# sourcedennis/wasm-pathtracer

Measured on AMD Instinct MI355X. Metric: Mray/s (primary+shadow+bounce) at 1920x1080, 1/2/4/8 GPU; L2 vs CPU ref, higher is better.
Workload: dtype f32; 1 GPU; C3 bunny scene (scene id 2), 1920x1080, 64 spp per GPU share (64 spp frame), depth 8, NormalNEE; rays=25682600955, parallelism=single GPU

## Files before the change

### include/wpt.h

```cpp
#ifndef WPT_H
#define WPT_H

#include <stddef.h>
#include <stdint.h>

#ifdef __cplusplus
extern "C" {
#endif

#define WPT_OK 0
#define WPT_ERR_NOT_INIT (-1)
#define WPT_ERR_ALREADY_INIT (-2)
#define WPT_ERR_INVALID_SCENE (-3)
#define WPT_ERR_INVALID_ARG (-4)
#define WPT_ERR_UNSUPPORTED (-5)
#define WPT_ERR_DEVICE (-6)
#define WPT_ERR_NO_MESH (-7)

#define WPT_NO_NEE 0
#define WPT_NORMAL_NEE 1
#define WPT_PNEE 2


int wpt_init(uint32_t width, uint32_t height, uint32_t scene_id, float cam_x, float cam_y, float cam_z,
// ... 17 lines not shown
int wpt_notify_mesh_loaded(uint32_t id);
int wpt_load_obj(uint32_t id, const char* text, size_t len, const float* scale, uint64_t* num_vertices);
int wpt_parse_obj(const char* text, size_t len, const float* scale, float* out, uint64_t capacity,
                  uint64_t* num_vertices);

uint8_t* wpt_allocate_texture(uint32_t id, uint32_t width, uint32_t height);

int wpt_notify_texture_loaded(uint32_t id);

int wpt_compute(size_t num_samples);


const char* wpt_last_error(void);

int wpt_set_device(int device);

int wpt_set_render_options(int32_t max_depth, uint32_t frame_seed, uint64_t batch_paths);

int wpt_set_partition(uint32_t rank, uint32_t nranks, uint32_t tile);

int64_t wpt_partition_pixels(uint32_t* out);

int64_t wpt_tile_partition(uint32_t width, uint32_t height, uint32_t rank, uint32_t nranks, uint32_t tile,
                           uint32_t* out);

int64_t wpt_photon_tree(uint32_t* child, float* cum, uint64_t* shot_stored);

int wpt_read_radiance(float* acc3, uint32_t* cnt);

int wpt_copy_partition(void* device_dst);

typedef int (*wpt_exchange_fn)(void* user);
int wpt_set_exchange(wpt_exchange_fn fn, void* user, void* local_dev, void* gathered_dev, uint64_t slot);
int64_t wpt_exchange_slot(void);

int wpt_comm_unique_id(void* out128);
int wpt_set_comm(uint32_t rank, uint32_t nranks, uint32_t tile, const void* unique_id128);
int wpt_gather_frame(uint32_t root);
int wpt_comm_destroy(void);
#define WPT_XFER_GATHER 0
#define WPT_XFER_ALLGATHER 1
typedef int (*wpt_transport_fn)(void* user, int32_t op, uint32_t root);
int wpt_set_transport(wpt_transport_fn fn, void* user, void* send_dev, void* recv_dev, uint64_t slot);
int64_t wpt_gather_plan(uint32_t rank, uint32_t nranks, uint32_t root, uint64_t slot, uint64_t* out);
float wpt_seq_sum(const float* v, uint64_t n);
float wpt_seq_sum_chunks(const float* v, uint64_t n);
int wpt_seq_sum_device(const float* v, uint64_t n, float* out);

int wpt_stats(uint64_t* out, size_t n);
int wpt_kernel_times(double* out, size_t n);
int wpt_set_counting(int on);
int wpt_set_profiling(int on);
int wpt_set_lanes(int32_t n);
#define WPT_OPT_DEFAULTS 0
#define WPT_OPT_TRAVERSAL 1
#define WPT_OPT_TRAVERSAL_SH 2
#define WPT_OPT_FUSED 3
#define WPT_OPT_FUSED_BELOW 4
#define WPT_OPT_SMALL_LANES 5
#define WPT_OPT_PIXEL_TILE 6
#define WPT_OPT_GRID_PCT 7
#define WPT_OPT_REFILL 8
#define WPT_OPT_REFILL_SH 9
#define WPT_OPT_TREELET 10
#define WPT_OPT_BVH_BUILD 11
#define WPT_OPT_LANES 12
#define WPT_OPT_FINISH_BELOW 13
#define WPT_OPT_TRACE_GRID_PCT 14
#define WPT_OPT_FINISH_EVERY 20
#define WPT_OPT_PROBE 22
#define WPT_OPT_STOCK 23
#define WPT_OPT_STOCK_LANES 24
#define WPT_OPT_FILL 25
#define WPT_OPT_ASYNC_PRIO 26
#define WPT_OPT_ASYNC_GRID_PCT 27
#define WPT_OPT_STOCK_AHEAD 30
#define WPT_OPT_STOCK_EVERY 32
#define WPT_OPT_STOCK_EXTRA 33
#define WPT_OPT_ASYNC_ONESHOT 31
#define WPT_OPT_STOCK_PREFILL 35
#define WPT_OPT_ASYNC_FUSED_BELOW 36
#define WPT_OPT_PRESOLVE 37
#define WPT_OPT_DROP_MISS 38
#define WPT_OPT_LOG 34
#define WPT_OPT_SCENE_TRAVERSAL 28
#define WPT_OPT_SCENE_TRI_ONLY 29
int wpt_set_option(int32_t option, int64_t value);
int64_t wpt_probe_read(uint32_t* meta, uint32_t* rec, uint64_t* rec_entries, double* ticks_per_us);
int wpt_get_option(int32_t option, int64_t* value);
int wpt_scene_build_info(double* out);
int wpt_clear_stats(void);
int wpt_sync(void);
int wpt_bvh_depth(void);

int wpt_trace_rays(size_t n, const float* rays, float* t_out, int32_t* id_out);
int wpt_shadow_rays(size_t n, const float* pq, const int32_t* light, uint8_t* occluded);
int wpt_presolve_rays(size_t n, const float* rays, uint8_t* resolved, float* t_out, int32_t* id_out);

int wpt_shutdown(void);

void* wpt_debug_scene_new(int32_t scene_id, const float* mesh_vertices, size_t num_vertices);
int wpt_debug_scene_info(void* h, uint64_t* out);
int wpt_debug_scene_nodes4(void* h, uint32_t* out);
int wpt_debug_scene_nodes(void* h, uint32_t* out);
int wpt_debug_scene_shapes(void* h, float* out);
int wpt_debug_scene_lights(void* h, uint32_t* out);
int wpt_debug_scene_presolve(void* h, size_t n, const float* rays, uint8_t* resolved, float* t_out, int32_t* id_out);
int wpt_debug_scene_guards(void* h, uint32_t* num_guards, float* boxes, uint32_t* leaf_guard);
void wpt_debug_scene_free(void* h);
void* wpt_debug_scene_new_gpu(int32_t scene_id, const float* mesh_vertices, size_t num_vertices);
int wpt_debug_scene_build_info(void* h, double* out);

#ifdef __cplusplus
}
#endif

#endif
```

### wasm-pathtracer_amd/_lib.py

```python
import ctypes
import os

HERE = os.path.dirname(os.path.abspath(__file__))
_VARIANT = os.environ.get("WPT_LIB_VARIANT", "")
LIB_PATH = os.path.join(HERE, f"libwpt_{_VARIANT}.so" if _VARIANT else "libwpt.so")

_lib = None

c_u32, c_i32, c_f32, c_sz = ctypes.c_uint32, ctypes.c_int32, ctypes.c_float, ctypes.c_size_t
c_p = ctypes.c_void_p

_SIGS = {
    "wpt_init": (ctypes.c_int, [c_u32, c_u32, c_u32, c_f32, c_f32, c_f32, c_f32, c_f32]),
    "wpt_results": (ctypes.POINTER(ctypes.c_uint8), [c_u32]),
    "wpt_update_scene": (ctypes.c_int, [c_u32]),
    "wpt_update_settings": (ctypes.c_int, [c_u32, c_u32, c_u32, c_u32, c_u32]),
    "wpt_update_viewport": (ctypes.c_int, [c_u32, c_u32]),
    "wpt_update_camera": (ctypes.c_int, [c_f32, c_f32, c_f32, c_f32, c_f32]),
    "wpt_allocate_mesh": (ctypes.c_int, [c_u32, c_u32]),
    "wpt_mesh_vertices": (ctypes.POINTER(ctypes.c_float), [c_u32]),
    "wpt_notify_mesh_loaded": (ctypes.c_int, [c_u32]),
    "wpt_load_obj": (ctypes.c_int, [c_u32, ctypes.c_char_p, c_sz, c_p, c_p]),
    "wpt_parse_obj": (ctypes.c_int, [ctypes.c_char_p, c_sz, c_p, c_p, ctypes.c_uint64, c_p]),
    "wpt_allocate_texture": (ctypes.POINTER(ctypes.c_uint8), [c_u32, c_u32, c_u32]),
    "wpt_notify_texture_loaded": (ctypes.c_int, [c_u32]),
    "wpt_compute": (ctypes.c_int, [c_sz]),
    "wpt_last_error": (ctypes.c_char_p, []),
    "wpt_set_device": (ctypes.c_int, [ctypes.c_int]),
    "wpt_set_render_options": (ctypes.c_int, [c_i32, c_u32, ctypes.c_uint64]),
    "wpt_set_partition": (ctypes.c_int, [c_u32, c_u32, c_u32]),
    "wpt_partition_pixels": (ctypes.c_int64, [c_p]),
    "wpt_tile_partition": (ctypes.c_int64, [c_u32, c_u32, c_u32, c_u32, c_u32, c_p]),
    "wpt_photon_tree": (ctypes.c_int64, [c_p, c_p, c_p]),
    "wpt_read_radiance": (ctypes.c_int, [c_p, c_p]),
    "wpt_copy_partition": (ctypes.c_int, [c_p]),
    "wpt_set_exchange": (ctypes.c_int, [c_p, c_p, c_p, c_p, ctypes.c_uint64]),
    "wpt_exchange_slot": (ctypes.c_int64, []),
    "wpt_stats": (ctypes.c_int, [c_p, c_sz]),
    "wpt_kernel_times": (ctypes.c_int, [c_p, c_sz]),
    "wpt_set_counting": (ctypes.c_int, [ctypes.c_int]),
    "wpt_set_profiling": (ctypes.c_int, [ctypes.c_int]),
    "wpt_set_lanes": (ctypes.c_int, [ctypes.c_int32]),
    "wpt_set_option": (ctypes.c_int, [ctypes.c_int32, ctypes.c_int64]),
    "wpt_get_option": (ctypes.c_int, [ctypes.c_int32, c_p]),
    "wpt_probe_read": (ctypes.c_int64, [c_p, c_p, c_p, c_p]),
    "wpt_scene_build_info": (ctypes.c_int, [c_p]),
    "wpt_clear_stats": (ctypes.c_int, []),
    "wpt_sync": (ctypes.c_int, []),
    "wpt_bvh_depth": (ctypes.c_int, []),
    "wpt_trace_rays": (ctypes.c_int, [c_sz, c_p, c_p, c_p]),
    "wpt_shadow_rays": (ctypes.c_int, [c_sz, c_p, c_p, c_p]),
    "wpt_presolve_rays": (ctypes.c_int, [c_sz, c_p, c_p, c_p, c_p]),
    "wpt_debug_scene_presolve": (ctypes.c_int, [c_p, c_sz, c_p, c_p, c_p, c_p]),
    "wpt_debug_scene_guards": (ctypes.c_int, [c_p, c_p, c_p, c_p]),
    "wpt_shutdown": (ctypes.c_int, []),
    "wpt_debug_scene_new": (c_p, [c_i32, c_p, c_sz]),
    "wpt_debug_scene_info": (ctypes.c_int, [c_p, c_p]),
    "wpt_debug_scene_nodes": (ctypes.c_int, [c_p, c_p]),
    "wpt_debug_scene_shapes": (ctypes.c_int, [c_p, c_p]),
    "wpt_debug_scene_nodes4": (ctypes.c_int, [c_p, c_p]),
    "wpt_comm_unique_id": (ctypes.c_int, [c_p]),
    "wpt_set_comm": (ctypes.c_int, [c_u32, c_u32, c_u32, c_p]),
    "wpt_gather_frame": (ctypes.c_int, [c_u32]),
    "wpt_comm_destroy": (ctypes.c_int, []),
    "wpt_set_transport": (ctypes.c_int, [c_p, c_p, c_p, c_p, ctypes.c_uint64]),
    "wpt_gather_plan": (ctypes.c_int64, [c_u32, c_u32, c_u32, ctypes.c_uint64, c_p]),
    "wpt_seq_sum": (ctypes.c_float, [c_p, ctypes.c_uint64]),
    "wpt_seq_sum_chunks": (ctypes.c_float, [c_p, ctypes.c_uint64]),
    "wpt_seq_sum_device": (ctypes.c_int, [c_p, ctypes.c_uint64, c_p]),
    "wpt_debug_scene_lights": (ctypes.c_int, [c_p, c_p]),
    "wpt_debug_scene_free": (None, [c_p]),
    "wpt_debug_scene_new_gpu": (c_p, [c_i32, c_p, c_sz]),
    "wpt_debug_scene_build_info": (ctypes.c_int, [c_p, c_p]),
}

EXPORTED = tuple(_SIGS)


def header_symbols():
    import re
    hdr = os.path.join(os.path.dirname(HERE), "include", "wpt.h")
    txt = open(hdr).read()
    return sorted(set(re.findall(r"\b(wpt_[a-z_0-9]+)\s*\(", txt)))


def lib():
    global _lib
    if _lib is not None:
        return _lib
    try:
        import torch
    except ImportError:
        pass
    if not os.path.exists(LIB_PATH):
        raise RuntimeError(f"{LIB_PATH} is missing: run __graft_entry__.build() (make -C wasm-pathtracer_amd/csrc)")
    L = ctypes.CDLL(LIB_PATH)
    for name, (res, args) in _SIGS.items():
        f = getattr(L, name)
        f.restype = res
        f.argtypes = args
    _lib = L
    return L
```

### wasm-pathtracer_amd/csrc/wpt_api.cpp

```cpp
#include <cstring>
#include <map>
#include <memory>
#include <string>
#include <vector>

#include "../../include/wpt.h"
#include "wpt_bvh_gpu.h"
#include "wpt_comm.h"
#include "wpt_obj.h"
#include "wpt_partition.h"
#include "wpt_render.h"
#include "wpt_seqsum.h"

using namespace wpt;

namespace {

struct Session {
  std::map<uint32_t, std::vector<float>> preload;
  std::map<uint32_t, std::vector<float>> meshes;
  std::map<uint32_t, std::vector<uint8_t>> textures;
  uint32_t scene_id = 0;
  HostScene scene;
  Renderer renderer;
// ... 411 lines not shown
  std::string err;
  if (!s.renderer.copy_partition((float*)s.comm_send, err)) return fail(WPT_ERR_DEVICE, err);
  if (!comm_gather(s.comm, s.comm_send, s.comm_recv, s.comm_slot, root, s.renderer.stream(), err))
    return fail(WPT_ERR_DEVICE, err);
  if (comm_rank(s.comm) == root && !s.renderer.unpack_ranks(s.comm_recv, s.comm_slot, err))
    return fail(WPT_ERR_DEVICE, err);
  return WPT_OK;
}

namespace {
int xfer_exchange(void* user) {
  Session& s = *(Session*)user;
  return s.xfer(s.xfer_user, WPT_XFER_ALLGATHER, 0);
}
}

int wpt_set_transport(wpt_transport_fn fn, void* user, void* send_dev, void* recv_dev, uint64_t slot) {
  if (!g_session) return fail(WPT_ERR_NOT_INIT, "init not called");
  Session& s = *g_session;
  if (!fn) {
    if (s.xfer) {
      s.renderer.set_exchange(nullptr, nullptr, nullptr, nullptr, 0);
      s.xfer = nullptr;
      s.xfer_user = nullptr;
      s.xfer_send = s.xfer_recv = nullptr;
      s.xfer_slot = 0;
    }
    return WPT_OK;
  }
  if (!send_dev || !recv_dev) return fail(WPT_ERR_INVALID_ARG, "null transport buffer");
  if (slot < s.renderer.exchange_slot() || slot < s.renderer.part_pixels())
    return fail(WPT_ERR_INVALID_ARG, "transport slot smaller than the largest partition");
  s.drop_comm();
  s.xfer = fn;
  s.xfer_user = user;
  s.xfer_send = (float4*)send_dev;
  s.xfer_recv = (float4*)recv_dev;
  s.xfer_slot = slot;
  s.renderer.set_exchange(xfer_exchange, &s, send_dev, recv_dev, slot);
  return WPT_OK;
}

int64_t wpt_gather_plan(uint32_t rank, uint32_t nranks, uint32_t root, uint64_t slot, uint64_t* out) {
  if (nranks == 0 || rank >= nranks || root >= nranks) return fail(WPT_ERR_INVALID_ARG, "bad rank");
  std::vector<XferOp> ops;
  gather_plan(rank, nranks, root, slot, ops);
  if (out)
    for (size_t i = 0; i < ops.size(); i++) {
      out[4 * i] = ops[i].peer;
      out[4 * i + 1] = ops[i].offset;
      out[4 * i + 2] = ops[i].count;
      out[4 * i + 3] = ops[i].recv ? 1u : 0u;
    }
  return (int64_t)ops.size();
}

float wpt_seq_sum(const float* v, uint64_t n) { return wpt::seq_sum_f32(v, (size_t)n); }

float wpt_seq_sum_chunks(const float* v, uint64_t n) {
  std::vector<wpt::ChunkEff> eff(2 * ((size_t)n / wpt::kSumChunk + 1));
  wpt::seq_sum_effects(v, (size_t)n, eff.data());
  return wpt::seq_sum_walk(v, (size_t)n, eff.data());
}

int wpt_seq_sum_device(const float* v, uint64_t n, float* out) {
  if (!g_session) return fail(WPT_ERR_NOT_INIT, "init not called");
  if (!out || (n && !v)) return fail(WPT_ERR_INVALID_ARG, "null pointer");
  std::string err;
  if (!g_session->renderer.seq_sum_device(v, n, *out, err)) return fail(WPT_ERR_DEVICE, err);
  return WPT_OK;
}

int wpt_comm_destroy(void) {
  if (!g_session) return fail(WPT_ERR_NOT_INIT, "init not called");
  g_session->drop_comm();
  return WPT_OK;
}

int wpt_stats(uint64_t* out, size_t n) {
  if (!g_session) return fail(WPT_ERR_NOT_INIT, "init not called");
  std::string err;
  if (!g_session->renderer.flush_counts(err)) return fail(WPT_ERR_DEVICE, err);
  const Stats& st = g_session->renderer.stats();
  uint64_t v[42] = {st.paths,          st.rays,           st.shadow_rays,    st.node_visits,  st.prim_tests,
                    st.bounces,        st.ext_visits,     st.ext_tests,      st.ext_node_bytes, st.sh_visits,
                    st.sh_tests,       st.sh_node_bytes,  st.fallback_ext,   st.fallback_sh,  st.ext_lane_iters,
                    st.ext_live_iters, st.sh_lane_iters,  st.sh_live_iters,  st.photon_rays,  st.photons,
                    st.sum_chunks,     st.sum_resummed,   st.sum_fetched,    st.stock_consumed, st.fill_paths,
                    st.trace_bytes,    st.finish_paths,   st.finish_max_bounces, st.max_ray_visits,
                    st.ex_body_lanes,  st.ex_bodies,      st.lf_body_lanes,  st.lf_bodies,    st.stock_traced,
                    st.stock_deficit,  st.stock_waits,    st.plan_us,        st.stock_us,
                    st.stock_rays,     st.stock_rays_used, st.presolved_rays,
                    st.dropped_rays};
  for (size_t i = 0; i < n && i < 42; i++) out[i] = v[i];
  return WPT_OK;
}

int wpt_kernel_times(double* out, size_t n) {
  if (!g_session) return fail(WPT_ERR_NOT_INIT, "init not called");
  const KernelTimes& t = g_session->renderer.times();
  double v[28] = {t.generate, (double)t.n_generate, t.extend, (double)t.n_extend, t.shade, (double)t.n_shade,
                  t.shadow, (double)t.n_shadow, t.accumulate, (double)t.n_accumulate, t.trace, (double)t.n_trace};
  for (int k = 0; k < 6; k++) {
    v[12 + 2 * k] = t.busy[k];
    v[13 + 2 * k] = (double)t.logical[k];
  }
  v[24] = t.retrace;
  v[25] = (double)t.n_retrace;
  v[26] = t.busy[6];
  v[27] = (double)t.logical[6];
  for (size_t i = 0; i < n && i < 28; i++) out[i] = v[i];
  return WPT_OK;
}

int wpt_set_counting(int on) {
  if (!g_session) return fail(WPT_ERR_NOT_INIT, "init not called");
  g_session->renderer.set_counting(on != 0);
  return WPT_OK;
}

int wpt_scene_build_info(double* out) {
  if (!g_session) return fail(WPT_ERR_NOT_INIT, "init not called");
  if (!out) return fail(WPT_ERR_INVALID_ARG, "null argument");
  out[0] = g_session->scene.bvh_ms;
  out[1] = g_session->scene.bvh_on_gpu ? 1.0 : 0.0;
  return WPT_OK;
}

int wpt_set_lanes(int32_t n) {
  if (!g_session) return fail(WPT_ERR_NOT_INIT, "init not called");
  if (!g_session->renderer.set_lanes(n)) return fail(WPT_ERR_INVALID_ARG, "lanes out of range");
  return WPT_OK;
}

int wpt_set_option(int32_t option, int64_t value) {
  if (option == WPT_OPT_BVH_BUILD) {
    if (value < 0 || value > 2) return fail(WPT_ERR_INVALID_ARG, "option value out of range");
    g_bvh_build = (int)value;
    return WPT_OK;
  }
  std::string err;
  if (!g_session) {
    if (option == WPT_OPT_DEFAULTS) {
      g_default_opts.clear();
      g_bvh_build = 0;
      return WPT_OK;
    }
    if (option == WPT_OPT_LANES && (value < 1 || value > kMaxLanes)) return fail(WPT_ERR_INVALID_ARG, "lanes out of range");
    if (option != WPT_OPT_LANES && option != WPT_OPT_GRID_PCT) {
      Renderer probe;
      if (!probe.set_option(option, value, err)) return fail(WPT_ERR_INVALID_ARG, err);
    } else if (option == WPT_OPT_GRID_PCT && (value < 1 || value > 100)) {
      return fail(WPT_ERR_INVALID_ARG, "option value out of range");
    }
    g_default_opts[option] = value;
    return WPT_OK;
  }
  Session& s = *g_session;
  int64_t prev = 0;
  const bool had = s.renderer.get_option(option, prev);
  if (!s.renderer.set_option(option, value, err)) return fail(WPT_ERR_INVALID_ARG, err);
  if (Renderer::scene_option(option)) {
    const int rc = rebuild_scene(s, s.scene_id);
    if (rc != WPT_OK) {
      const std::string keep = g_err;
      std::string e2;
      if (had) (void)s.renderer.set_option(option, prev, e2);
      g_err = keep;
      return rc;
    }
    return reset_session(s);
  }
  if (option == WPT_OPT_PIXEL_TILE && s.renderer.nranks() == 1) {
    if (!s.renderer.set_partition(s.renderer.rank(), s.renderer.nranks(), s.renderer.tile(), err))
      return fail(WPT_ERR_DEVICE, err);
  }
  return WPT_OK;
}

int64_t wpt_probe_read(uint32_t* meta, uint32_t* rec, uint64_t* rec_entries, double* ticks_per_us) {
  if (!g_session) return fail(WPT_ERR_NOT_INIT, "init not called");
  Session& s = *g_session;
  std::string err;
  if (!meta || !rec) {
    if (!s.renderer.probe_read(s.probe_meta, s.probe_rec, s.probe_tpu, err)) return fail(WPT_ERR_DEVICE, err);
    s.probe_taken = true;
    if (rec_entries) *rec_entries = s.probe_rec.size();
    if (ticks_per_us) *ticks_per_us = s.probe_tpu;
    return (int64_t)(s.probe_meta.size() / 5);
  }
  if (!s.probe_taken) return fail(WPT_ERR_INVALID_ARG, "probe: call with meta = rec = NULL first (size query)");
  if (!rec_entries || *rec_entries < s.probe_rec.size())
    return fail(WPT_ERR_INVALID_ARG, "probe: rec smaller than the size query's entries");
  std::memcpy(meta, s.probe_meta.data(), s.probe_meta.size() * sizeof(uint32_t));
  std::memcpy(rec, s.probe_rec.data(), s.probe_rec.size() * sizeof(uint4));
  *rec_entries = s.probe_rec.size();
  if (ticks_per_us) *ticks_per_us = s.probe_tpu;
  const int64_t n = (int64_t)(s.probe_meta.size() / 5);
  s.probe_meta.clear();
  s.probe_rec.clear();
  s.probe_taken = false;
  return n;
}

int wpt_get_option(int32_t option, int64_t* value) {
  if (!value) return fail(WPT_ERR_INVALID_ARG, "null argument");
  if (option == WPT_OPT_BVH_BUILD) { *value = g_bvh_build; return WPT_OK; }
  if (!g_session) {
    auto it = g_default_opts.find(option);
    if (it != g_default_opts.end()) { *value = it->second; return WPT_OK; }
    Renderer probe;
    if (!probe.get_option(option, *value)) return fail(WPT_ERR_INVALID_ARG, "unknown option");
    return WPT_OK;
  }
  if (!g_session->renderer.get_option(option, *value)) return fail(WPT_ERR_INVALID_ARG, "unknown option");
  return WPT_OK;
}

int wpt_set_profiling(int on) {
  if (!g_session) return fail(WPT_ERR_NOT_INIT, "init not called");
  g_session->renderer.set_profiling(on != 0);
  return WPT_OK;
}

int wpt_clear_stats(void) {
  if (!g_session) return fail(WPT_ERR_NOT_INIT, "init not called");
  g_session->renderer.clear_stats();
  return WPT_OK;
}

int wpt_sync(void) {
  if (!g_session) return fail(WPT_ERR_NOT_INIT, "init not called");
  std::string err;
  if (!g_session->renderer.sync(err)) return fail(WPT_ERR_DEVICE, err);
  return WPT_OK;
}

int wpt_bvh_depth(void) {
  if (!g_session) return fail(WPT_ERR_NOT_INIT, "init not called");
  return (int)g_session->renderer.bvh_depth();
}

int wpt_trace_rays(size_t n, const float* rays, float* t_out, int32_t* id_out) {
  if (!g_session) return fail(WPT_ERR_NOT_INIT, "init not called");
  std::string err;
  if (!g_session->renderer.trace_rays(n, rays, t_out, id_out, err)) return fail(WPT_ERR_DEVICE, err);
  return WPT_OK;
}

int wpt_presolve_rays(size_t n, const float* rays, uint8_t* resolved, float* t_out, int32_t* id_out) {
  if (!g_session) return fail(WPT_ERR_NOT_INIT, "init not called");
  if (n && (!rays || !resolved || !t_out || !id_out)) return fail(WPT_ERR_INVALID_ARG, "null argument");
  std::string err;
  if (!g_session->renderer.presolve_rays(n, rays, resolved, t_out, id_out, err)) return fail(WPT_ERR_DEVICE, err);
  return WPT_OK;
}

int wpt_shadow_rays(size_t n, const float* pq, const int32_t* light, uint8_t* occluded) {
  if (!g_session) return fail(WPT_ERR_NOT_INIT, "init not called");
  std::string err;
  if (!g_session->renderer.shadow_rays(n, pq, light, occluded, err)) return fail(WPT_ERR_INVALID_ARG, err);
  return WPT_OK;
}

int wpt_shutdown(void) {
  if (!g_session) return fail(WPT_ERR_NOT_INIT, "init not called");
  delete g_session;
  g_session = nullptr;
  return WPT_OK;
}

void* wpt_debug_scene_new(int32_t scene_id, const float* mesh_vertices, size_t num_vertices) {
  std::vector<float> mesh;
  if (mesh_vertices && num_vertices) mesh.assign(mesh_vertices, mesh_vertices + ((num_vertices / 3) * 9));
  HostScene* sc = new HostScene();
  std::string err;
  if (!build_scene(scene_id, mesh, *sc, err)) {
    delete sc;
    fail(WPT_ERR_INVALID_SCENE, err);
    return nullptr;
  }
  return sc;
}

void* wpt_debug_scene_new_gpu(int32_t scene_id, const float* mesh_vertices, size_t num_vertices) {
  static BvhGpu* gpu = nullptr;
  const hipError_t he = hipSetDevice(g_device);
  if (he != hipSuccess) {
    fail(WPT_ERR_DEVICE, std::string("hipSetDevice failed: ") + hipGetErrorString(he));
    return nullptr;
  }
  if (!gpu) gpu = new BvhGpu();
  gpu->min_shapes = 0;
  std::vector<float> mesh;
  if (mesh_vertices && num_vertices) mesh.assign(mesh_vertices, mesh_vertices + ((num_vertices / 3) * 9));
  HostScene* sc = new HostScene();
  std::string err;
  if (!build_scene(scene_id, mesh, *sc, err, gpu)) {
    delete sc;
    fail(err.rfind("HIP error", 0) == 0 || err.rfind("GPU BVH", 0) == 0 ? WPT_ERR_DEVICE : WPT_ERR_INVALID_SCENE,
         err);
    return nullptr;
  }
  return sc;
}

int wpt_debug_scene_build_info(void* h, double* out) {
  if (!h || !out) return fail(WPT_ERR_INVALID_ARG, "null argument");
  const HostScene* sc = (const HostScene*)h;
  out[0] = sc->bvh_ms;
  out[1] = sc->bvh_on_gpu ? 1.0 : 0.0;
  return WPT_OK;
}

int wpt_debug_scene_info(void* h, uint64_t* out) {
  const HostScene* sc = (const HostScene*)h;
  if (!sc) return fail(WPT_ERR_INVALID_ARG, "null scene");
  uint64_t v[8] = {sc->shapes.size(), sc->num_inf, sc->nodes.size(), sc->lights.size(), sc->depth,
                   sc->use_bvh ? 1u : 0u, sc->tri_only ? 1u : 0u, sc->nodes4.size()};
  memcpy(out, v, sizeof v);
  return WPT_OK;
}

int wpt_debug_scene_nodes(void* h, uint32_t* out) {
  const HostScene* sc = (const HostScene*)h;
  if (!sc) return fail(WPT_ERR_INVALID_ARG, "null scene");
  for (size_t i = 0; i < sc->nodes.size(); i++) {
    const Node2& n = sc->nodes[i];
    float b[6] = {n.bmin[0], n.bmin[1], n.bmin[2], n.bmax[0], n.bmax[1], n.bmax[2]};
    memcpy(out + 8 * i, b, sizeof b);
    out[8 * i + 6] = n.left_first;
    out[8 * i + 7] = n.count;
  }
  return WPT_OK;
}

int wpt_debug_scene_nodes4(void* h, uint32_t* out) {
  const HostScene* sc = (const HostScene*)h;
  if (!sc) return fail(WPT_ERR_INVALID_ARG, "null scene");
  for (size_t i = 0; i < sc->nodes4.size(); i++) {
    const Node4& n = sc->nodes4[i];
    uint32_t* o = out + 37 * i;
    memset(o, 0, 37 * sizeof(uint32_t));
    for (int k = 0; k < 4; k++) {
      const uint32_t c = n.child[k];
      if (c == kChildEmpty) continue;
      o[0]++;
      uint32_t* e = o + 1 + 9 * k;
      if (!(c & 0x80000000u)) {
        e[0] = 1;
        e[1] = c;
      } else {
        e[0] = 2;
        if ((c & 0xC0000000u) == 0xC0000000u) {
          e[1] = sc->leaf_table[2 * (c & 0x3FFFFFFFu)];
          e[2] = sc->leaf_table[2 * (c & 0x3FFFFFFFu) + 1];
        } else {
          e[1] = c & 0xFFFFFFu;
          e[2] = (c >> 24) & 0x3Fu;
        }
      }
      const float b[6] = {n.xmin[k], n.ymin[k], n.zmin[k], n.xmax[k], n.ymax[k], n.zmax[k]};
      memcpy(e + 3, b, sizeof b);
    }
  }
  return WPT_OK;
}

int wpt_debug_scene_shapes(void* h, float* out) {
  const HostScene* sc = (const HostScene*)h;
  if (!sc) return fail(WPT_ERR_INVALID_ARG, "null scene");
  for (size_t i = 0; i < sc->shapes.size(); i++) {
    const Shape& s = sc->shapes[i];
    float* o = out + 16 * i;
    memcpy(o, s.g, sizeof s.g);
    o[12] = (float)s.kind;
    o[13] = s.emissive ? 1.0f : 0.0f;
    o[14] = 0.0f;
    o[15] = 0.0f;
  }
  return WPT_OK;
}

int wpt_debug_scene_lights(void* h, uint32_t* out) {
  const HostScene* sc = (const HostScene*)h;
  if (!sc) return fail(WPT_ERR_INVALID_ARG, "null scene");
  for (size_t i = 0; i < sc->lights.size(); i++) out[i] = sc->lights[i];
  return WPT_OK;
}

int wpt_debug_scene_presolve(void* h, size_t n, const float* rays, uint8_t* resolved, float* t_out, int32_t* id_out) {
  const HostScene* sc = (const HostScene*)h;
  if (!sc || (n && (!rays || !resolved || !t_out || !id_out))) return fail(WPT_ERR_INVALID_ARG, "null argument");
  HostPlanes hp{};
  hp.num_inf = 0;
  PresolveBoxes pre{};
  if (sc->use_bvh && sc->shapes.size() > sc->num_inf && sc->num_inf <= 16) {
    pre = sc->pre;
    hp.num_inf = sc->num_inf;
    for (uint32_t i = 0; i < sc->num_inf; i++) {
      const float* g = sc->shapes[i].g;
      const V3 loc = mk(g[0], g[1], g[2]), nrm = mk(g[3], g[4], g[5]);
      hp.planes[i] = HostPlanes::P4{nrm.x, nrm.y, nrm.z, dot(nrm, loc)};
    }
  }
  for (size_t i = 0; i < n; i++) {
    const float* r = rays + 6 * i;
    resolved[i] = presolve_ray(hp, pre, mk(r[0], r[1], r[2]), mk(r[3], r[4], r[5]), t_out[i], id_out[i]) ? 1 : 0;
  }
  return WPT_OK;
}

int wpt_debug_scene_guards(void* h, uint32_t* num_guards, float* boxes, uint32_t* leaf_guard) {
  const HostScene* sc = (const HostScene*)h;
  if (!sc || !num_guards) return fail(WPT_ERR_INVALID_ARG, "null argument");
  *num_guards = sc->pre.num_guards;
  if (boxes) {
    memcpy(boxes, sc->pre.root, 6 * sizeof(float));
    memcpy(boxes + 6, sc->pre.guard, 6 * kMaxGuards * sizeof(float));
  }
  if (leaf_guard)
    for (size_t i = 0; i < sc->nodes.size(); i++) leaf_guard[i] = i < sc->leaf_guard.size() ? sc->leaf_guard[i] : ~0u;
  return WPT_OK;
}

void wpt_debug_scene_free(void* h) { delete (HostScene*)h; }

}
```

### wasm-pathtracer_amd/csrc/wpt_presolve.h

```cpp
#pragma once
#include "wpt_math.h"

namespace wpt {

constexpr int kMaxGuards = 4;

struct PresolveBoxes {
  uint32_t num_guards;
  float root[6];
  float guard[kMaxGuards][6];
};

WPT_HD void presolve_slab(const float* b, V3 o, V3 inv, float& hh, float& tmax) {
  const float tx1 = (b[0] - o.x) * inv.x;
  const float tx2 = (b[3] - o.x) * inv.x;
  const float ty1 = (b[1] - o.y) * inv.y;
  const float ty2 = (b[4] - o.y) * inv.y;
  const float tz1 = (b[2] - o.z) * inv.z;
  const float tz2 = (b[5] - o.z) * inv.z;
  const float tmin = fmaxf(fmaxf(fminf(tx1, tx2), fminf(ty1, ty2)), fminf(tz1, tz2));
  tmax = fminf(fminf(fmaxf(tx1, tx2), fmaxf(ty1, ty2)), fmaxf(tz1, tz2));
  hh = fmaxf(tmin, 0.0f);
}

WPT_HD float presolve_inf() {
#if defined(__HIP_DEVICE_COMPILE__)
  float v;
  asm volatile("v_mov_b32 %0, 0x7f800000" : "=v"(v));
  return v;
#else
  return u2f(0x7f800000u);
#endif
}

template <class SC>
WPT_HD bool presolve_ray(const SC& S, const PresolveBoxes& B, V3 o, V3 d, float& t, int32_t& id) {
  t = 0.0f;
  id = -1;
  if (B.num_guards == 0u) return false;
  if (d.x == 0.0f || d.y == 0.0f || d.z == 0.0f) return false;
  const V3 inv = mk(1.0f / d.x, 1.0f / d.y, 1.0f / d.z);
  const float inf = presolve_inf();
  if (!(fabsf(inv.x) < inf) || !(fabsf(inv.y) < inf) || !(fabsf(inv.z) < inf)) return false;
  float best = inf;
  int32_t best_id = -1;
  bool found = false;
  for (uint32_t i = 0; i < S.num_inf; i++) {
    const V3 n = mk(S.planes[i].x, S.planes[i].y, S.planes[i].z);
    const float n_dot_dir = dot(n, d);
    if (n_dot_dir == 0.0f) continue;
    const float tt = (S.planes[i].w - dot(n, o)) / n_dot_dir;
    if (tt <= 0.0f) continue;
    if (!found || (0.0f < tt && tt < best)) {
      found = true;
      best = tt;
      best_id = (int32_t)i;
    }
  }
  float hh, tmax;
  presolve_slab(B.root, o, inv, hh, tmax);
  if ((hh <= tmax) & (hh < best)) {
    bool clear = true;
#if defined(__HIP_DEVICE_COMPILE__)
#pragma unroll
#endif
    for (int g = 0; g < kMaxGuards; g++) {
      if ((uint32_t)g < B.num_guards) {
        presolve_slab(B.guard[g], o, inv, hh, tmax);
        clear = clear && (!(hh <= tmax) || best < hh);
      }
    }
    if (!clear) return false;
  }
  t = best_id >= 0 ? best : inf;
  id = best_id;
  return true;
}

struct HostPlanes {
  struct P4 { float x, y, z, w; };
  P4 planes[16];
  uint32_t num_inf;
};

}
```

### wasm-pathtracer_amd/csrc/wpt_render.h

```cpp
#pragma once
#include <hip/hip_runtime.h>
#include <stdint.h>
#include <string>
#include <algorithm>
#include <deque>
#include <vector>

#include "wpt_scene.h"
#include "wpt_seqsum.h"

namespace wpt {

constexpr int kMaxInf = 16;
constexpr int kMaxBvhDepth = 4096;
constexpr int kMaxBounces = 512;

struct DevScene {
  const float4* nodes;
  const float4* tree;
  uint32_t tree_pairs, tree_root_lf;
  const float4* prims;
  const uint32_t* kinds;
  const float4* all;
  const uint32_t* all_kinds;
  const float4* mats;
  const float4* lights;
  const float4* nodes4;
  const uint32_t* leaf_table;
  uint32_t num_inf, num_finite, num_shapes, num_lights;
  uint32_t use_bvh, tri_only;
  uint32_t refill_lanes;
  uint32_t refill_lanes_sh;
  int stack_cap;
  uint32_t* overflow;
  const uint32_t* oct_child;
  const float* oct_cum;
  const uint32_t* oct_corners;
  uint32_t oct_nodes;
  uint32_t oct_lds_words;
  float bg[3];
  float4 planes[kMaxInf];
  uint4* probe;
  const PresolveBoxes* pre;
};

struct Stats {
  uint64_t paths = 0;
  uint64_t rays = 0;
  uint64_t shadow_rays = 0;
  uint64_t node_visits = 0;
  uint64_t prim_tests = 0;
  uint64_t bounces = 0;
  uint64_t ext_visits = 0, ext_tests = 0, ext_node_bytes = 0;
  uint64_t sh_visits = 0, sh_tests = 0, sh_node_bytes = 0;
  uint64_t fallback_ext = 0, fallback_sh = 0;
  uint64_t ex_body_lanes = 0, ex_bodies = 0, lf_body_lanes = 0, lf_bodies = 0;
  uint64_t ext_lane_iters = 0, ext_live_iters = 0, sh_lane_iters = 0, sh_live_iters = 0;
  uint64_t photon_rays = 0, photons = 0;
  uint64_t trace_bytes = 0;
  uint64_t max_ray_visits = 0;
  uint64_t sum_chunks = 0, sum_resummed = 0, sum_fetched = 0;
  uint64_t finish_paths = 0, finish_max_bounces = 0;
  uint64_t stock_traced = 0, stock_consumed = 0, fill_paths = 0;
  uint64_t stock_deficit = 0, stock_waits = 0, plan_us = 0, stock_us = 0;
  uint64_t stock_rays = 0;
  uint64_t stock_rays_used = 0;
  uint64_t presolved_rays = 0;
  uint64_t dropped_rays = 0;
};

constexpr int kTimedKernels = 7;
struct KernelTimes {
  double generate = 0, extend = 0, shade = 0, shadow = 0, accumulate = 0, trace = 0, retrace = 0;
  uint64_t n_extend = 0, n_shadow = 0, n_shade = 0, n_generate = 0, n_accumulate = 0, n_trace = 0, n_retrace = 0;
  double busy[kTimedKernels] = {0, 0, 0, 0, 0, 0, 0};
  uint64_t logical[kTimedKernels] = {0, 0, 0, 0, 0, 0, 0};
};

constexpr int kMaxLanes = 8;
constexpr uint64_t kMinLanePaths = 1024;
constexpr size_t kFinishWord = 2 + 2 * (size_t)kMaxBounces;
constexpr size_t kResWord = kFinishWord + 4;
constexpr size_t kCountWords = kResWord + 2 * ((size_t)kMaxBounces + 1);
static_assert(kResWord % 2 == 0, "the presolved counts are 64-bit slots");
constexpr uint32_t kWorkWords = 16;
constexpr uint32_t kWorkCopies = 64;
struct PathSet {
  hipStream_t stream = nullptr;
  hipStream_t lo = nullptr;
  hipEvent_t done = nullptr;
  uint64_t cap = 0;
  uint32_t* pixel = nullptr;
  float4* col = nullptr;
  float4* ro[2] = {nullptr, nullptr};
  float4* rd[2] = {nullptr, nullptr};
  float4* thr[2] = {nullptr, nullptr};
  float* t = nullptr;
  int32_t* id = nullptr;
  float* t1 = nullptr;
  int32_t* id1 = nullptr;
  float4 *so = nullptr, *sd = nullptr, *sc = nullptr;
  uint32_t* counts = nullptr;
  uint32_t* h_counts = nullptr;
  uint2* spill = nullptr;
  size_t spill_cap = 0;
  float* hit_t(int k) const { return k ? t1 : t; }
  int32_t* hit_id(int k) const { return k ? id1 : id; }
  uint32_t* ext_count(int b) const { return b == 0 ? counts : counts + 2 + 2 * (b - 1); }
  uint32_t* sh_count(int b) const { return counts + 3 + 2 * b; }
  unsigned long long* append_ctr(int b) const { return reinterpret_cast<unsigned long long*>(counts + 2 + 2 * b); }
  unsigned long long* res_ctr(int b) const { return reinterpret_cast<unsigned long long*>(counts + kResWord + 2 * b); }
};

constexpr int kAsyncLane0 = 2;
struct Batch {
  enum State { kNew, kBouncing, kCountWait, kIssued };
  uint64_t k0 = 0, n = 0;
  int half = -1;
  const uint32_t* part = nullptr;
  uint32_t npix = 0;
  const uint32_t* moff = nullptr;
  const uint32_t* mbase = nullptr;
  const uint32_t* mlist = nullptr;
  uint32_t nent = 0;
  bool stock = false;
  bool async = false;
  int queue = 0;
  int lane0 = 0, nl = 1;
  uint64_t off[kMaxLanes + 1] = {};
  bool fused = false, pnee = false;
  bool presolve = false;
  int maxb = 0, b = 0;
  bool finished = false;
  State state = kNew;
  hipEvent_t done[kMaxLanes] = {};
  hipEvent_t live[kMaxLanes] = {};
  uint32_t* hc = nullptr;
  uint32_t* hl = nullptr;
};

struct LaunchCtx {
  int lane = 0;
  const PathSet* ps = nullptr;
  hipStream_t stream = nullptr;
  bool async = false;
  uint64_t paths = 0;
  int batch_lanes = 1;
  bool timed = false;
  bool count = false;
  int bounce = 0;
  int hit_sel = 0;
  const uint32_t* probe_res = nullptr;
};

class Renderer {
 public:
  Renderer();
  ~Renderer();
  bool set_device(int dev, std::string& err);
  bool upload_scene(const HostScene& sc, std::string& err);
  bool set_viewport(uint32_t w, uint32_t h, std::string& err);
  void set_camera(const float cam[5]);
  void set_types(int left, int right, int debug) { left_type_ = left; right_type_ = right; debug_ = debug; }
  void set_adaptive(bool left, bool right) { adaptive_[0] = left; adaptive_[1] = right; }
  bool adaptive() const { return adaptive_[0] || adaptive_[1]; }
  bool fill_sampling_blue(std::string& err);
  bool sampling_rgba(uint8_t* out, std::string& err);
  void set_options(int max_depth, uint32_t seed, uint64_t batch) {
    if (seed != seed_) photons_ok_ = false;
    max_depth_ = max_depth; seed_ = seed; if (batch) batch_ = batch;
  }
  bool build_photons(std::string& err);
  bool photon_tree(std::vector<uint32_t>& child, std::vector<float>& cum, uint64_t& shot, uint64_t& stored,
                   std::string& err);
  bool set_partition(uint32_t rank, uint32_t nranks, uint32_t tile, std::string& err);
  bool reset(std::string& err);
  bool compute(uint64_t num_paths, std::string& err);
  bool sync(std::string& err);
  bool results_rgba(uint8_t* host_out, std::string& err);
  bool read_radiance(float* acc3, uint32_t* cnt, std::string& err);
  bool copy_partition(float* dev_dst, std::string& err);
  using ExchangeFn = int (*)(void*);
  void set_exchange(ExchangeFn fn, void* user, void* local_dev, void* gathered_dev, uint64_t slot) {
    xfn_ = fn; xuser_ = user; xlocal_ = (float4*)local_dev; xall_ = (float4*)gathered_dev; xslot_ = slot;
  }
  uint64_t exchange_slot() const { return maxpart_; }
  uint32_t rank() const { return rank_; }
  uint32_t nranks() const { return nranks_; }
  uint32_t tile() const { return tile_; }
  bool unpack_ranks(const float4* gathered, uint64_t slot, std::string& err);
  bool trace_rays(size_t n, const float* rays, float* t_out, int32_t* id_out, std::string& err);
  bool presolve_rays(size_t n, const float* rays, uint8_t* resolved, float* t_out, int32_t* id_out, std::string& err);
  bool shadow_rays(size_t n, const float* pq, const int32_t* light, uint8_t* occ, std::string& err);
  bool probe_read(std::vector<uint32_t>& meta, std::vector<uint4>& rec, double& ticks_per_us, std::string& err);
  void set_counting(bool on) { counting_ = on; }
  void set_profiling(bool on) { profiling_ = on; }
  bool set_lanes(int n) {
    if (n < 1 || n > lanes_made_) return false;
    nlanes_ = n;
    return true;
  }
  int lanes() const { return nlanes_; }
  static bool scene_option(int opt) { return opt == 1 || opt == 2 || opt == 10; }
  bool set_option(int opt, int64_t v, std::string& err);
  bool get_option(int opt, int64_t& v) const;
  int wants_bvh4() const {
    return (traversal_ == 1 || traversal_sh_ == 1) ? 1 : (traversal_ == 3 || traversal_sh_ == 3) ? 2 : 0;
  }
  bool seq_sum_device(const float* v, uint64_t n, float& out, std::string& err);
  const Stats& stats() const { return stats_; }
  const KernelTimes& times() const { return times_; }
  void clear_stats() {
    std::string e;
    (void)flush_counts(e);
    stats_ = Stats();
    times_ = KernelTimes();
  }
  bool flush_counts(std::string& err);
  uint32_t width() const { return w_; }
  uint32_t height() const { return h_; }
  uint32_t part_pixels() const { return (uint32_t)part_pix_.size(); }
  const std::vector<uint32_t>& part_list() const { return part_pix_; }
  hipStream_t stream() const { return stream_; }
  uint32_t bvh_depth() const { return depth_; }

 private:
  bool ensure_paths(uint64_t n, std::string& err);
  bool ensure_lane(int i, uint64_t n, std::string& err);
  void free_lane_paths(PathSet& L);
  LaunchCtx batch_ctx(const Batch& B, int i, int b) const;
  LaunchCtx lane0_ctx(bool count) const;
  bool run_batch(uint64_t k0, uint64_t n, int half, std::string& err, const uint32_t* part_pix = nullptr,
                 uint32_t part_n = 0, const Batch* map = nullptr);
  bool batch_begin(Batch& B, std::string& err);
  bool batch_advance(Batch& B, bool block, std::string& err);
  bool batch_tail(Batch& B, std::string& err);
  void batch_counts(const Batch& B, const uint32_t* hc);
  bool pump(bool block, std::string& err);
  bool wait_issued(Batch* B, std::string& err);
  bool drain_async(std::string& err);
  bool host_wait(hipEvent_t e, std::string& err);
  bool host_wait_stream(hipStream_t s, std::string& err);
  hipEvent_t ev_sync_ = nullptr;
  uint64_t batch_cap() const;
  int main_lanes() const;
  bool compute_half(int h, uint64_t n, std::string& err);
  bool merge_random_halves(uint64_t nl, uint64_t nr, bool& merged, std::string& err);
  bool plan_round(int h, std::string& err);
  bool exchange_frame(std::string& err);
  bool plan_slice(int h, uint64_t a, uint64_t b, uint64_t& local, std::string& err);
  void free_rounds();
  bool launch_extend(const LaunchCtx& C, const float4* ro, const float4* rd, const uint32_t* cnt, std::string& err);
  bool launch_shadow(const LaunchCtx& C, const uint32_t* cnt, uint8_t* occ_out, std::string& err);
  bool launch_trace(const LaunchCtx& C, std::string& err);
  bool size_grids(std::string& err);
  uint32_t max_grid() const;
  size_t spill_slots() const;
  uint32_t spill_grid(const PathSet& L) const;
  bool ensure_spill(int l, uint32_t grid, std::string& err);
  uint32_t oneshot_grid(uint64_t paths) const {
    const uint64_t g = (2 * paths + 255) / 256;
    const uint64_t gmax = (1ull << 30) / (sizeof(uint2) * 256 * spill_slots());
    return (uint32_t)std::max<uint64_t>(1, std::min(g, gmax));
  }
  void free_scene();
  void free_paths();
  void free_photons();
  bool adaptive_[2] = {false, false};
  struct HalfRounds {
    uint64_t total = 0, pos = 0;
    uint32_t idx = 0;
    uint32_t* rc = nullptr;
    uint32_t* rbase = nullptr;
    uint32_t* gc = nullptr;
    uint32_t* gbase = nullptr;
// ... 44 lines not shown
  uint32_t refill_id_ = 0;
  int refill_lane_ = 0;
  uint32_t round_need_[2] = {0, 0};
  bool stock_redo_[2] = {false, false};
  int log_ = 0;
  bool stock_active(int h) const { return stock_slots_ != 0 && nranks_ == 1 && adaptive_[h]; }
  bool stock_alloc(std::string& err);
  void stock_drop();
  bool stock_round(int h, uint64_t left, std::string& err);
  bool stock_consume(int h, uint64_t a, uint64_t b, std::string& err);
  bool stock_flush(std::string& err);
  bool refill_count(Refill& f, bool block, std::string& err);
  uint32_t refill_scale(int h, uint32_t ahead, uint64_t after) const;
  Refill* refill_slot(std::string& err);
  void refill_plan(Refill& F, int h, uint32_t ahead, uint32_t q);
  bool refill_issue(Refill& F, int h, uint64_t wt, std::string& err);
  bool stock_prefill(int h, uint64_t budget, std::string& err);
  bool stock_prefill_ = true;
  std::deque<Batch*> aq_[2];
  bool fill_on_ = false;
  int async_prio_ = 0;
  int async_grid_pct_ = 100;
  uint64_t async_fused_below_ = 1ull << 26;
  uint32_t* d_seam_pix_[2] = {nullptr, nullptr};
  uint32_t* d_rest_pix_[2] = {nullptr, nullptr};
  uint32_t seam_npix_[2] = {0, 0}, rest_npix_[2] = {0, 0};
  static constexpr int kMaxFill = 8;
  Batch fill_[kMaxFill];
  int nfill_ = 0;
  hipEvent_t fill_ev_[kMaxFill][2] = {};
  uint32_t* h_fill_cnt_ = nullptr;
  bool async_pending() const { return !aq_[0].empty() || !aq_[1].empty(); }
  int fill_lane() const { return kAsyncLane0 + stock_lanes_; }
  bool issue_fill(int h, uint64_t k0, uint64_t n, std::string& err);
  bool drain_fill(std::string& err);
  bool compute_halves(uint64_t nl, uint64_t nr, std::string& err);
  uint32_t async_grid(const LaunchCtx& C, uint32_t g, int base_pct, uint32_t rays_per_path = 1) const {
    if (!C.async) return g;
    if (async_oneshot_) return std::max<uint32_t>(1u, (uint32_t)((C.paths * rays_per_path + 255) / 256));
    return async_grid_pct_ > 0 ? std::max<uint32_t>(1u, (uint32_t)((uint64_t)g * async_grid_pct_ / base_pct)) : g;
  }
  bool async_oneshot_ = false;
  uint8_t* d_samp_ = nullptr;
  ExchangeFn xfn_ = nullptr;
  void* xuser_ = nullptr;
  float4* xlocal_ = nullptr;
  float4* xall_ = nullptr;
  uint64_t xslot_ = 0;
  uint64_t maxpart_ = 0;
  uint32_t* d_xidx_ = nullptr;
  bool photons_ok_ = false;
  uint64_t photons_shot_ = 0, photons_stored_ = 0;
  std::vector<uint32_t> oct_child_;
  std::vector<float> oct_cum_;
  uint32_t* d_oct_child_ = nullptr;
  float* d_oct_cum_ = nullptr;
  uint32_t* d_oct_corners_ = nullptr;

  int device_ = -1;
  int ncu_ = 256;
  static constexpr int kTravVariants = 8;
  uint32_t grid_ext_[2 * kTravVariants] = {};
  uint32_t grid_sh_[2 * kTravVariants] = {};
  uint32_t grid_tr_[4] = {};
  uint32_t grid_shade_ = 512;
  uint32_t shade_occ_[32] = {};
  size_t shade_occ_smem_[32] = {};
  bool fused_ = false;
  uint64_t fused_below_ = 1ull << 24;
  int small_lanes_ = 2;
  int traversal_ = 3, traversal_sh_ = 3;
  int trav_ext_ = 0, trav_sh_ = 0;
  bool treelet_ = true;
  uint32_t pixel_tile_ = 8;
  int grid_pct_ = 50;
#ifndef WPT_TRACE_GRID_PCT
#define WPT_TRACE_GRID_PCT 75
#endif
  int trace_grid_pct_ = WPT_TRACE_GRID_PCT;
  uint32_t refill_ = 12, refill_sh_ = 16;
  uint64_t finish_below_ = 1u << 18;
  int finish_every_ = 4;
  uint32_t num_guards_ = 0;
  bool presolve_ = true;
  bool drop_miss_ = true;
  uint32_t probe_cap_ = 0, probe_waves_ = 0, probe_used_ = 0;
  uint4* d_probe_ = nullptr;
  std::vector<uint32_t> probe_meta_;
  uint4* probe_slot(const LaunchCtx& C, int kernel, uint32_t grid);
  uint32_t* d_fallback_ = nullptr;
  hipStream_t stream_ = nullptr;
  PathSet lanes_[kMaxLanes];
  int lanes_made_ = 0;
  bool stats_pending_ = false;
  int pend_nl_ = 0, pend_b_ = 0;
  bool pend_stock_ = false, pend_presolve_ = false;
  int nlanes_ = 4;
  hipEvent_t ev_main_ = nullptr;
  hipEvent_t ev_ref_ = nullptr;
  std::vector<void*> scene_bufs_;
  DevScene ds_{};
  uint32_t depth_ = 0;
  bool scene_ok_ = false;

  uint32_t w_ = 0, h_ = 0;
  float cam_[5] = {0, 0, 0, 0, 0};
  int left_type_ = 1, right_type_ = 1, debug_ = 0;
  int max_depth_ = 0;
  uint32_t seed_ = 0xBABABEBEu;
  uint64_t batch_ = 1ull << 27;

  uint32_t rank_ = 0, nranks_ = 1, tile_ = 16;
  std::vector<uint32_t> part_pix_;
  uint32_t* d_part_pix_ = nullptr;
  uint32_t* d_half_pix_[2] = {nullptr, nullptr};
  uint32_t* d_frame_pix_ = nullptr;
  uint32_t half_npix_[2] = {0, 0};
  uint64_t next_path_ = 0;

  float4* d_acc_ = nullptr;
  uint32_t* d_cnt_ = nullptr;
  uint8_t* d_rgba_ = nullptr;

  unsigned long long* d_work_ = nullptr;
  uint32_t* h_word_ = nullptr;

  bool counting_ = false;
  bool profiling_ = false;
  Stats stats_;
  KernelTimes times_;
  struct PendingTiming {
    hipEvent_t a, b;
    int slot;
  };
  bool next_event(hipEvent_t* e, std::string& err);
  bool resolve_timings(std::string& err);
  std::vector<hipEvent_t> ev_pool_;
  size_t ev_used_ = 0;
  std::vector<PendingTiming> pending_;
};

}
```

### wasm-pathtracer_amd/csrc/wpt_render.hip

```cpp
#include "wpt_render.h"
#include "wpt_partition.h"
#include "wpt_photon.h"
#include "wpt_quartic.h"
#include "wpt_seqsum.h"

#include <algorithm>
#include <chrono>
#include <cstdlib>
#include <cmath>
#include <cstdio>
#include <cstring>
#include <deque>
#include <mutex>
#include <unordered_map>
#include <thread>
#include <type_traits>

#define HIP_OK(expr)                                                     \
  do {                                                                   \
    hipError_t e_ = (expr);                                              \
    if (e_ != hipSuccess) {                                              \
      err = std::string(#expr " failed: ") + hipGetErrorString(e_);      \
      return false;                                                      \
    }                                                                    \
// ... 925 lines not shown
  const bool self_z = xs_next(s) <= wz;
  const float ajx = xs * xo, ajy = ys * yo, ajz = zs * zo;
  uint32_t corner[8];
  if (depth <= kOctLattice) {
    const int32_t kx = (int32_t)((b[0] + sz) / xs), ky = (int32_t)((b[1] + sz) / ys), kz = (int32_t)((b[2] + sz) / zs);
    const uint32_t ax = oct_cell(v.x + ajx, kx + (int32_t)xo, xs, depth);
    const uint32_t ay = oct_cell(v.y + ajy, ky + (int32_t)yo, ys, depth);
    const uint32_t az = oct_cell(v.z + ajz, kz + (int32_t)zo, zs, depth);
    corner[0] = leaf;
    const int32_t last = (1 << depth) - 1;
    const auto adj = [&](int32_t k, float off) {
      const int32_t a = k + (int32_t)off;
      return (uint32_t)(a < 0 ? 0 : (a > last ? last : a));
    };
    if (WPT_OCT_TABLE && S.oct_corners && ax == adj(kx, xo) && ay == adj(ky, yo) && az == adj(kz, zo)) {
      const uint32_t ocase = (xo > 0.0f ? 4u : 0u) | (yo > 0.0f ? 2u : 0u) | (zo > 0.0f ? 1u : 0u);
      const uint4* row = reinterpret_cast<const uint4*>(S.oct_corners + 64 * (size_t)leaf + 8 * ocase);
      const uint4 q0 = row[0], q1 = row[1];
      corner[1] = q0.y;
      corner[2] = q0.z;
      corner[3] = q0.w;
      corner[4] = q1.x;
      corner[5] = q1.y;
      corner[6] = q1.z;
      corner[7] = q1.w;
    } else {
#pragma unroll
      for (int c = 1; c < 8; c++)
        corner[c] =
            oct_walk(O, (c & 4) ? ax : (uint32_t)kx, (c & 2) ? ay : (uint32_t)ky, (c & 1) ? az : (uint32_t)kz, depth);
    }
  } else {
    float nb[6];
    int d;
    corner[0] = leaf;
#pragma unroll
    for (int c = 1; c < 8; c++)
      corner[c] = oct_find(S, O, add(v, mk((c & 4) ? ajx : 0.0f, (c & 2) ? ajy : 0.0f, (c & 1) ? ajz : 0.0f)), depth, nb, d);
  }
  const int pick = (self_x ? 0 : 4) + (self_y ? 0 : 2) + (self_z ? 0 : 1);
  uint32_t node = corner[0];
#pragma unroll
  for (int c = 1; c < 8; c++) node = pick == c ? corner[c] : node;
  const auto cum = O.cum + (size_t)node * S.num_lights;
  const float r = xs_next(s);
  uint32_t lo = 0, hi = S.num_lights;
  while (lo + 1u < hi) {
    const uint32_t mid = (lo + hi) / 2u;
    if (cum[mid] <= r) lo = mid;
    else hi = mid;
  }
  light = lo;
  float p = 0.0f;
  p += oct_bin_prob(S, O, corner[0], lo) * wx * wy * wz;
  p += oct_bin_prob(S, O, corner[4], lo) * wax * wy * wz;
  p += oct_bin_prob(S, O, corner[2], lo) * wx * way * wz;
  p += oct_bin_prob(S, O, corner[1], lo) * wx * wy * waz;
  p += oct_bin_prob(S, O, corner[6], lo) * wax * way * wz;
  p += oct_bin_prob(S, O, corner[3], lo) * wx * way * waz;
  p += oct_bin_prob(S, O, corner[5], lo) * wax * wy * waz;
  p += oct_bin_prob(S, O, corner[7], lo) * wax * way * waz;
  pdf = p;
}

template <bool TRI_ONLY>
__device__ __forceinline__ V3 hit_normal(const DevScene& S, int32_t id, V3 o, V3 d, float t) {
  uint32_t kind;
  const float4* rec = shape_rec<TRI_ONLY>(S, id, kind);
  if (rec) return TRI_ONLY ? tri_normal(rec, d) : prim_normal(kind, rec, o, d, t);
  V3 pn = ld3(S.planes[id]);
  if (dot(pn, d) > 0.0f) pn = neg(pn);
  return normalize(pn);
}

__device__ __forceinline__ void st_hit(float* t, int32_t* id, float tv, int32_t iv) {
  *t = tv;
  *id = iv;
}

struct ShadeParams {
  int max_depth;
  int debug;
  int drop_miss;
};

struct RayStream {
  float4* o;
  float4* d;
  float4* thr;
};
struct ShadowStream {
  float4* o;
  float4* d;
  float4* c;
};

struct ShadeOut {
  bool alive, shadow;
  float4 ro, rd, th;
  float4 so, sd, sc;
};

template <bool TRI_ONLY, bool PNEE, class OV, bool CR = false>
__device__ __forceinline__ void shade_path(const DevScene& S, const OV& O, const ShadeParams& P,
                                           float4* __restrict__ col, float t,
                                           int32_t id, float4 o4, float4 d4, float4 th4, ShadeOut& R,
                                           const lds_f4v* lq = nullptr) {
  const V3 o = ld3(o4), d = ld3(d4);
  const uint32_t path = __float_as_uint(d4.w);
  V3 thr = ld3(th4);
  uint32_t flags = __float_as_uint(th4.w);
  const uint32_t type = (flags >> kTypeShift) & 3u;
  const bool has_nee = type == 1u || type == 2u;
  bool bounced = (flags & kFlagBounced) != 0;
  const uint32_t depth = ((flags >> kDepthShift) & kDepthMask) + 1u;
  auto end_counts = [&](uint32_t nsh) {
    if constexpr (CR) reinterpret_cast<uint32_t*>(col + path)[3] = depth | (nsh << 16);
  };
  if (id < 0) {
    const V3 add_c = mulv(thr, mk(S.bg[0], S.bg[1], S.bg[2]));
    if ((__float_as_uint(add_c.x) | __float_as_uint(add_c.y) | __float_as_uint(add_c.z)) != 0u) {
      const float4 c4 = col[path];
      const V3 c = add(ld3(c4), add_c);
      col[path] = make_float4(c.x, c.y, c.z, c4.w);
    }
    end_counts(flags >> kShadowShift);
    return;
  }
  const float4 m = S.mats[id];
  V3 nrm = mk(0.0f, 0.0f, 0.0f);
  if (TRI_ONLY) nrm = hit_normal<TRI_ONLY>(S, id, o, d, t);
  const V3 hp = add(o, scale(d, t));
  if (m.w != 0.0f) {
    if (P.debug ? !bounced : (!has_nee || !bounced)) {
      const float4 c4 = col[path];
      const V3 c = add(ld3(c4), mulv(thr, ld3(m)));
      col[path] = make_float4(c.x, c.y, c.z, c4.w);
    }
    end_counts(flags >> kShadowShift);
    return;
  }
  if (!TRI_ONLY) nrm = hit_normal<TRI_ONLY>(S, id, o, d, t);
  uint32_t s = __float_as_uint(o4.w);
  const float r1 = xs_next(s);
  const float r2 = xs_next(s);
  const float ang = (2.0f * kPi) * r1;
  const float x = mcos(ang) * sqrtf(1.0f - r2);
  const float y = sqrtf(r2);
  const float z = msin(ang) * sqrtf(1.0f - r2);
  const V3 xn = orthogonal(nrm);
  const V3 zn = cross(nrm, xn);
  const V3 wi = normalize(add(add(scale(xn, x), scale(nrm, y)), scale(zn, z)));
  const float pdf = dot(wi, nrm) / kPi;
  const float ipi = 1.0f / kPi;
  const V3 brdf = mk(clamp01(ipi * m.x), clamp01(ipi * m.y), clamp01(ipi * m.z));
  const float cos_i = dot(wi, nrm);
  thr = divs(scale(mulv(thr, brdf), cos_i), pdf);
  const V3 no = add(hp, scale(wi, kEpsilon));
  bounced = true;
  if (has_nee && S.num_lights > 0) {
    uint32_t li;
    float light_chance;
    if (PNEE && type == 2u) {
      photon_sample(S, O, s, hp, li, light_chance);
    } else {
      li = xs_next_in_range(s, S.num_lights);
      light_chance = 1.0f / (float)S.num_lights;
    }
    float4 L0, L1, L2, L3, L4;
    if (lq) {
      const lds_f4v* q = lq + 5 * li;
      L0 = to_f4(q[0]);
      L1 = to_f4(q[1]);
      L2 = to_f4(q[2]);
      L3 = to_f4(q[3]);
      L4 = to_f4(q[4]);
    } else {
      const float4* L = S.lights + 5 * (size_t)li;
      L0 = L[0];
      L1 = L[1];
      L2 = L[2];
      L3 = L[3];
      L4 = L[4];
    }
    const float q1 = xs_next(s);
    const float q2 = xs_next(s);
    const float q1s = sqrtf(q1);
    const V3 pt = add(add(scale(ld3(L0), 1.0f - q1s), scale(ld3(L1), q1s * (1.0f - q2))), scale(ld3(L2), q2 * q1s));
    V3 ln = ld3(L3);
    if (xs_next(s) > 0.5f) ln = neg(ln);
    const V3 inten = ld3(L4);
    V3 tl = sub(pt, hp);
    const float d2 = dot(tl, tl);
    const float dl = sqrtf(d2);
    tl = divs(tl, dl);
    const float ci = dot(tl, nrm);
    const float co = dot(neg(tl), ln);
    if (ci > 0.0f && co > 0.0f) {
      if (P.debug) {
        const float4 c4 = col[path];
        const V3 c = add(ld3(c4), mulv(thr, inten));
        col[path] = make_float4(c.x, c.y, c.z, c4.w);
      } else {
        const float solid = (L0.w * co) / d2;
        const V3 contrib = scale(scale(scale(mulv(thr, inten), solid), ci), 1.0f / light_chance);
        const V3 sorig = add(hp, scale(tl, kEpsilon));
        R.so = make_float4(sorig.x, sorig.y, sorig.z, dl);
        R.sd = make_float4(tl.x, tl.y, tl.z, L1.w);
        R.sc = make_float4(contrib.x, contrib.y, contrib.z, d4.w);
        R.shadow = true;
      }
    }
  }
  const bool capped = P.max_depth > 0 && (int)depth >= P.max_depth;
  if (!capped && depth < (uint32_t)kMaxBounces) {
    const float keep = fmaxf(fminf(fmaxf(fmaxf(thr.x, thr.y), thr.z), 0.9f), 0.1f);
    if (xs_next(s) < keep) {
      thr = scale(thr, 1.0f / keep);
      const uint32_t nsh = (flags >> kShadowShift) + (R.shadow ? 1u : 0u);
      flags = (flags & ~((~0u) << kDepthShift)) | (depth << kDepthShift) | (nsh << kShadowShift) | kFlagBounced;
      R.ro = make_float4(no.x, no.y, no.z, __uint_as_float(s));
      R.rd = make_float4(wi.x, wi.y, wi.z, d4.w);
      R.th = make_float4(thr.x, thr.y, thr.z, __uint_as_float(flags));
      R.alive = true;
    }
  }
  if (!R.alive) end_counts((flags >> kShadowShift) + (R.shadow ? 1u : 0u));
}

template <bool TRI_ONLY, bool PNEE, int OCT, bool CR = false, bool PS = false>
__global__ void WPT_SHADE_BOUNDS k_shade(DevScene S, ShadeParams P, RayStream in, RayStream out,
                                                       ShadowStream sh, float4* __restrict__ col,
                                                       const uint32_t* __restrict__ count, const float* __restrict__ t_in,
                                                       const int32_t* __restrict__ id_in,
                                                       unsigned long long* __restrict__ append,
                                                       float* __restrict__ t_nx, int32_t* __restrict__ id_nx,
                                                       uint32_t end) {
  constexpr uint32_t kWaves = kShadeBlock / 64;
  static_assert(kWaves < 64, "the scan's totals and the second atomic lane sit in one wave");
  __shared__ uint32_t s_off[PS ? 3 : 2][kWaves];
  __shared__ f4v s_light[5 * kShadeLights];
  const uint32_t nh = *count;
  const uint32_t n = PS ? nh + reinterpret_cast<const uint32_t*>(append)[kResWord - 2] : nh;
  const bool lds_lights = S.num_lights <= kShadeLights;
  if (lds_lights) {
    for (uint32_t k = threadIdx.x; k < 5 * S.num_lights; k += kShadeBlock) {
      const float4 v = S.lights[k];
      s_light[k] = f4v{v.x, v.y, v.z, v.w};
    }
  }
  extern __shared__ uint32_t s_oct[];
  if (PNEE && OCT != 0) {
    const uint32_t nc = S.oct_nodes, nw = S.oct_lds_words;
    for (uint32_t k = threadIdx.x; k < nw; k += kShadeBlock)
      s_oct[k] = k < nc ? S.oct_child[k] : __float_as_uint(S.oct_cum[k - nc]);
  }
  __syncthreads();
  using OV = std::conditional_t<OCT == 2, OctL2, std::conditional_t<OCT == 1, OctL1, OctG>>;
  OV O;
  if constexpr (OCT == 2) {
    O.child = (const lds_u32*)s_oct;
    O.cum = (const lds_f32*)(s_oct + S.oct_nodes);
  } else if constexpr (OCT == 1) {
    O.child = (const lds_u32*)s_oct;
    O.cum = S.oct_cum;
  } else {
    O.child = S.oct_child;
    O.cum = S.oct_cum;
  }
  const uint32_t lane = threadIdx.x & 63u, wid = threadIdx.x >> 6;
  const uint64_t below = (1ull << lane) - 1ull;
  for (uint32_t i0 = blockIdx.x * kShadeBlock; i0 < n; i0 += gridDim.x * kShadeBlock) {
    const uint32_t i = i0 + threadIdx.x;
    ShadeOut R;
    R.alive = R.shadow = false;
    if (i < n) {
      const uint32_t q = !PS || i < nh ? i : end - 1u - (i - nh);
      shade_path<TRI_ONLY, PNEE, OV, CR>(S, O, P, col, t_in[q], id_in[q], in.o[q], in.d[q], in.thr[q], R,
                                     lds_lights ? (const lds_f4v*)s_light : nullptr);
    }
    bool res = false;
    float pt = 0.0f;
    int32_t pid = -1;
    if constexpr (PS) {
      if (R.alive) res = presolve_ray(S, *S.pre, ld3(R.ro), ld3(R.rd), pt, pid);
    }
    bool drop = false;
    if constexpr (PS) {
      if (res && pid < 0 && P.drop_miss) {
        const V3 add_c = mulv(ld3(R.th), mk(S.bg[0], S.bg[1], S.bg[2]));
        drop = (__float_as_uint(add_c.x) | __float_as_uint(add_c.y) | __float_as_uint(add_c.z)) == 0u;
      }
      if (drop) {
        R.alive = res = false;
        if constexpr (CR) {
          const uint32_t f = __float_as_uint(R.th.w);
          reinterpret_cast<uint32_t*>(col + __float_as_uint(R.rd.w))[3] =
              (((f >> kDepthShift) & kDepthMask) + 1u) | ((f >> kShadowShift) << 16);
        }
      }
    }
    const uint64_t am = __ballot(R.alive && !res), sm = __ballot(R.shadow), rm = PS ? __ballot(res) : 0ull;
    const uint64_t dm = PS ? __ballot(drop) : 0ull;
    if (lane == 0) {
      s_off[0][wid] = (uint32_t)__popcll(am);
      s_off[1][wid] = (uint32_t)__popcll(sm);
      if constexpr (PS) s_off[2][wid] = (uint32_t)__popcll(rm) | ((uint32_t)__popcll(dm) << 16);
    }
    __syncthreads();
    if constexpr (!PS) {
      if (wid == 0) {
        const uint32_t a = lane < kWaves ? s_off[0][lane] : 0u, b = lane < kWaves ? s_off[1][lane] : 0u;
        uint32_t ia = a, ib = b;
#pragma unroll
        for (uint32_t k = 1; k < kWaves; k <<= 1) {
          const uint32_t ya = __shfl_up(ia, k, 64), yb = __shfl_up(ib, k, 64);
          if (lane >= k) { ia += ya; ib += yb; }
        }
        unsigned long long base = 0ull;
        if (lane == kWaves - 1) base = atomicAdd(append, (unsigned long long)ia | ((unsigned long long)ib << 32));
        const uint32_t ba = (uint32_t)__shfl((int)(uint32_t)base, (int)(kWaves - 1), 64);
        const uint32_t bb = (uint32_t)__shfl((int)(uint32_t)(base >> 32), (int)(kWaves - 1), 64);
        if (lane < kWaves) {
          s_off[0][lane] = ba + ia - a;
          s_off[1][lane] = bb + ib - b;
        }
      }
    } else if (wid == 0) {
      const uint32_t a = lane < kWaves ? s_off[0][lane] : 0u, b = lane < kWaves ? s_off[1][lane] : 0u;
      const uint32_t c = lane < kWaves ? s_off[2][lane] : 0u;
      uint32_t ia = a, ib = b, ic = c;
#pragma unroll
      for (uint32_t k = 1; k < kWaves; k <<= 1) {
        const uint32_t ya = __shfl_up(ia, k, 64), yb = __shfl_up(ib, k, 64), yc = __shfl_up(ic, k, 64);
        if (lane >= k) { ia += ya; ib += yb; ic += yc; }
      }
      const uint32_t tc = (uint32_t)__shfl((int)ic, (int)(kWaves - 1), 64);
      unsigned long long base = 0ull;
      uint32_t off;
      asm volatile("v_mov_b32 %0, %1" : "=v"(off) : "i"((uint32_t)(kResWord / 2)));
      if (lane == kWaves - 1 || lane == kWaves)
        base = atomicAdd(append + (lane == kWaves - 1 ? 0u : off),
                         lane == kWaves - 1 ? ((unsigned long long)ia | ((unsigned long long)ib << 32))
                                            : ((unsigned long long)(tc & 0xffffu) | ((unsigned long long)(tc >> 16) << 32)));
      const uint32_t ba = (uint32_t)__shfl((int)(uint32_t)base, (int)(kWaves - 1), 64);
      const uint32_t bb = (uint32_t)__shfl((int)(uint32_t)(base >> 32), (int)(kWaves - 1), 64);
      const uint32_t bc = (uint32_t)__shfl((int)(uint32_t)base, (int)kWaves, 64);
      if (lane < kWaves) {
        s_off[0][lane] = ba + ia - a;
        s_off[1][lane] = bb + ib - b;
        s_off[2][lane] = bc + ((ic - c) & 0xffffu);
      }
    }
    __syncthreads();
    if (R.alive) {
      uint32_t p = s_off[0][wid] + (uint32_t)__popcll(am & below);
      if constexpr (PS) {
        if (res) p = end - 1u - (s_off[2][wid] + (uint32_t)__popcll(rm & below));
      }
      st_stream(out.o + p, R.ro);
      st_stream(out.d + p, R.rd);
      st_stream(out.thr + p, R.th);
      if constexpr (PS) {
        if (res) {
          t_nx[p] = pt;
          id_nx[p] = pid;
        }
      }
    }
    if (R.shadow) {
      const uint32_t p = s_off[1][wid] + (uint32_t)__popcll(sm & below);
      st_stream(sh.o + p, R.so);
      st_stream(sh.d + p, R.sd);
      st_stream(sh.c + p, R.sc);
    }
    __syncthreads();
  }
}

struct WaveFeed {
  uint32_t n, v, wave, nwaves;
  __device__ WaveFeed(uint32_t n_) : n(n_), v(0) {
    wave = (blockIdx.x * kTBlock + threadIdx.x) >> 6;
    nwaves = (gridDim.x * kTBlock) >> 6;
  }
  static constexpr uint32_t K = kFeedChunk;
  __device__ uint32_t pos(uint32_t k) const { return ((k / K) * nwaves + wave) * K + (k % K); }
  __device__ bool more() const { return pos(v) < n; }
  __device__ uint32_t taken() const { return taken_below(n); }
  __device__ uint32_t taken_below(uint32_t m) const {
    const uint32_t C = m / K, rem = m % K;
    const uint32_t full = C > wave ? (C - wave - 1u) / nwaves + 1u : 0u;
    const uint32_t part = (rem != 0u && C % nwaves == wave) ? rem : 0u;
    return min(v, full * K + part);
  }
  __device__ uint32_t take(uint64_t take_m) {
    const uint32_t rank = (uint32_t)__popcll(take_m & ((1ull << (threadIdx.x & 63)) - 1ull));
    const uint32_t p = pos(v + rank);
    v += (uint32_t)__popcll(take_m);
    return p;
  }
};

__global__ void __launch_bounds__(kBlock) k_photon_gen(DevScene S, uint32_t seed, uint32_t k0, uint32_t n,
                                                       float4* __restrict__ ro, float4* __restrict__ rd,
                                                       float4* __restrict__ rec) {
  const uint32_t i = blockIdx.x * kBlock + threadIdx.x;
  if (i >= n) return;
  uint32_t s = photon_seed(seed, k0 + i);
  const uint32_t li = xs_next_in_range(s, S.num_lights);
  const float4* L = S.lights + 5 * (size_t)li;
  const float4 L0 = L[0], L1 = L[1], L2 = L[2], L3 = L[3], L4 = L[4];
  const float q1 = xs_next(s);
  const float q2 = xs_next(s);
  const float q1s = sqrtf(q1);
  const V3 pt = add(add(scale(ld3(L0), 1.0f - q1s), scale(ld3(L1), q1s * (1.0f - q2))), scale(ld3(L2), q2 * q1s));
  V3 ln = ld3(L3);
  if (xs_next(s) > 0.5f) ln = neg(ln);
  float x, y, z;
  do {
    x = xs_next(s) * 2.0f - 1.0f;
    y = xs_next(s) * 2.0f - 1.0f;
    z = xs_next(s) * 2.0f - 1.0f;
  } while (x * x + y * y + z * z > 1.0f);
  V3 v = normalize(mk(x, y, z));
  if (dot(v, ln) < 0.0f) v = neg(v);
  const V3 o = add(pt, scale(v, kEpsilon));
  ro[i] = make_float4(o.x, o.y, o.z, 0.0f);
  rd[i] = make_float4(v.x, v.y, v.z, 0.0f);
  const float imax = fmaxf(fmaxf(L4.x, L4.y), L4.z);
  rec[i] = make_float4(__uint_as_float(li), dot(ln, v) * imax, 0.0f, 0.0f);
}

template <bool TRI_ONLY>
__global__ void __launch_bounds__(kBlock) k_photon_hit(DevScene S, uint32_t n, const float4* __restrict__ ro,
                                                       const float4* __restrict__ rd, const float* __restrict__ t_in,
                                                       const int32_t* __restrict__ id_in,
                                                       const float4* __restrict__ rec, float4* __restrict__ hit_out,
                                                       uint32_t* __restrict__ light_out) {
  const uint32_t i = blockIdx.x * kBlock + threadIdx.x;
  if (i >= n) return;
  const int32_t id = id_in[i];
  const float4 r = rec[i];
  if (id < 0 || S.mats[id].w != 0.0f) {
    light_out[i] = 0xFFFFFFFFu;
    return;
  }
  const V3 o = ld3(ro[i]), d = ld3(rd[i]);
  const float t = t_in[i];
  const V3 nrm = hit_normal<TRI_ONLY>(S, id, o, d, t);
  const V3 hp = add(add(o, scale(d, t)), scale(nrm, kEpsilon));
  hit_out[i] = make_float4(hp.x, hp.y, hp.z, r.y);
  light_out[i] = __float_as_uint(r.x);
// ... 296 lines not shown
        cv = ct = cb = 0;
      }
    }
  }
  if (COUNT) {
    const unsigned long long wet = wave_sum(et), wst = wave_sum(st), web = wave_sum(eb), wsb = wave_sum(sb);
    work_add(work, 0, ev);
    work_add_wave(work, 1, wet);
    work_add_wave(work, 2, web);
    work_add(work, 3, sv);
    work_add_wave(work, 4, wst);
    work_add_wave(work, 5, wsb);
    const unsigned long long ne_w = feed.taken_below(ne), ns_w = feed.taken() - ne_w;
    work_add_wave(work, 15, 40ull * ne_w + 64ull * ns_w + web + wsb + 64ull * (wet + wst));
    bodies.flush(work, 6, 8);
    for (int o = 32; o > 0; o >>= 1) vmax = max(vmax, (uint32_t)__shfl_xor((int)vmax, o));
    if ((threadIdx.x & 63u) == 0u && vmax) atomicMax(work + (blockIdx.x & (kWorkCopies - 1u)) * kWorkWords + 14, (unsigned long long)vmax);
  }
}

template <bool TRI_ONLY, bool PNEE, bool CR = false>
#ifndef WPT_FINISH_WAVES
#define WPT_FINISH_WAVES 1
#endif
__global__ void __launch_bounds__(kTBlock, TRI_ONLY ? WPT_FINISH_WAVES : 1) k_finish(DevScene S, ShadeParams P, RayStream in,
                                                   const uint32_t* __restrict__ count, float4* __restrict__ col,
                                                   uint2* __restrict__ spill, uint32_t* __restrict__ counters) {
  __shared__ uint32_t s_code[kLdsSlots * kTBlock];
  __shared__ float s_h[kLdsSlots * kTBlock];
  __shared__ float s_lrec[16 * kLdsLights];
  __shared__ int32_t s_lid[kLdsLights];
  __shared__ f4v s_tree[4 * kTreePairs + 1];
  const Hot H = load_hot(S, (lds_f32h*)s_lrec, (lds_i32*)s_lid, (lds_f4v*)s_tree, (const float4*)s_tree);
  const uint32_t n = *count;
  const uint32_t G = gridDim.x * kTBlock;
  const Stack stk{(lds_u32*)(s_code + threadIdx.x), (lds_f32*)(s_h + threadIdx.x),
                  spill + blockIdx.x * kTBlock + threadIdx.x, G, S.stack_cap, S.overflow};
  const OctG O{S.oct_child, S.oct_cum};
  const float inf = __int_as_float(0x7f800000);
  uint32_t nrays = 0, nshadow = 0, npaths = 0, longest = 0, dummy = 0;
  for (uint32_t i = blockIdx.x * kTBlock + threadIdx.x; i < n; i += G) {
    float4 o4 = in.o[i], d4 = in.d[i], th4 = in.thr[i];
    const uint32_t r0 = nrays;
    npaths++;
    for (;;) {
      Lane L;
      bool occ = false;
      nrays++;
      if (begin_extend<TRI_ONLY, false, false>(S, H, L, ld3(o4), ld3(d4), dummy, dummy, dummy))
        while (step<false, TRI_ONLY, false, false>(S, H, L, stk, -1, 0.0f, occ, dummy, dummy, dummy)) {
        }
      ShadeOut R;
      R.alive = R.shadow = false;
      shade_path<TRI_ONLY, PNEE, OctG, CR>(S, O, P, col, L.best_id >= 0 ? L.best : inf, L.best_id, o4, d4, th4, R);
      if (R.shadow) {
        nshadow++;
        const float dir_len = R.so.w, early0 = 0.0f;
        const int32_t light = (int32_t)__float_as_uint(R.sd.w);
        float early = early0;
        bool occluded = false;
        Lane Ls;
        if (begin_shadow<TRI_ONLY, false, false>(S, H, Ls, ld3(R.so), ld3(R.sd), dir_len, light, early, occluded,
                                                 dummy, dummy, dummy))
          while (step<true, TRI_ONLY, false, false>(S, H, Ls, stk, light, early, occluded, dummy, dummy, dummy)) {
          }
        if (!shadow_verdict(Ls, dir_len, light, occluded)) add_contribution(col, R.sc);
      }
      if (!R.alive) break;
      o4 = R.ro;
      d4 = R.rd;
      th4 = R.th;
    }
    longest = max(longest, nrays - r0);
  }
  if (nrays) atomicAdd(counters, nrays);
  if (nshadow) atomicAdd(counters + 1, nshadow);
  if (npaths) {
    atomicAdd(counters + 2, npaths);
    atomicMax(counters + 3, longest);
  }
}

__global__ void k_probe_add(uint4* rec, const uint32_t* __restrict__ res) { rec[0].w += res[0] + res[1]; }

__global__ void __launch_bounds__(kBlock) k_presolve(DevScene S, uint32_t n, const float* __restrict__ rays,
                                                     uint8_t* __restrict__ resolved, float* __restrict__ t_out,
                                                     int32_t* __restrict__ id_out) {
  const uint32_t i = blockIdx.x * kBlock + threadIdx.x;
  if (i >= n) return;
  const float* r = rays + 6 * (size_t)i;
  float t;
  int32_t id;
  const bool res = presolve_ray(S, *S.pre, mk(r[0], r[1], r[2]), mk(r[3], r[4], r[5]), t, id);
  resolved[i] = res ? 1 : 0;
  t_out[i] = t;
  id_out[i] = id;
}

__global__ void __launch_bounds__(kBlock) k_accumulate(const uint32_t* __restrict__ part_pix, uint64_t k0, uint32_t n,
                                                       uint32_t npix, const float4* __restrict__ col,
                                                       float4* __restrict__ acc, uint32_t* __restrict__ cnt) {
  const uint32_t i = blockIdx.x * kBlock + threadIdx.x;
  const uint32_t lim = n < npix ? n : npix;
  if (i >= lim) return;
  const uint32_t pl = (uint32_t)((k0 + i) % npix);
  const uint32_t pixel = part_pix ? part_pix[pl] : pl;
  float4 a = acc[pixel];
  uint32_t c = cnt[pixel];
  for (uint32_t j = i; j < n; j += npix) {
    const float4 v = col[j];
    a.x += v.x;
    a.y += v.y;
    a.z += v.z;
    c += 1;
  }
  acc[pixel] = a;
  cnt[pixel] = c;
}

__global__ void k_rgba(const float4* __restrict__ acc, const uint32_t* __restrict__ cnt, uint32_t npix,
                       uint8_t* __restrict__ out) {
  const uint32_t i = blockIdx.x * kBlock + threadIdx.x;
  if (i >= npix) return;
  const float4 a = acc[i];
  const uint32_t c = cnt[i];
  uchar4 r = make_uchar4(0, 0, 0, 255);
  if (c > 0) {
    const float fc = (float)c;
    r.x = (uint8_t)(fmaxf(fminf(a.x / fc, 1.0f), 0.0f) * 255.0f);
    r.y = (uint8_t)(fmaxf(fminf(a.y / fc, 1.0f), 0.0f) * 255.0f);
    r.z = (uint8_t)(fmaxf(fminf(a.z / fc, 1.0f), 0.0f) * 255.0f);
  }
  reinterpret_cast<uchar4*>(out)[i] = r;
}

__global__ void k_pack_partition(const uint32_t* __restrict__ part_pix, uint32_t n, const float4* __restrict__ acc,
                                 const uint32_t* __restrict__ cnt, float4* __restrict__ out) {
  const uint32_t i = blockIdx.x * kBlock + threadIdx.x;
  if (i >= n) return;
  const uint32_t p = part_pix ? part_pix[i] : i;
  float4 a = acc[p];
  a.w = __uint_as_float(cnt[p]);
  out[i] = a;
}

inline uint32_t blocks_for(uint64_t n) { return (uint32_t)((n + kBlock - 1) / kBlock); }

}

namespace {
struct RingBlock {
  int dev;
  void* p;
  size_t bytes;
};
constexpr size_t kRingCacheBlocks = 4;
std::mutex& ring_mu() {
  static std::mutex* m = new std::mutex;
  return *m;
}
std::vector<RingBlock>& ring_cache() {
  static std::vector<RingBlock>* v = new std::vector<RingBlock>;
  return *v;
}
}

static hipError_t ring_take(int dev, size_t bytes, void** p, size_t* got) {
  {
    std::lock_guard<std::mutex> g(ring_mu());
    auto& c = ring_cache();
    size_t best = c.size();
    for (size_t i = 0; i < c.size(); i++)
      if (c[i].dev == dev && c[i].bytes >= bytes && c[i].bytes / 2 <= bytes && (best == c.size() || c[i].bytes < c[best].bytes))
        best = i;
    if (best < c.size()) {
      *p = c[best].p;
      *got = c[best].bytes;
      c.erase(c.begin() + best);
      return hipSuccess;
// ... 86 lines not shown
  }
  if (h_fill_cnt_) (void)hipHostFree(h_fill_cnt_);
  for (auto& fe : fill_ev_)
    for (hipEvent_t e : fe)
      if (e) (void)hipEventDestroy(e);
  if (ev_main_) (void)hipEventDestroy(ev_main_);
  if (ev_sync_) (void)hipEventDestroy(ev_sync_);
  if (ev_ref_) (void)hipEventDestroy(ev_ref_);
  if (h_word_) (void)hipHostFree(h_word_);
  for (auto& e : ev_pool_)
    if (e) (void)hipEventDestroy(e);
  if (stream_) (void)hipStreamDestroy(stream_);
}

bool Renderer::set_device(int dev, std::string& err) {
  if (device_ == dev && stream_) return true;
  if (stream_) {
    err = "device already selected";
    return false;
  }
  HIP_OK(hipSetDevice(dev));
  device_ = dev;
  HIP_OK(hipStreamCreateWithFlags(&stream_, hipStreamNonBlocking));
  HIP_OK(hipDeviceGetAttribute(&ncu_, hipDeviceAttributeMultiprocessorCount, dev));
  HIP_OK(hipEventCreateWithFlags(&ev_main_, hipEventDisableTiming));
  HIP_OK(hipEventCreateWithFlags(&ev_sync_, hipEventDisableTiming));
  HIP_OK(hipEventCreate(&ev_ref_));
  HIP_OK(hipHostMalloc(&h_word_, sizeof(uint32_t) * 4));
  lanes_made_ = kMaxLanes;
  for (int i = 0; i < kMaxLanes; i++) {
    PathSet& L = lanes_[i];
    if (i == 0) L.stream = stream_;
    else HIP_OK(hipStreamCreateWithFlags(&L.stream, hipStreamNonBlocking));
    HIP_OK(hipEventCreateWithFlags(&L.done, hipEventDisableTiming));
    HIP_OK(hipMalloc(&L.counts, sizeof(uint32_t) * kCountWords));
    HIP_OK(hipHostMalloc(&L.h_counts, sizeof(uint32_t) * kCountWords));
  }
  HIP_OK(hipMalloc(&d_work_, sizeof(unsigned long long) * kWorkWords * kWorkCopies));
  HIP_OK(hipMalloc(&d_fallback_, sizeof(uint32_t) * 4));
  HIP_OK(hipMemset(d_fallback_, 0, sizeof(uint32_t) * 4));
  HIP_OK(hipMemset(d_work_, 0, sizeof(unsigned long long) * kWorkWords * kWorkCopies));
  return true;
}

void Renderer::free_scene() {
  for (void* p : scene_bufs_) (void)hipFree(p);
  scene_bufs_.clear();
  scene_ok_ = false;
}

void Renderer::free_lane_paths(PathSet& L) {
  void* bufs[] = {L.pixel, L.col, L.ro[0], L.rd[0], L.thr[0], L.ro[1], L.rd[1], L.thr[1], L.t, L.id, L.t1, L.id1,
                  L.so, L.sd, L.sc};
  for (void* p : bufs)
    if (p) (void)hipFree(p);
  L.pixel = nullptr;
  L.col = nullptr;
  for (int k = 0; k < 2; k++) L.ro[k] = L.rd[k] = L.thr[k] = nullptr;
  L.t = L.t1 = nullptr;
  L.id = L.id1 = nullptr;
  L.so = L.sd = L.sc = nullptr;
  L.cap = 0;
}

void Renderer::free_paths() {
  for (PathSet& L : lanes_) free_lane_paths(L);
}

bool Renderer::upload_scene(const HostScene& sc, std::string& err) {
  if (!stream_) { err = "no device"; return false; }
  if (!drain_async(err)) return false;
  stock_drop();
  HIP_OK(hipStreamSynchronize(stream_));
  free_photons();
  free_scene();
  if (sc.num_inf > (uint32_t)kMaxInf && sc.use_bvh) { err = "too many infinite shapes"; return false; }
  if (sc.use_bvh && sc.depth >= (uint32_t)kMaxBvhDepth) { err = "BVH deeper than supported"; return false; }
  const size_t ns = sc.shapes.size();
  const size_t nf = ns - sc.num_inf;
  auto rec = [](const Shape& s, float4* out) {
    memset(out, 0, 4 * sizeof(float4));
    const float* g = s.g;
    if (s.kind == kTri) {
      V3 v0 = mk(g[0], g[1], g[2]), v1 = mk(g[3], g[4], g[5]), v2 = mk(g[6], g[7], g[8]);
      V3 n = cross(sub(v1, v0), sub(v2, v0));
      V3 nn = normalize(n);
      float od = dot(n, v0);
      out[0] = make_float4(v0.x, v0.y, v0.z, n.x);
      out[1] = make_float4(v1.x, v1.y, v1.z, n.y);
      out[2] = make_float4(v2.x, v2.y, v2.z, n.z);
      out[3] = make_float4(nn.x, nn.y, nn.z, od);
    } else if (s.kind == kPlane) {
      V3 loc = mk(g[0], g[1], g[2]), n = mk(g[3], g[4], g[5]);
      out[0] = make_float4(n.x, n.y, n.z, dot(n, loc));
      out[1] = make_float4(loc.x, loc.y, loc.z, 0.0f);
    } else if (s.kind == kSphere) {
      out[0] = make_float4(g[0], g[1], g[2], g[3]);
    } else if (s.kind == kTorus) {
      out[0] = make_float4(g[0], g[1], g[2], g[3]);
      out[1] = make_float4(g[4], 0.0f, 0.0f, 0.0f);
    } else {
      out[0] = make_float4(g[0], g[1], g[2], g[3]);
      out[1] = make_float4(g[4], g[5], 0.0f, 0.0f);
    }
  };
  std::vector<float4> prims(4 * std::max<size_t>(nf, 1)), all(4 * std::max<size_t>(ns, 1));
  std::vector<uint32_t> kinds(std::max<size_t>(nf, 1)), all_kinds(std::max<size_t>(ns, 1));
  std::vector<float4> mats(std::max<size_t>(ns, 1));
  for (size_t i = 0; i < ns; i++) {
    const Shape& s = sc.shapes[i];
    rec(s, &all[4 * i]);
    all_kinds[i] = s.kind;
    if (i >= sc.num_inf) {
      rec(s, &prims[4 * (i - sc.num_inf)]);
      kinds[i - sc.num_inf] = s.kind;
    }
    mats[i] = make_float4(s.m[0], s.m[1], s.m[2], s.emissive ? 1.0f : 0.0f);
  }
  std::vector<float4> lights(5 * std::max<size_t>(sc.lights.size(), 1));
  for (size_t l = 0; l < sc.lights.size(); l++) {
    const Shape& s = sc.shapes[sc.lights[l]];
    if (s.kind != kTri) { err = "only triangles can be area lights (Tracable::pick_random)"; return false; }
    const float* g = s.g;
    V3 v0 = mk(g[0], g[1], g[2]), v1 = mk(g[3], g[4], g[5]), v2 = mk(g[6], g[7], g[8]);
    float a = len(sub(v0, v1)), b = len(sub(v1, v2)), c = len(sub(v2, v0));
    float sp = (a + b + c) * 0.5f;
    float area = sqrtf(sp * (sp - a) * (sp - b) * (sp - c));
    V3 nn = normalize(cross(sub(v1, v0), sub(v2, v0)));
    lights[5 * l + 0] = make_float4(v0.x, v0.y, v0.z, area);
    lights[5 * l + 1] = make_float4(v1.x, v1.y, v1.z, u2f(sc.lights[l]));
    lights[5 * l + 2] = make_float4(v2.x, v2.y, v2.z, 0.0f);
    lights[5 * l + 3] = make_float4(nn.x, nn.y, nn.z, 0.0f);
    lights[5 * l + 4] = make_float4(s.m[0], s.m[1], s.m[2], 0.0f);
  }
  const std::vector<Node2>& tree_nodes = sc.nodes;
  std::vector<float4> nodes(2 * tree_nodes.size());
  for (size_t i = 0; i < tree_nodes.size(); i++) {
    const Node2& n = tree_nodes[i];
    nodes[2 * i] = make_float4(n.bmin[0], n.bmin[1], n.bmin[2], n.bmax[0]);
    nodes[2 * i + 1] = make_float4(n.bmax[1], n.bmax[2], u2f(n.left_first), u2f(n.count));
  }
  auto up = [&](const void* src, size_t bytes, void** dst) -> bool {
    void* p = nullptr;
    if (hipMalloc(&p, bytes) != hipSuccess) { err = "hipMalloc failed (scene)"; return false; }
    scene_bufs_.push_back(p);
    if (hipMemcpy(p, src, bytes, hipMemcpyHostToDevice) != hipSuccess) { err = "hipMemcpy failed (scene)"; return false; }
    *dst = p;
    return true;
  };
  DevScene ds{};
  void* p;
  if (!up(nodes.data(), nodes.size() * sizeof(float4), &p)) return false;
  ds.nodes = (const float4*)p;
  {
    std::vector<float4> tree;
    uint32_t root_lf = 0;
    const uint32_t root = 0u;
    const bool on = kTreePairs > 0 && sc.use_bvh && !sc.nodes.empty() && tree_nodes[root].count == 0 &&
                    tree_nodes.size() < (size_t)kTreeFlag && treelet_;
    if (on) {
      auto encodable = [&](uint32_t n) {
        return tree_nodes[n].count == 0 || (tree_nodes[n].count < 128u && tree_nodes[n].left_first < (1u << 24));
      };
      std::vector<uint32_t> order;
      std::unordered_map<uint32_t, uint32_t> tix;
      std::deque<uint32_t> q{tree_nodes[root].left_first};
      while (!q.empty() && order.size() < kTreePairs) {
        const uint32_t lf = q.front();
        q.pop_front();
        if (!encodable(lf) || !encodable(lf + 1)) continue;
        tix[lf] = (uint32_t)order.size();
        order.push_back(lf);
        for (uint32_t c = lf; c < lf + 2; c++)
          if (tree_nodes[c].count == 0) q.push_back(tree_nodes[c].left_first);
      }
      for (uint32_t t = 0; t < order.size(); t++) {
        for (uint32_t k = 0; k < 4; k++) tree.push_back(nodes[2 * (size_t)order[t] + k]);
        for (uint32_t c = 0; c < 2; c++) {
          const Node2& n = tree_nodes[order[t] + c];
          auto it = tix.find(n.left_first);
          if (n.count == 0 && it != tix.end()) tree[4 * t + 2 * c + 1].z = u2f(kTreeFlag | it->second);
        }
      }
      if (!order.empty() && order[0] == tree_nodes[root].left_first) root_lf = kTreeFlag;
      else tree.clear();
    }
    ds.tree_pairs = (uint32_t)(tree.size() / 4);
    ds.tree_root_lf = root_lf;
    if (tree.empty()) tree.push_back(make_float4(0.f, 0.f, 0.f, 0.f));
    if (!up(tree.data(), tree.size() * sizeof(float4), &p)) return false;
    ds.tree = (const float4*)p;
  }
  if (!up(prims.data(), prims.size() * sizeof(float4), &p)) return false;
  ds.prims = (const float4*)p;
  if (!up(kinds.data(), kinds.size() * sizeof(uint32_t), &p)) return false;
  ds.kinds = (const uint32_t*)p;
  if (!up(all.data(), all.size() * sizeof(float4), &p)) return false;
  ds.all = (const float4*)p;
  if (!up(all_kinds.data(), all_kinds.size() * sizeof(uint32_t), &p)) return false;
  ds.all_kinds = (const uint32_t*)p;
  if (!up(mats.data(), mats.size() * sizeof(float4), &p)) return false;
  ds.mats = (const float4*)p;
  if (!up(lights.data(), lights.size() * sizeof(float4), &p)) return false;
  ds.lights = (const float4*)p;
  {
    const size_t n4 = std::max<size_t>(sc.nodes4.size(), 1);
    std::vector<Node4> n4v(n4);
    if (!sc.nodes4.empty()) memcpy(n4v.data(), sc.nodes4.data(), sizeof(Node4) * sc.nodes4.size());
    if (!up(n4v.data(), sizeof(Node4) * n4, &p)) return false;
    ds.nodes4 = (const float4*)p;
    std::vector<uint32_t> lt(std::max<size_t>(sc.leaf_table.size(), 2), 0u);
    std::copy(sc.leaf_table.begin(), sc.leaf_table.end(), lt.begin());
    if (!up(lt.data(), sizeof(uint32_t) * lt.size(), &p)) return false;
    ds.leaf_table = (const uint32_t*)p;
    auto mode = [&](int want) {
      const bool b4 = want == 1 || (want == 3 && !sc.tri_only && sc.use_bvh);
      return (b4 && !sc.nodes4.empty()) ? 1 : 0;
    };
    trav_ext_ = mode(traversal_);
    trav_sh_ = mode(traversal_sh_);
  }
  ds.num_inf = sc.num_inf;
  ds.num_finite = (uint32_t)nf;
  ds.num_shapes = (uint32_t)ns;
  ds.num_lights = (uint32_t)sc.lights.size();
  ds.use_bvh = sc.use_bvh ? 1u : 0u;
  ds.tri_only = sc.tri_only ? 1u : 0u;
  ds.refill_lanes = refill_;
  ds.refill_lanes_sh = refill_sh_;
  for (int k = 0; k < 3; k++) ds.bg[k] = sc.background[k];
  for (uint32_t i = 0; i < sc.num_inf && i < (uint32_t)kMaxInf; i++) ds.planes[i] = all[4 * i];
  {
    PresolveBoxes pre{};
    if (sc.use_bvh && nf != 0) pre = sc.pre;
    if (!up(&pre, sizeof pre, &p)) return false;
    ds.pre = (const PresolveBoxes*)p;
    num_guards_ = pre.num_guards;
  }
  ds_ = ds;
  depth_ = sc.depth;
  ds_.stack_cap = (int)std::max<uint32_t>(sc.depth + 2, 3 * sc.depth4 + 4);
  ds_.overflow = d_fallback_ + 2;
  if (!size_grids(err)) return false;
  scene_ok_ = true;
  return true;
}

bool Renderer::set_option(int opt, int64_t v, std::string& err) {
  auto range = [&](int64_t lo, int64_t hi) {
    if (v < lo || v > hi) {
      err = "option value out of range";
      return false;
    }
    return true;
  };
  switch (opt) {
    case 1:
    case 2:
      if (!range(0, 3) || v == 2) { err = "traversal: 0 (bvh2), 1 (bvh4) or 3 (auto)"; return false; }
      (opt == 1 ? traversal_ : traversal_sh_) = (int)v;
      return true;
    case 3: if (!range(0, 1)) return false; fused_ = v != 0; return true;
    case 4: if (!range(0, (int64_t)1 << 40)) return false; fused_below_ = (uint64_t)v; return true;
    case 5: if (!range(1, kMaxLanes)) return false; small_lanes_ = (int)v; return true;
    case 6: if (!range(0, 4096)) return false; pixel_tile_ = (uint32_t)v; return true;
    case 7:
      if (!range(1, 100)) return false;
      grid_pct_ = (int)v;
      return !stream_ || size_grids(err);
    case 8: if (!range(1, 64)) return false; refill_ = (uint32_t)v; ds_.refill_lanes = refill_; return true;
    case 9: if (!range(1, 64)) return false; refill_sh_ = (uint32_t)v; ds_.refill_lanes_sh = refill_sh_; return true;
    case 10: if (!range(0, 1)) return false; treelet_ = v != 0; return true;
    case 12:
      if (!set_lanes((int)v)) { err = "lanes out of range"; return false; }
      return true;
    case 13: if (!range(0, (int64_t)1 << 32)) return false; finish_below_ = (uint64_t)v; return true;
    case 14:
      if (!range(1, 100)) return false;
      trace_grid_pct_ = (int)v;
      return !stream_ || size_grids(err);
    case 20: if (!range(1, 64)) return false; finish_every_ = (int)v; return true;
    case 23:
      if (v != 0 && (v < 64 || v > 4096 || (v & (v - 1)) != 0)) { err = "stock: 0 or a power of two 64..4096"; return false; }
      if (!drain_async(err)) return false;
      stock_drop();
      stock_slots_ = (uint32_t)v;
      return true;
    case 25: if (!range(0, 1)) return false; fill_on_ = v != 0; return true;
    case 30: if (!range(0, 64)) return false; stock_ahead_ = (uint32_t)v; return true;
    case 32: if (!range(1, 1024)) return false; stock_every_ = (uint32_t)v; return true;
    case 33: if (!range(0, 64)) return false; stock_extra_ = (uint32_t)v; return true;
    case 31: if (!range(0, 1)) return false; async_oneshot_ = v != 0; return true;
    case 34: if (!range(0, 1)) return false; log_ = (int)v; return true;
    case 35: if (!range(0, 1)) return false; stock_prefill_ = v != 0; return true;
    case 36: if (!range(0, (int64_t)1 << 40)) return false; async_fused_below_ = (uint64_t)v; return true;
    case 37: if (!range(0, 1)) return false; presolve_ = v != 0; return true;
    case 38: if (!range(0, 1)) return false; drop_miss_ = v != 0; return true;
    case 26:
      if (!range(0, 1)) return false;
      if (!drain_async(err)) return false;
      async_prio_ = (int)v;
      return true;
    case 27: if (!range(0, 100)) return false; async_grid_pct_ = (int)v; return true;
    case 28:
    case 29: err = "read-only option"; return false;
    case 24:
      if (!range(1, kMaxLanes - kAsyncLane0 - 1)) return false;
      if (!drain_async(err)) return false;
      stock_lanes_ = (int)v;
      refill_lane_ = 0;
      return true;
    case 22:
      if (!range(0, 1 << 20)) return false;
      probe_cap_ = (uint32_t)v;
      probe_used_ = 0;
      probe_meta_.clear();
      if (d_probe_) { (void)hipFree(d_probe_); d_probe_ = nullptr; }
      return true;
    default: err = "unknown option"; return false;
  }
}

bool Renderer::get_option(int opt, int64_t& v) const {
  switch (opt) {
    case 1: v = traversal_; return true;
    case 2: v = traversal_sh_; return true;
    case 3: v = fused_ ? 1 : 0; return true;
    case 4: v = (int64_t)fused_below_; return true;
    case 5: v = small_lanes_; return true;
    case 6: v = pixel_tile_; return true;
    case 7: v = grid_pct_; return true;
    case 8: v = refill_; return true;
    case 9: v = refill_sh_; return true;
    case 10: v = treelet_ ? 1 : 0; return true;
    case 12: v = nlanes_; return true;
    case 13: v = (int64_t)finish_below_; return true;
    case 14: v = trace_grid_pct_; return true;
    case 20: v = finish_every_; return true;
    case 22: v = probe_cap_; return true;
    case 23: v = stock_slots_; return true;
    case 25: v = fill_on_ ? 1 : 0; return true;
    case 30: v = stock_ahead_; return true;
    case 32: v = stock_every_; return true;
    case 33: v = stock_extra_; return true;
    case 31: v = async_oneshot_ ? 1 : 0; return true;
    case 34: v = log_; return true;
    case 35: v = stock_prefill_ ? 1 : 0; return true;
    case 36: v = (int64_t)async_fused_below_; return true;
    case 37: v = presolve_ ? 1 : 0; return true;
    case 38: v = drop_miss_ ? 1 : 0; return true;
    case 26: v = async_prio_; return true;
    case 27: v = async_grid_pct_; return true;
    case 28: v = !scene_ok_ ? -1 : !ds_.use_bvh ? 2 : trav_ext_; return true;
    case 29: v = !scene_ok_ ? -1 : ds_.tri_only ? 1 : 0; return true;
    case 24: v = stock_lanes_; return true;
    default: return false;
  }
}

bool Renderer::set_viewport(uint32_t w, uint32_t h, std::string& err) {
  if (!stream_) { err = "no device"; return false; }
  if (w == 0 || h == 0) { err = "empty viewport"; return false; }
  if (!drain_async(err)) return false;
  stock_drop();
  HIP_OK(hipStreamSynchronize(stream_));
  w_ = w;
  h_ = h;
  free_rounds();
  if (d_acc_) (void)hipFree(d_acc_);
  if (d_cnt_) (void)hipFree(d_cnt_);
  if (d_rgba_) (void)hipFree(d_rgba_);
  if (d_samp_) (void)hipFree(d_samp_);
  d_acc_ = nullptr; d_cnt_ = nullptr; d_rgba_ = nullptr; d_samp_ = nullptr;
  HIP_OK(hipMalloc(&d_acc_, sizeof(float4) * (size_t)w * h));
  HIP_OK(hipMalloc(&d_cnt_, sizeof(uint32_t) * (size_t)w * h));
  HIP_OK(hipMalloc(&d_rgba_, 4 * (size_t)w * h));
  HIP_OK(hipMalloc(&d_samp_, 4 * (size_t)w * h));
  return set_partition(rank_, nranks_, tile_, err);
}

void Renderer::set_camera(const float cam[5]) { memcpy(cam_, cam, sizeof cam_); }

bool Renderer::set_partition(uint32_t rank, uint32_t nranks, uint32_t tile, std::string& err) {
  if (nranks == 0 || rank >= nranks || tile == 0) { err = "bad partition"; return false; }
  if (!drain_async(err)) return false;
  stock_drop();
  HIP_OK(hipStreamSynchronize(stream_));
  rank_ = rank; nranks_ = nranks; tile_ = tile;
  part_pix_.clear();
  if (d_part_pix_) { (void)hipFree(d_part_pix_); d_part_pix_ = nullptr; }
  for (uint32_t*& p : d_half_pix_)
    if (p) { (void)hipFree(p); p = nullptr; }
  for (int k = 0; k < 2; k++) {
    if (d_seam_pix_[k]) { (void)hipFree(d_seam_pix_[k]); d_seam_pix_[k] = nullptr; }
    if (d_rest_pix_[k]) { (void)hipFree(d_rest_pix_[k]); d_rest_pix_[k] = nullptr; }
    seam_npix_[k] = rest_npix_[k] = 0;
  }
  if (d_frame_pix_) { (void)hipFree(d_frame_pix_); d_frame_pix_ = nullptr; }
  half_npix_[0] = half_npix_[1] = 0;
  if (d_xidx_) { (void)hipFree(d_xidx_); d_xidx_ = nullptr; }
  maxpart_ = 0;
  if (w_ && h_ && nranks > 1) {
    tile_partition(w_, h_, rank, nranks, tile, part_pix_);
    if (!part_pix_.empty()) {
      HIP_OK(hipMalloc(&d_part_pix_, sizeof(uint32_t) * part_pix_.size()));
      HIP_OK(hipMemcpy(d_part_pix_, part_pix_.data(), sizeof(uint32_t) * part_pix_.size(), hipMemcpyHostToDevice));
    }
    std::vector<std::vector<uint32_t>> parts(nranks);
    for (uint32_t r = 0; r < nranks; r++) {
      tile_partition(w_, h_, r, nranks, tile, parts[r]);
      maxpart_ = std::max<uint64_t>(maxpart_, parts[r].size());
    }
    std::vector<uint32_t> xidx((size_t)nranks * maxpart_, 0xFFFFFFFFu);
    for (uint32_t r = 0; r < nranks; r++)
      std::copy(parts[r].begin(), parts[r].end(), xidx.begin() + (size_t)r * maxpart_);
    if (!xidx.empty()) {
      HIP_OK(hipMalloc(&d_xidx_, sizeof(uint32_t) * xidx.size()));
      HIP_OK(hipMemcpy(d_xidx_, xidx.data(), sizeof(uint32_t) * xidx.size(), hipMemcpyHostToDevice));
    }
  } else if (w_ && h_) {
    part_pix_.resize((size_t)w_ * h_);
    for (size_t i = 0; i < part_pix_.size(); i++) part_pix_[i] = (uint32_t)i;
    const uint32_t tile_px = pixel_tile_;
    std::vector<uint32_t> px;
    tile_order(w_, h_, 0, w_, tile_px, px);
    HIP_OK(hipMalloc(&d_frame_pix_, sizeof(uint32_t) * px.size()));
    HIP_OK(hipMemcpy(d_frame_pix_, px.data(), sizeof(uint32_t) * px.size(), hipMemcpyHostToDevice));
    const uint32_t half = w_ / 2;
    for (int hh = 0; hh < 2; hh++) {
      tile_order(w_, h_, hh ? half : 0u, hh ? w_ : half, tile_px, px);
      half_npix_[hh] = (uint32_t)px.size();
      if (!px.empty()) {
        HIP_OK(hipMalloc(&d_half_pix_[hh], sizeof(uint32_t) * px.size()));
// ... 67 lines not shown
}

bool Renderer::ensure_paths(uint64_t n, std::string& err) { return ensure_lane(0, n, err); }

#define LAUNCH_TIMED(C, slot, accum, counter, ...)                       \
  do {                                                                   \
    hipEvent_t a_ = nullptr, b_ = nullptr;                               \
    if ((C).timed) {                                                     \
      if (!next_event(&a_, err) || !next_event(&b_, err)) return false;  \
      HIP_OK(hipEventRecord(a_, (C).stream));                            \
    }                                                                    \
    __VA_ARGS__;                                                         \
    HIP_OK(hipGetLastError());                                           \
    if ((C).timed) {                                                     \
      HIP_OK(hipEventRecord(b_, (C).stream));                            \
      pending_.push_back(PendingTiming{a_, b_, slot});                   \
    }                                                                    \
  } while (0)

bool Renderer::next_event(hipEvent_t* e, std::string& err) {
  if (ev_used_ == ev_pool_.size()) {
    hipEvent_t x;
    HIP_OK(hipEventCreate(&x));
    ev_pool_.push_back(x);
  }
  *e = ev_pool_[ev_used_++];
  return true;
}

bool Renderer::resolve_timings(std::string& err) {
  std::vector<std::pair<float, float>> iv[kTimedKernels];
  for (const PendingTiming& p : pending_) {
    float ms = 0, t0 = 0, t1 = 0;
    HIP_OK(hipEventElapsedTime(&ms, p.a, p.b));
    HIP_OK(hipEventElapsedTime(&t0, ev_ref_, p.a));
    HIP_OK(hipEventElapsedTime(&t1, ev_ref_, p.b));
    double* acc[kTimedKernels] = {&times_.generate, &times_.extend,     &times_.shade,  &times_.shadow,
                                  &times_.accumulate, &times_.trace, &times_.retrace};
    uint64_t* n[kTimedKernels] = {&times_.n_generate,   &times_.n_extend, &times_.n_shade,  &times_.n_shadow,
                                  &times_.n_accumulate, &times_.n_trace,  &times_.n_retrace};
    *acc[p.slot] += ms;
    *n[p.slot] += 1;
    iv[p.slot].push_back({t0, t1});
  }
  for (int k = 0; k < kTimedKernels; k++) {
    std::sort(iv[k].begin(), iv[k].end());
    double busy = 0, lo = 0, hi = -1e30;
    for (const auto& x : iv[k]) {
      if (x.first > hi) {
        if (hi > lo) busy += hi - lo;
        lo = x.first;
        hi = x.second;
      } else {
        hi = std::max<double>(hi, x.second);
      }
    }
    if (hi > lo) busy += hi - lo;
    times_.busy[k] += busy;
  }
  pending_.clear();
  ev_used_ = 0;
  return true;
}

uint64_t Renderer::batch_cap() const {
  const int nl = main_lanes();
  uint64_t c = lanes_[0].cap;
  for (int i = 1; i < nl; i++) c = std::min(c, lanes_[i].cap);
  return c * (uint64_t)nl;
}

int Renderer::main_lanes() const {
  const bool async = (stock_slots_ || fill_on_) && nranks_ == 1 && (adaptive_[0] || adaptive_[1]);
  return async ? std::min(nlanes_, kAsyncLane0) : nlanes_;
}

static void add_counts(Stats& st, const uint32_t* hc, int b, bool stock, bool presolve) {
  uint64_t& r = stock ? st.stock_rays : st.rays;
  uint64_t& sr = stock ? st.stock_rays : st.shadow_rays;
  for (int i = 0; i < b; i++) {
    const uint32_t drop = presolve ? hc[kResWord + 2 * i + 1] : 0u;
    const uint64_t res = (uint64_t)(presolve ? hc[kResWord + 2 * i] : 0u) + drop;
    r += (i == 0 ? hc[0] : hc[2 + 2 * (i - 1)]) + res;
    sr += hc[3 + 2 * i];
    st.presolved_rays += res;
    st.dropped_rays += drop;
  }
  r += hc[kFinishWord];
  sr += hc[kFinishWord + 1];
  st.finish_paths += hc[kFinishWord + 2];
  st.finish_max_bounces = std::max<uint64_t>(st.finish_max_bounces, hc[kFinishWord + 3]);
}

bool Renderer::flush_counts(std::string& err) {
  if (!stats_pending_) return true;
  for (int l = 0; l < pend_nl_; l++)
    if (!host_wait(lanes_[l].done, err)) return false;
  for (int l = 0; l < pend_nl_; l++) add_counts(stats_, lanes_[l].h_counts, pend_b_, pend_stock_, pend_presolve_);
  stats_pending_ = false;
  return true;
}

void Renderer::batch_counts(const Batch& B, const uint32_t* hc) {
  for (int i = 0; i < B.nl; i++) add_counts(stats_, hc + (size_t)i * kCountWords, B.b, B.stock, B.presolve);
  stats_.bounces += (uint64_t)B.b;
}

bool Renderer::batch_begin(Batch& B, std::string& err) {
  const bool round = B.half >= 0 && !B.moff;
  const uint32_t* rnd_off = B.moff ? B.moff : round ? rounds_[B.half].rc : nullptr;
  const uint32_t* rnd_base = B.moff ? B.mbase : round ? rounds_[B.half].rbase : nullptr;
  const uint32_t npix = B.moff ? B.nent : B.part ? B.npix : (uint32_t)part_pix_.size();
  const uint32_t* part = B.part ? B.part : (nranks_ > 1 ? d_part_pix_ : nullptr);
  GenParams G;
  G.W = w_; G.H = h_; G.npix = npix;
  const float fw = (float)w_, fh = (float)h_;
  G.w_inv = 1.0f / fw; G.h_inv = 1.0f / fh; G.ar = fw / fh;
  G.cam[0] = cam_[0]; G.cam[1] = cam_[1]; G.cam[2] = cam_[2];
  G.cx = mcos(cam_[3]); G.sx = msin(cam_[3]);
  G.cy = mcos(cam_[4]); G.sy = msin(cam_[4]);
  G.seed = seed_;
  G.half = w_ / 2;
  G.left_type = (uint32_t)left_type_; G.right_type = (uint32_t)right_type_;
  const uint32_t slots = B.stock ? stock_used_slots_ : 0u;
  for (int i = 0; i <= B.nl; i++) B.off[i] = B.n * (uint64_t)i / (uint64_t)B.nl;
  B.presolve = presolve_ && max_depth_ > 0 && num_guards_ != 0;
  if (profiling_ && !B.async) HIP_OK(hipEventRecord(ev_ref_, stream_));
  HIP_OK(hipEventRecord(ev_main_, stream_));
  for (int i = 0; i < B.nl; i++) {
    const int l = B.lane0 + i;
    PathSet& L = lanes_[l];
    if (B.presolve && !L.t1 && L.cap) {
      HIP_OK(hipMalloc(&L.t1, 4 * L.cap));
      HIP_OK(hipMalloc(&L.id1, 4 * L.cap));
    }
    const LaunchCtx C = batch_ctx(B, i, 0);
    const hipStream_t s = C.stream;
    if (C.paths > L.cap) { err = "batch exceeds lane capacity"; return false; }
    if (l != 0) HIP_OK(hipStreamWaitEvent(s, ev_main_, 0));
    if (s != L.stream) HIP_OK(hipStreamWaitEvent(s, L.done, 0));
    const uint32_t nn = (uint32_t)C.paths;
    HIP_OK(hipMemsetAsync(L.counts, 0, sizeof(uint32_t) * (B.presolve ? kCountWords : kResWord), s));
    if (B.presolve)
      LAUNCH_TIMED(C, 0, generate, n_generate,
                   k_generate_ps<<<(nn + kBlock * kGenTile - 1u) / (kBlock * kGenTile), kBlock, 0, s>>>(
                       G, part, B.k0 + B.off[i], nn, L.pixel, L.thr[0], L.col, L.ro[0], L.rd[0], L.counts, rnd_off,
                       rnd_base, B.mlist, slots, ds_, L.t, L.id, reinterpret_cast<uint32_t*>(L.res_ctr(0)),
                       drop_miss_ ? 1u : 0u));
    else
      LAUNCH_TIMED(C, 0, generate, n_generate,
                   k_generate<<<blocks_for(nn), kBlock, 0, s>>>(G, part, B.k0 + B.off[i], nn, L.pixel, L.thr[0], L.col,
                                                              L.ro[0], L.rd[0], L.counts, rnd_off, rnd_base, B.mlist,
                                                              slots));
  }
  B.maxb = max_depth_ > 0 ? std::min(max_depth_, kMaxBounces) : kMaxBounces;
  B.fused = (fused_ || B.n < (B.async && async_fused_below_ ? async_fused_below_ : fused_below_)) && trav_ext_ != 1 &&
            trav_sh_ != 1;
  B.pnee = left_type_ == 2 || right_type_ == 2;
  B.b = 0;
  B.finished = false;
  B.state = Batch::kBouncing;
  return true;
}

bool Renderer::batch_advance(Batch& B, bool block, std::string& err) {
  const ShadeParams SP{max_depth_, debug_, drop_miss_ ? 1 : 0};
  auto launch_finish = [&](const LaunchCtx& C, const RayStream& rin, uint32_t g, bool pn) -> bool {
    const PathSet& L = *C.ps;
#define WPT_FIN(T, PN, CR)                                                                                 \
  k_finish<T, PN, CR><<<g, kTBlock, 0, C.stream>>>(ds_, SP, rin, L.ext_count(C.bounce + 1), L.col, L.spill, \
                                                  L.counts + kFinishWord)
#define WPT_FIN2(T, PN) \
  if (B.stock) WPT_FIN(T, PN, true); \
  else WPT_FIN(T, PN, false)
    if (ds_.tri_only) {
      if (pn) WPT_FIN2(true, true);
      else WPT_FIN2(true, false);
    } else {
      if (pn) WPT_FIN2(false, true);
      else WPT_FIN2(false, false);
    }
#undef WPT_FIN2
#undef WPT_FIN
    HIP_OK(hipGetLastError());
    return true;
  };
  while (B.state == Batch::kBouncing || B.state == Batch::kCountWait) {
    if (B.state == Batch::kCountWait) {
      const int b = B.b - 1;
      uint32_t live[kMaxLanes];
      uint64_t left = 0;
      if (B.async) {
        for (int i = 0; i < B.nl; i++) {
          if (!block) {
            const hipError_t q = hipEventQuery(B.live[i]);
            if (q == hipErrorNotReady) return true;
            HIP_OK(q);
          }
          HIP_OK(hipEventSynchronize(B.live[i]));
        }
        for (int i = 0; i < B.nl; i++) live[i] = B.hl[i];
      } else {
        if (async_pending() && !pump(false, err)) return false;
        for (int i = 0; i < B.nl; i++)
          if (!host_wait_stream(lanes_[B.lane0 + i].stream, err)) return false;
        for (int i = 0; i < B.nl; i++) live[i] = lanes_[B.lane0 + i].h_counts[0];
      }
      for (int i = 0; i < B.nl; i++) left += live[i];
      B.state = Batch::kBouncing;
      if (left == 0) break;
      if (left <= finish_below_ && b + 1 < B.maxb) {
        for (int i = 0; i < B.nl; i++) {
          const LaunchCtx C = batch_ctx(B, i, b);
          const PathSet& L = *C.ps;
          if (B.fused && !launch_shadow(C, L.sh_count(b), nullptr, err)) return false;
          if (live[i] == 0) continue;
          const RayStream rin{L.ro[(b + 1) & 1], L.rd[(b + 1) & 1], L.thr[(b + 1) & 1]};
          const uint32_t g =
              (uint32_t)std::min<uint64_t>((live[i] + kTBlock - 1) / kTBlock,
                                           std::min(async_grid(C, grid_tr_[ds_.tri_only ? 1 : 0], trace_grid_pct_),
                                                    spill_grid(L)));
          if (!launch_finish(C, rin, g, B.pnee)) return false;
        }
        B.finished = true;
        break;
      }
      continue;
    }
    if (B.b >= B.maxb) break;
    const int b = B.b;
    for (int i = 0; i < B.nl; i++) {
      const LaunchCtx C = batch_ctx(B, i, b);
      const PathSet& L = *C.ps;
      const uint32_t nn = (uint32_t)C.paths;
      const int hs = C.hit_sel;
      const bool traced = (B.fused && b > 0) ? launch_trace(C, err)
                                             : launch_extend(C, L.ro[b & 1], L.rd[b & 1], L.ext_count(b), err);
      if (!traced) return false;
      {
        const RayStream in{L.ro[b & 1], L.rd[b & 1], L.thr[b & 1]};
        const RayStream out{L.ro[(b + 1) & 1], L.rd[(b + 1) & 1], L.thr[(b + 1) & 1]};
        const ShadowStream sh{L.so, L.sd, L.sc};
        [[maybe_unused]] const uint32_t sgrid =
            std::max<uint32_t>(1, std::min<uint32_t>((nn + kShadeBlock - 1) / kShadeBlock, grid_shade_));
#if WPT_SHADE_GRID_VAR
#define WPT_SHADE_GRID(T, PN, OC, CR, PS)                                                                       \
  const int vi = (PS ? 16 : 0) + (CR ? 8 : 0) + (T ? 4 : 0) + (PN ? 1 + OC : 0);                                \
  const size_t smem = OC ? 4 * (size_t)ds_.oct_lds_words : 0;                                                   \
  if (shade_occ_[vi] == 0 || shade_occ_smem_[vi] != smem) {                                                     \
// ... 751 lines not shown

bool Renderer::results_rgba(uint8_t* out, std::string& err) {
  const uint32_t np = w_ * h_;
  k_rgba<<<blocks_for(np), kBlock, 0, stream_>>>(d_acc_, d_cnt_, np, d_rgba_);
  HIP_OK(hipGetLastError());
  HIP_OK(hipMemcpyAsync(out, d_rgba_, 4 * (size_t)np, hipMemcpyDeviceToHost, stream_));
  HIP_OK(hipStreamSynchronize(stream_));
  return true;
}

bool Renderer::read_radiance(float* acc3, uint32_t* cnt, std::string& err) {
  const size_t np = (size_t)w_ * h_;
  std::vector<float4> a(np);
  HIP_OK(hipMemcpyAsync(a.data(), d_acc_, sizeof(float4) * np, hipMemcpyDeviceToHost, stream_));
  if (cnt) HIP_OK(hipMemcpyAsync(cnt, d_cnt_, sizeof(uint32_t) * np, hipMemcpyDeviceToHost, stream_));
  HIP_OK(hipStreamSynchronize(stream_));
  for (size_t i = 0; i < np; i++) {
    acc3[3 * i] = a[i].x;
    acc3[3 * i + 1] = a[i].y;
    acc3[3 * i + 2] = a[i].z;
  }
  return true;
}

bool Renderer::copy_partition(float* dev_dst, std::string& err) {
  const uint32_t n = (uint32_t)part_pix_.size();
  k_pack_partition<<<blocks_for(n), kBlock, 0, stream_>>>(nranks_ > 1 ? d_part_pix_ : nullptr, n, d_acc_, d_cnt_,
                                                          (float4*)dev_dst);
  HIP_OK(hipGetLastError());
  HIP_OK(hipStreamSynchronize(stream_));
  return true;
}

bool Renderer::launch_extend(const LaunchCtx& C, const float4* ro, const float4* rd, const uint32_t* cnt,
                             std::string& err) {
  const PathSet& L = *C.ps;
  const int v = (ds_.tri_only ? 1 : 0) | (C.count ? 2 : 0) | (trav_ext_ << 2);
  const int full = C.batch_lanes == 1 ? kTravVariants : 0;
  const uint32_t g = std::min(async_grid(C, grid_ext_[v + full], 100), spill_grid(L));
  DevScene ds = ds_;
  ds.probe = probe_slot(C, 1, g);
#define WPT_EXT(T, CN, F)                                                                                     \
  k_extend<T, CN, F><<<g, kTBlock, 0, C.stream>>>(ds, ro, rd, cnt, L.hit_t(C.hit_sel), L.hit_id(C.hit_sel), \
                                                 L.spill, d_work_, d_fallback_)
  switch (v) {
    case 0: LAUNCH_TIMED(C, 1, extend, n_extend, WPT_EXT(false, false, 0)); break;
    case 1: LAUNCH_TIMED(C, 1, extend, n_extend, WPT_EXT(true, false, 0)); break;
    case 2: LAUNCH_TIMED(C, 1, extend, n_extend, WPT_EXT(false, true, 0)); break;
    case 3: LAUNCH_TIMED(C, 1, extend, n_extend, WPT_EXT(true, true, 0)); break;
    case 4: LAUNCH_TIMED(C, 1, extend, n_extend, WPT_EXT(false, false, 1)); break;
    case 5: LAUNCH_TIMED(C, 1, extend, n_extend, WPT_EXT(true, false, 1)); break;
    case 6: LAUNCH_TIMED(C, 1, extend, n_extend, WPT_EXT(false, true, 1)); break;
    default: LAUNCH_TIMED(C, 1, extend, n_extend, WPT_EXT(true, true, 1)); break;
  }
#undef WPT_EXT
  if (ds.probe && C.probe_res) {
    k_probe_add<<<1, 1, 0, C.stream>>>(ds.probe, C.probe_res);
    HIP_OK(hipGetLastError());
  }
  return true;
}

bool Renderer::launch_shadow(const LaunchCtx& C, const uint32_t* cnt, uint8_t* occ_out, std::string& err) {
  const PathSet& L = *C.ps;
  const int v = (ds_.tri_only ? 1 : 0) | (C.count ? 2 : 0) | (trav_sh_ << 2);
  const int full = C.batch_lanes == 1 ? kTravVariants : 0;
  const uint32_t g = std::min(async_grid(C, grid_sh_[v + full], 100), spill_grid(L));
  DevScene ds = ds_;
  ds.probe = probe_slot(C, 3, g);
#define WPT_SH(T, CN, F)                                                                                        \
  k_shadow<T, CN, F><<<g, kTBlock, 0, C.stream>>>(ds, cnt, L.so, L.sd, L.sc, L.col, occ_out, L.spill, d_work_, \
                                                 d_fallback_)
  switch (v) {
    case 0: LAUNCH_TIMED(C, 3, shadow, n_shadow, WPT_SH(false, false, 0)); break;
    case 1: LAUNCH_TIMED(C, 3, shadow, n_shadow, WPT_SH(true, false, 0)); break;
    case 2: LAUNCH_TIMED(C, 3, shadow, n_shadow, WPT_SH(false, true, 0)); break;
    case 3: LAUNCH_TIMED(C, 3, shadow, n_shadow, WPT_SH(true, true, 0)); break;
    case 4: LAUNCH_TIMED(C, 3, shadow, n_shadow, WPT_SH(false, false, 1)); break;
    case 5: LAUNCH_TIMED(C, 3, shadow, n_shadow, WPT_SH(true, false, 1)); break;
    case 6: LAUNCH_TIMED(C, 3, shadow, n_shadow, WPT_SH(false, true, 1)); break;
    default: LAUNCH_TIMED(C, 3, shadow, n_shadow, WPT_SH(true, true, 1)); break;
  }
#undef WPT_SH
  return true;
}

bool Renderer::launch_trace(const LaunchCtx& C, std::string& err) {
  const PathSet& L = *C.ps;
  const int b = C.bounce;
  const int v = (ds_.tri_only ? 1 : 0) | (C.count ? 2 : 0);
  const uint32_t g = std::min(async_grid(C, grid_tr_[v], trace_grid_pct_, 2), spill_grid(L));
  DevScene ds = ds_;
  ds.probe = probe_slot(C, 5, g);
#define WPT_TR(T, CN)                                                                                          \
  k_trace<T, CN><<<g, kTBlock, 0, C.stream>>>(ds, L.ro[b & 1], L.rd[b & 1], L.ext_count(b), L.hit_t(C.hit_sel), \
                                             L.hit_id(C.hit_sel), L.sh_count(b - 1), L.so, L.sd, L.sc, L.col,  \
                                             L.spill, d_work_)
  switch (v) {
    case 0: LAUNCH_TIMED(C, 5, trace, n_trace, WPT_TR(false, false)); break;
    case 1: LAUNCH_TIMED(C, 5, trace, n_trace, WPT_TR(true, false)); break;
    case 2: LAUNCH_TIMED(C, 5, trace, n_trace, WPT_TR(false, true)); break;
    default: LAUNCH_TIMED(C, 5, trace, n_trace, WPT_TR(true, true)); break;
  }
#undef WPT_TR
  if (ds.probe && C.probe_res) {
    k_probe_add<<<1, 1, 0, C.stream>>>(ds.probe, C.probe_res);
    HIP_OK(hipGetLastError());
  }
  return true;
}

uint4* Renderer::probe_slot(const LaunchCtx& C, int kernel, uint32_t grid) {
  if (probe_used_ >= probe_cap_) return nullptr;
  const uint32_t waves = grid * (kTBlock / 64);
  if (!d_probe_) {
    probe_waves_ = max_grid() * (kTBlock / 64);
    const uint64_t cap_max = (1ull << 28) / std::max<uint32_t>(probe_waves_, 1);
    probe_cap_ = (uint32_t)std::min<uint64_t>(probe_cap_, cap_max);
    if (hipMalloc(&d_probe_, sizeof(uint4) * (size_t)probe_waves_ * probe_cap_) != hipSuccess) {
      d_probe_ = nullptr;
      probe_cap_ = 0;
      return nullptr;
    }
  }
  if (waves > probe_waves_) return nullptr;
  const uint32_t first = probe_used_ * probe_waves_;
  probe_meta_.insert(probe_meta_.end(), {(uint32_t)kernel, (uint32_t)C.lane, (uint32_t)C.bounce, waves, first});
  probe_used_++;
  return d_probe_ + first;
}

bool Renderer::probe_read(std::vector<uint32_t>& meta, std::vector<uint4>& rec, double& ticks_per_us,
                          std::string& err) {
  HIP_OK(hipDeviceSynchronize());
  int khz = 0;
  HIP_OK(hipDeviceGetAttribute(&khz, hipDeviceAttributeWallClockRate, device_ < 0 ? 0 : device_));
  ticks_per_us = khz / 1000.0;
  meta = probe_meta_;
  rec.assign((size_t)probe_used_ * probe_waves_, make_uint4(0, 0, 0, 0));
  if (probe_used_) HIP_OK(hipMemcpy(rec.data(), d_probe_, sizeof(uint4) * rec.size(), hipMemcpyDeviceToHost));
  probe_used_ = 0;
  probe_meta_.clear();
  return true;
}

size_t Renderer::spill_slots() const {
  return (size_t)ds_.stack_cap > (size_t)kLdsSlots ? (size_t)ds_.stack_cap - kLdsSlots : 1;
}

uint32_t Renderer::spill_grid(const PathSet& L) const {
  return (uint32_t)std::min<size_t>(L.spill_cap / (spill_slots() * kTBlock), 0xFFFFFFFFu);
}

bool Renderer::ensure_spill(int l, uint32_t grid, std::string& err) {
  PathSet& L = lanes_[l];
  const size_t need = spill_slots() * (size_t)grid * kTBlock;
  if (need <= L.spill_cap) return true;
  HIP_OK(hipStreamSynchronize(L.stream));
  if (L.lo) HIP_OK(hipStreamSynchronize(L.lo));
  if (L.spill) (void)hipFree(L.spill);
  L.spill = nullptr;
  L.spill_cap = 0;
  HIP_OK(hipMalloc(&L.spill, need * sizeof(uint2)));
  L.spill_cap = need;
  return true;
}

uint32_t Renderer::max_grid() const {
  uint32_t g = 0;
  for (uint32_t x : grid_ext_) g = std::max(g, x);
  for (uint32_t x : grid_sh_) g = std::max(g, x);
  for (uint32_t x : grid_tr_) g = std::max(g, x);
  return g;
}

bool Renderer::size_grids(std::string& err) {
  int bpc = 0;
#define WPT_OCC(arr, idx, K)                                                      \
  HIP_OK(hipOccupancyMaxActiveBlocksPerMultiprocessor(&bpc, K, (int)kTBlock, 0)); \
  arr[idx] = (uint32_t)std::max(1, ncu_ * (bpc > 0 ? bpc : 1) * pct / 100);
  for (int full = 0; full < 2; full++) {
    const int pct = full ? 100 : grid_pct_;
    const int o = full ? kTravVariants : 0;
    WPT_OCC(grid_ext_, o + 0, (k_extend<false, false, 0>));
    WPT_OCC(grid_ext_, o + 1, (k_extend<true, false, 0>));
    WPT_OCC(grid_ext_, o + 2, (k_extend<false, true, 0>));
    WPT_OCC(grid_ext_, o + 3, (k_extend<true, true, 0>));
    WPT_OCC(grid_ext_, o + 4, (k_extend<false, false, 1>));
    WPT_OCC(grid_ext_, o + 5, (k_extend<true, false, 1>));
// ... 423 lines not shown
      for (uint32_t oc = 0; oc < 8; oc++) {
        const uint32_t ax = adj(it.kx, (oc & 4u) ? 1 : -1), ay = adj(it.ky, (oc & 2u) ? 1 : -1),
                       az = adj(it.kz, (oc & 1u) ? 1 : -1);
        uint32_t* row = corners.data() + 64 * (size_t)it.node + 8 * oc;
        row[0] = it.node;
        for (uint32_t c = 1; c < 8; c++)
          row[c] = walk((c & 4u) ? ax : it.kx, (c & 2u) ? ay : it.ky, (c & 1u) ? az : it.kz, it.d);
      }
    }
    HIP_OK(hipMalloc(&d_oct_corners_, sizeof(uint32_t) * corners.size()));
    HIP_OK(hipMemcpy(d_oct_corners_, corners.data(), sizeof(uint32_t) * corners.size(), hipMemcpyHostToDevice));
    ds_.oct_corners = d_oct_corners_;
  }
  {
    const size_t nodes = oct_child_.size(), all = nodes + oct_cum_.size();
    ds_.oct_lds_words = all <= kOctLdsWords ? (uint32_t)all : nodes <= kOctLdsWords ? (uint32_t)nodes : 0u;
  }
  photons_ok_ = true;
  return true;
}

bool Renderer::photon_tree(std::vector<uint32_t>& child, std::vector<float>& cum, uint64_t& shot, uint64_t& stored,
                           std::string& err) {
  if (!scene_ok_) { err = "no scene"; return false; }
  if (!build_photons(err)) return false;
  child = oct_child_;
  cum = oct_cum_;
  shot = photons_shot_;
  stored = photons_stored_;
  return true;
}

bool Renderer::trace_rays(size_t n, const float* rays, float* t_out, int32_t* id_out, std::string& err) {
  if (!scene_ok_) { err = "no scene"; return false; }
  if (n == 0) return true;
  if (n > 0xFFFFFFFFull) { err = "too many rays"; return false; }
  if (!ensure_paths(n, err)) return false;
  const PathSet& L = lanes_[0];
  std::vector<float4> o(n), d(n);
  for (size_t i = 0; i < n; i++) {
    const float* r = rays + 6 * i;
    o[i] = make_float4(r[0], r[1], r[2], 0.0f);
    d[i] = make_float4(r[3], r[4], r[5], 0.0f);
  }
  const uint32_t nn = (uint32_t)n;
  HIP_OK(hipMemcpyAsync(L.ro[0], o.data(), 16 * n, hipMemcpyHostToDevice, stream_));
  HIP_OK(hipMemcpyAsync(L.rd[0], d.data(), 16 * n, hipMemcpyHostToDevice, stream_));
  HIP_OK(hipMemcpyAsync(L.counts, &nn, 4, hipMemcpyHostToDevice, stream_));
  if (!launch_extend(lane0_ctx(counting_), L.ro[0], L.rd[0], L.counts, err)) return false;
  HIP_OK(hipMemcpyAsync(t_out, L.t, 4 * n, hipMemcpyDeviceToHost, stream_));
  HIP_OK(hipMemcpyAsync(id_out, L.id, 4 * n, hipMemcpyDeviceToHost, stream_));
  HIP_OK(hipStreamSynchronize(stream_));
  return true;
}

bool Renderer::presolve_rays(size_t n, const float* rays, uint8_t* resolved, float* t_out, int32_t* id_out,
                             std::string& err) {
  if (!scene_ok_) { err = "no scene"; return false; }
  if (n == 0) return true;
  if (n > 0xFFFFFFFFull / 8) { err = "too many rays"; return false; }
  float* dr = nullptr;
  float* dt = nullptr;
  int32_t* di = nullptr;
  uint8_t* df = nullptr;
  bool ok = hipMalloc(&dr, 24 * n) == hipSuccess && hipMalloc(&dt, 4 * n) == hipSuccess &&
            hipMalloc(&di, 4 * n) == hipSuccess && hipMalloc(&df, n) == hipSuccess;
  if (ok) ok = hipMemcpyAsync(dr, rays, 24 * n, hipMemcpyHostToDevice, stream_) == hipSuccess;
  if (ok) {
    k_presolve<<<blocks_for((uint32_t)n), kBlock, 0, stream_>>>(ds_, (uint32_t)n, dr, df, dt, di);
    ok = hipGetLastError() == hipSuccess &&
         hipMemcpyAsync(resolved, df, n, hipMemcpyDeviceToHost, stream_) == hipSuccess &&
         hipMemcpyAsync(t_out, dt, 4 * n, hipMemcpyDeviceToHost, stream_) == hipSuccess &&
         hipMemcpyAsync(id_out, di, 4 * n, hipMemcpyDeviceToHost, stream_) == hipSuccess &&
         hipStreamSynchronize(stream_) == hipSuccess;
  }
  (void)hipFree(dr);
  (void)hipFree(dt);
  (void)hipFree(di);
  (void)hipFree(df);
  if (!ok) err = "HIP error in presolve_rays";
  return ok;
}

bool Renderer::shadow_rays(size_t n, const float* pq, const int32_t* light, uint8_t* occ, std::string& err) {
  if (!scene_ok_) { err = "no scene"; return false; }
  if (n == 0) return true;
  if (n > 0xFFFFFFFFull) { err = "too many rays"; return false; }
  for (size_t i = 0; i < n; i++)
    if (light[i] < (int32_t)ds_.num_inf || light[i] >= (int32_t)ds_.num_shapes) { err = "light id out of range"; return false; }
  if (!ensure_paths(n, err)) return false;
  std::vector<float4> o(n), d(n);
  for (size_t i = 0; i < n; i++) {
    const float* r = pq + 6 * i;
    const V3 p = mk(r[0], r[1], r[2]), q = mk(r[3], r[4], r[5]);
    V3 dir = sub(q, p);
    const float dl = len(dir);
    dir = divs(dir, dl);
    const V3 org = add(p, scale(dir, kEpsilon));
    o[i] = make_float4(org.x, org.y, org.z, dl);
    d[i] = make_float4(dir.x, dir.y, dir.z, u2f((uint32_t)light[i]));
  }
  uint8_t* dq = nullptr;
  HIP_OK(hipMalloc(&dq, n));
  const uint32_t nn = (uint32_t)n;
  const PathSet& L = lanes_[0];
  HIP_OK(hipMemcpyAsync(L.so, o.data(), 16 * n, hipMemcpyHostToDevice, stream_));
  HIP_OK(hipMemcpyAsync(L.sd, d.data(), 16 * n, hipMemcpyHostToDevice, stream_));
  HIP_OK(hipMemcpyAsync(L.counts, &nn, 4, hipMemcpyHostToDevice, stream_));
  const bool ok = launch_shadow(lane0_ctx(counting_), L.counts, dq, err);
  if (ok) {
    HIP_OK(hipMemcpyAsync(occ, dq, n, hipMemcpyDeviceToHost, stream_));
    HIP_OK(hipStreamSynchronize(stream_));
  }
  (void)hipFree(dq);
  return ok;
}

}
```

### wasm-pathtracer_amd/csrc/wpt_scene.cpp

```cpp
#include "wpt_scene.h"

#include <algorithm>
#include <chrono>
#include <cmath>
#include <cstring>

namespace wpt {

namespace {

struct Box {
  float x0, y0, z0, x1, y1, z1;
};
inline Box join(const Box& a, const Box& o) {
  return Box{fminf(a.x0, o.x0), fminf(a.y0, o.y0), fminf(a.z0, o.z0),
             fmaxf(a.x1, o.x1), fmaxf(a.y1, o.y1), fmaxf(a.z1, o.z1)};
}
inline float surface(const Box& b) {
  float xs = b.x1 - b.x0, ys = b.y1 - b.y0, zs = b.z1 - b.z0;
  return 2.0f * (xs * ys + xs * zs + ys * zs);
}

bool shape_bounds(const Shape& s, Box* b, V3* loc) {
  switch (s.kind) {
// ... 292 lines not shown
  sc.leaf_table.clear();
  sc.depth4 = 0;
  if (sc.shapes.size() <= sc.num_inf) return;
  Collapse4 c(sc);
  c.costs();
  if (!c.leaf(0) && c.pick_t(0, 4) == 1) {
    c.make_node(0, 0);
    return;
  }
  sc.nodes4.push_back(Node4{});
  std::vector<Collapse4::Entry> kids;
  c.cut(0, 4, kids, 1);
  c.fill(0, kids);
}

void build_guards(HostScene& sc) {
  sc.pre = PresolveBoxes{};
  sc.leaf_guard.assign(sc.nodes.size(), ~0u);
  if (sc.shapes.size() <= sc.num_inf || sc.nodes.empty()) return;
  std::vector<uint32_t> leaves;
  {
    std::vector<uint32_t> todo{0u};
    while (!todo.empty()) {
      const uint32_t n = todo.back();
      todo.pop_back();
      if (sc.nodes[n].count != 0) { leaves.push_back(n); continue; }
      todo.push_back(sc.nodes[n].left_first);
      todo.push_back(sc.nodes[n].left_first + 1);
    }
  }
  struct Group {
    std::vector<uint32_t> leaves;
    float b[6];
    bool whole = false;
  };
  auto bounds = [&](Group& g) {
    for (int k = 0; k < 3; k++) { g.b[k] = INFINITY; g.b[3 + k] = -INFINITY; }
    for (uint32_t n : g.leaves)
      for (int k = 0; k < 3; k++) {
        g.b[k] = fminf(g.b[k], sc.nodes[n].bmin[k]);
        g.b[3 + k] = fmaxf(g.b[3 + k], sc.nodes[n].bmax[k]);
      }
  };
  auto area = [](const Group& g) {
    const double x = (double)g.b[3] - g.b[0], y = (double)g.b[4] - g.b[1], z = (double)g.b[5] - g.b[2];
    return x * y + y * z + z * x;
  };
  std::vector<Group> groups(1);
  groups[0].leaves = leaves;
  bounds(groups[0]);
  while (groups.size() < (size_t)kMaxGuards) {
    int pick = -1;
    for (size_t i = 0; i < groups.size(); i++)
      if (!groups[i].whole && groups[i].leaves.size() > 1 && (pick < 0 || area(groups[i]) > area(groups[pick])))
        pick = (int)i;
    if (pick < 0) break;
    Group& g = groups[pick];
    float best_gap = 0.0f, cut = 0.0f;
    int axis = -1;
    for (int k = 0; k < 3; k++) {
      std::vector<uint32_t> ord = g.leaves;
      std::sort(ord.begin(), ord.end(), [&](uint32_t a, uint32_t b) { return sc.nodes[a].bmin[k] < sc.nodes[b].bmin[k]; });
      float hi = sc.nodes[ord[0]].bmax[k];
      for (size_t i = 1; i < ord.size(); i++) {
        const float lo = sc.nodes[ord[i]].bmin[k];
        if (lo > hi && lo - hi > best_gap) { best_gap = lo - hi; cut = lo; axis = k; }
        hi = fmaxf(hi, sc.nodes[ord[i]].bmax[k]);
      }
    }
    if (axis < 0) { g.whole = true; continue; }
    Group a, b;
    for (uint32_t n : g.leaves) (sc.nodes[n].bmin[axis] < cut ? a : b).leaves.push_back(n);
    bounds(a);
    bounds(b);
    groups[pick] = std::move(a);
    groups.push_back(std::move(b));
  }
  sc.pre.num_guards = (uint32_t)groups.size();
  for (int k = 0; k < 3; k++) { sc.pre.root[k] = sc.nodes[0].bmin[k]; sc.pre.root[3 + k] = sc.nodes[0].bmax[k]; }
  for (size_t i = 0; i < groups.size(); i++) {
    for (int k = 0; k < 6; k++) sc.pre.guard[i][k] = groups[i].b[k];
    for (uint32_t n : groups[i].leaves) sc.leaf_guard[n] = (uint32_t)i;
  }
}

bool scene_init(HostScene& sc, std::vector<Shape> shapes, const float bg[3], Bvh2Builder* gpu, std::string* err) {
  sc.background[0] = bg[0]; sc.background[1] = bg[1]; sc.background[2] = bg[2];
  sc.use_bvh = true;
  sc.nodes.clear();
  Builder b(sc.nodes);
  std::vector<Shape> finite;
  finite.reserve(shapes.size());
  b.loc.reserve(shapes.size());
  b.box.reserve(shapes.size());
  uint32_t num_inf = 0;
  for (size_t i = 0; i < shapes.size(); i++) {
    Box bx;
    V3 lc;
    if (shape_bounds(shapes[i], &bx, &lc)) {
      b.loc.push_back(lc);
      b.box.push_back(bx);
      finite.push_back(shapes[i]);
    } else {
      std::swap(shapes[num_inf], shapes[i]);
      num_inf++;
    }
  }
  sc.num_inf = num_inf;
  sc.nodes.push_back(Node2{});
  sc.nodes.push_back(Node2{});
  sc.depth = 0;
  sc.shapes.reserve(shapes.size());
  sc.shapes.assign(shapes.begin(), shapes.begin() + num_inf);
  sc.bvh_on_gpu = false;
  sc.bvh_ms = 0.0;
  if (!finite.empty() && gpu && finite.size() >= gpu->min_shapes) {
    static_assert(sizeof(Box) == 6 * sizeof(float) && sizeof(V3) == 3 * sizeof(float), "packed boxes");
    std::string e;
    if (!gpu->build(&b.box[0].x0, &b.loc[0].x, finite.size(), sc.nodes, b.ord, sc.depth, sc.bvh_ms, e)) {
      if (err) *err = e;
      return false;
    }
    sc.bvh_on_gpu = true;
    for (uint32_t i : b.ord) sc.shapes.push_back(finite[i]);
  } else if (!finite.empty()) {
    const auto t0 = std::chrono::steady_clock::now();
    b.ord.resize(finite.size());
    for (size_t i = 0; i < finite.size(); i++) b.ord[i] = (uint32_t)i;
    for (auto& bn : b.bins) bn.reserve(finite.size());
    Box all;
    b.hull(b.ord.data(), b.ord.size(), &all);
    uint32_t maxd = 0;
    Node2 root = b.subdivide(0, finite.size(), all, 0, &maxd);
    sc.nodes[0] = root;
    sc.depth = maxd;
    sc.bvh_ms = std::chrono::duration<double, std::milli>(std::chrono::steady_clock::now() - t0).count();
    for (uint32_t i : b.ord) sc.shapes.push_back(finite[i]);
  }
  sc.tri_only = true;
  for (size_t i = num_inf; i < sc.shapes.size(); i++)
    if (sc.shapes[i].kind != kTri) sc.tri_only = false;
  sc.lights.clear();
  for (size_t i = 0; i < sc.shapes.size(); i++)
    if (sc.shapes[i].emissive) sc.lights.push_back((uint32_t)i);
  sc.nodes4.clear();
  sc.leaf_table.clear();
  sc.depth4 = 0;
  if (sc.want_bvh4 == 1 || (sc.want_bvh4 == 2 && !sc.tri_only && sc.use_bvh)) build_bvh4(sc);
  build_guards(sc);
  return true;
}

namespace {
V3 clamp_color(float r, float g, float b) { return mk(clamp01(r), clamp01(g), clamp01(b)); }

void museum_lights(std::vector<Shape>& s, float x, float y, V3 color) {
  V3 lc1 = mk(x - 1.0f, 0.0f, y + 2.8f), lc2 = mk(x + 1.0f, 0.0f, y + 2.8f);
  V3 lc3 = mk(x + 1.0f, 1.0f, y + 2.5f), lc4 = mk(x - 1.0f, 1.0f, y + 2.5f);
  s.push_back(make_triangle(lc3, lc2, lc1, true, color));
  s.push_back(make_triangle(lc4, lc3, lc1, true, color));
  lc1 = mk(x - 1.0f, 0.0f, y - 2.8f); lc2 = mk(x + 1.0f, 0.0f, y - 2.8f);
  lc3 = mk(x + 1.0f, 1.0f, y - 2.5f); lc4 = mk(x - 1.0f, 1.0f, y - 2.5f);
  s.push_back(make_triangle(lc3, lc2, lc1, true, color));
  s.push_back(make_triangle(lc4, lc3, lc1, true, color));
}

// ... 94 lines not shown
```

### wasm-pathtracer_amd/interface.py

```python
import ctypes

import numpy as np

from ._lib import lib

OK = 0
ERR_NOT_INIT, ERR_ALREADY_INIT, ERR_INVALID_SCENE, ERR_INVALID_ARG = -1, -2, -3, -4
ERR_UNSUPPORTED, ERR_DEVICE, ERR_NO_MESH = -5, -6, -7
NO_NEE, NORMAL_NEE, PNEE = 0, 1, 2


class WptError(RuntimeError):
    def __init__(self, code, msg):
        super().__init__(f"[{code}] {msg}")
        self.code = code


def _check(rc):
    if rc < 0:
        raise WptError(rc, lib().wpt_last_error().decode())
    return rc


def init(width, height, scene_id, cam_x, cam_y, cam_z, cam_rot_x, cam_rot_y):
# ... 82 lines not shown
    mesh_vertices(mesh_id, v.shape[0])[:] = v
    return notify_mesh_loaded(mesh_id)


def set_device(dev):
    _check(lib().wpt_set_device(dev))


def set_render_options(max_depth=0, frame_seed=0xBABABEBE, batch_paths=0):
    _check(lib().wpt_set_render_options(max_depth, frame_seed, batch_paths))


def set_partition(rank, nranks, tile=16):
    _check(lib().wpt_set_partition(rank, nranks, tile))


def partition_pixels():
    n = _check(lib().wpt_partition_pixels(None))
    out = np.empty(n, dtype=np.uint32)
    _check(lib().wpt_partition_pixels(out.ctypes.data))
    return out


def tile_partition(width, height, rank, nranks, tile=16):
    n = _check(lib().wpt_tile_partition(width, height, rank, nranks, tile, None))
    out = np.empty(n, dtype=np.uint32)
    _check(lib().wpt_tile_partition(width, height, rank, nranks, tile, out.ctypes.data))
    return out


def photon_tree(num_lights):
    n = _check(lib().wpt_photon_tree(None, None, None))
    child = np.empty(n, dtype=np.uint32)
    cum = np.empty(n * max(num_lights, 1), dtype=np.float32)
    ss = np.empty(2, dtype=np.uint64)
    _check(lib().wpt_photon_tree(child.ctypes.data, cum.ctypes.data, ss.ctypes.data))
    return child, cum[: n * num_lights].reshape(n, num_lights), int(ss[0]), int(ss[1])


def read_radiance(width, height):
    acc = np.empty(width * height * 3, dtype=np.float32)
    cnt = np.empty(width * height, dtype=np.uint32)
    _check(lib().wpt_read_radiance(acc.ctypes.data, cnt.ctypes.data))
    return acc.reshape(height, width, 3), cnt.reshape(height, width)


def comm_unique_id():
    buf = ctypes.create_string_buffer(128)
    _check(lib().wpt_comm_unique_id(buf))
    return buf.raw


def set_comm(rank, nranks, tile, unique_id):
    uid = ctypes.create_string_buffer(bytes(unique_id), 128)
    _check(lib().wpt_set_comm(rank, nranks, tile, uid))


def gather_frame(root=0):
    _check(lib().wpt_gather_frame(root))


def gather_plan(rank, nranks, root, slot):
    n = _check(lib().wpt_gather_plan(rank, nranks, root, slot, None))
    out = np.zeros(4 * max(n, 1), dtype=np.uint64)
    _check(lib().wpt_gather_plan(rank, nranks, root, slot, out.ctypes.data))
    return [(int(a), int(b), int(c), bool(d)) for a, b, c, d in out[: 4 * n].reshape(-1, 4)]


def comm_destroy():
    _check(lib().wpt_comm_destroy())


def copy_partition(device_ptr):
    _check(lib().wpt_copy_partition(ctypes.c_void_p(device_ptr)))


def stats():
    keys = ("paths", "rays", "shadow_rays", "node_visits", "prim_tests", "bounces", "ext_visits", "ext_tests",
            "ext_node_bytes", "sh_visits", "sh_tests", "sh_node_bytes", "fallback_ext", "fallback_sh",
            "ext_lane_iters", "ext_live_iters", "sh_lane_iters", "sh_live_iters", "photon_rays", "photons",
            "sum_chunks", "sum_resummed", "sum_fetched", "stock_consumed", "fill_paths", "trace_bytes",
            "finish_paths", "finish_max_bounces", "max_ray_visits", "ex_body_lanes", "ex_bodies", "lf_body_lanes",
            "lf_bodies", "stock_traced", "stock_deficit", "stock_waits", "plan_us", "stock_us",
            "stock_rays", "stock_rays_used", "presolved_rays", "dropped_rays")
    out = (ctypes.c_uint64 * len(keys))()
    _check(lib().wpt_stats(ctypes.addressof(out), len(keys)))
    return dict(zip(keys, list(out)))


def kernel_times():
    out = (ctypes.c_double * 28)()
    _check(lib().wpt_kernel_times(ctypes.addressof(out), 28))
    names = ("generate", "extend", "shade", "shadow", "accumulate", "trace")
    kt = {n: {"ms": out[2 * i], "launches": int(out[2 * i + 1]), "busy_ms": out[12 + 2 * i],
              "logical_launches": int(out[13 + 2 * i])} for i, n in enumerate(names)}
    return kt


def set_counting(on):
    _check(lib().wpt_set_counting(1 if on else 0))


def set_profiling(on):
    _check(lib().wpt_set_profiling(1 if on else 0))


def scene_build_info():
    out = (ctypes.c_double * 2)()
    _check(lib().wpt_scene_build_info(ctypes.addressof(out)))
    return float(out[0]), bool(out[1])


def set_lanes(n):
    _check(lib().wpt_set_lanes(int(n)))


OPTIONS = {"defaults": 0, "traversal": 1, "traversal_sh": 2, "fused": 3, "fused_below": 4, "small_lanes": 5, "pixel_tile": 6,
           "grid_pct": 7, "refill": 8, "refill_sh": 9, "treelet": 10, "bvh_build": 11, "lanes": 12,
           "finish_below": 13, "trace_grid_pct": 14, "finish_every": 20, "probe": 22, "stock": 23, "stock_lanes": 24,
           "fill": 25, "async_prio": 26, "async_grid_pct": 27, "scene_traversal": 28, "scene_tri_only": 29,
           "stock_ahead": 30, "async_oneshot": 31, "stock_every": 32, "stock_extra": 33,
           "log": 34, "stock_prefill": 35, "async_fused_below": 36, "presolve": 37, "drop_miss": 38}
TRAVERSALS = {"bvh2": 0, "bvh4": 1, "auto": 3}
OPTION_VALUES = {"traversal": TRAVERSALS, "traversal_sh": TRAVERSALS,
                 "bvh_build": {"auto": 0, "host": 1, "gpu": 2}}


def set_option(name, value):
    if isinstance(value, str) and not value.lstrip("-").isdigit():
        value = OPTION_VALUES[name][value]
    _check(lib().wpt_set_option(OPTIONS[name], int(value)))


def get_option(name):
    v = ctypes.c_int64(0)
    _check(lib().wpt_get_option(OPTIONS[name], ctypes.addressof(v)))
    return v.value


def probe_read():
    L = lib()
    ent = ctypes.c_uint64(0)
    tpu = ctypes.c_double(0.0)
    n = L.wpt_probe_read(None, None, ctypes.addressof(ent), ctypes.addressof(tpu))
    if n < 0:
        raise WptError(int(n), L.wpt_last_error().decode())
    meta = np.zeros((n, 5), np.uint32)
    rec = np.zeros((ent.value, 4), np.uint32)
    if n:
        ent.value = rec.shape[0]
        _check(L.wpt_probe_read(meta.ctypes.data, rec.ctypes.data, ctypes.addressof(ent), ctypes.addressof(tpu)))
    return meta, rec, tpu.value


def clear_stats():
    _check(lib().wpt_clear_stats())


def sync():
    _check(lib().wpt_sync())


def bvh_depth():
    return _check(lib().wpt_bvh_depth())


def trace_rays(rays):
    r = np.ascontiguousarray(rays, dtype=np.float32).reshape(-1, 6)
    n = r.shape[0]
    t = np.empty(n, dtype=np.float32)
    ids = np.empty(n, dtype=np.int32)
    _check(lib().wpt_trace_rays(n, r.ctypes.data, t.ctypes.data, ids.ctypes.data))
    return t, ids


def shadow_rays(pq, light_ids):
    p = np.ascontiguousarray(pq, dtype=np.float32).reshape(-1, 6)
    li = np.ascontiguousarray(light_ids, dtype=np.int32)
    occ = np.empty(p.shape[0], dtype=np.uint8)
    _check(lib().wpt_shadow_rays(p.shape[0], p.ctypes.data, li.ctypes.data, occ.ctypes.data))
    return occ.astype(bool)


def presolve_rays(rays):
    r = np.ascontiguousarray(rays, dtype=np.float32).reshape(-1, 6)
    n = r.shape[0]
    res = np.zeros(n, dtype=np.uint8)
    t = np.empty(n, dtype=np.float32)
    ids = np.empty(n, dtype=np.int32)
    _check(lib().wpt_presolve_rays(n, r.ctypes.data, res.ctypes.data, t.ctypes.data, ids.ctypes.data))
    return res.astype(bool), t, ids


def shutdown():
    _check(lib().wpt_shutdown())


class DebugScene:

    def __init__(self, scene_id, mesh=None, gpu=False):
        L = lib()
        m = None if mesh is None else np.ascontiguousarray(mesh, dtype=np.float32)
        new = L.wpt_debug_scene_new_gpu if gpu else L.wpt_debug_scene_new
        self.h = new(scene_id, None if m is None else m.ctypes.data, 0 if m is None else m.size // 3)
        if not self.h:
            raise WptError(ERR_INVALID_SCENE, L.wpt_last_error().decode())
        bi = np.zeros(2, dtype=np.float64)
        _check(L.wpt_debug_scene_build_info(self.h, bi.ctypes.data))
        self.bvh_ms, self.bvh_on_gpu = float(bi[0]), bool(bi[1])
        info = np.zeros(8, dtype=np.uint64)
        L.wpt_debug_scene_info(self.h, info.ctypes.data)
        (self.num_shapes, self.num_inf, self.num_nodes, self.num_lights, self.depth, self.use_bvh,
         self.tri_only, self.num_nodes4) = (int(x) for x in info)

    def nodes(self):
        out = np.empty((self.num_nodes, 8), dtype=np.uint32)
        lib().wpt_debug_scene_nodes(self.h, out.ctypes.data)
        return out

    def nodes4(self):
        out = np.empty((self.num_nodes4, 37), dtype=np.uint32)
        if self.num_nodes4:
            lib().wpt_debug_scene_nodes4(self.h, out.ctypes.data)
        return out

    def shapes(self):
        out = np.empty((self.num_shapes, 16), dtype=np.float32)
        lib().wpt_debug_scene_shapes(self.h, out.ctypes.data)
        return out

    def lights(self):
        out = np.empty(self.num_lights, dtype=np.uint32)
        lib().wpt_debug_scene_lights(self.h, out.ctypes.data)
        return out

    def presolve(self, rays):
        r = np.ascontiguousarray(rays, dtype=np.float32).reshape(-1, 6)
        n = r.shape[0]
        res = np.zeros(n, dtype=np.uint8)
        t = np.empty(n, dtype=np.float32)
        ids = np.empty(n, dtype=np.int32)
        _check(lib().wpt_debug_scene_presolve(self.h, n, r.ctypes.data, res.ctypes.data, t.ctypes.data,
                                              ids.ctypes.data))
        return res.astype(bool), t, ids

    def guards(self):
        ng = ctypes.c_uint32(0)
        boxes = np.zeros(30, dtype=np.float32)
        lg = np.zeros(max(self.num_nodes, 1), dtype=np.uint32)
        _check(lib().wpt_debug_scene_guards(self.h, ctypes.addressof(ng), boxes.ctypes.data, lg.ctypes.data))
        return boxes[:6].copy(), boxes[6:].reshape(4, 6)[: ng.value].copy(), lg[: self.num_nodes]

    def __del__(self):
        try:
            if getattr(self, "h", None):
                lib().wpt_debug_scene_free(self.h)
                self.h = None
        except Exception:
            pass
```

Before: 9635 Mray/s.

## Presolve unoccluded shadow rays in shade kernel and add contributions directly

Adds a conservative shadow-ray presolve in the shade kernel. It tests infinite planes, guard boxes that hold no lights, and a few emissive guard triangles, so that shadow rays which provably reach the light skip the shadow traversal stream and add their contribution straight to the color buffer. The goal is to cut the number of shadow rays enqueued and traversed in the BVH. In exchange it adds per-lane slab and triangle tests, a third packed counter field (the packing narrows from 16-bit to 10-bit fields), an extra atomic lane, and non-atomic color updates from the shade kernel.

```diff
diff --git a/include/wpt.h b/include/wpt.h
--- a/include/wpt.h
+++ b/include/wpt.h
@@ -123,6 +123,7 @@
 #define WPT_OPT_ASYNC_FUSED_BELOW 36
 #define WPT_OPT_PRESOLVE 37
 #define WPT_OPT_DROP_MISS 38
+#define WPT_OPT_PRESOLVE_SHADOW 39
 #define WPT_OPT_LOG 34
 #define WPT_OPT_SCENE_TRAVERSAL 28
 #define WPT_OPT_SCENE_TRI_ONLY 29
@@ -137,6 +138,7 @@
 int wpt_trace_rays(size_t n, const float* rays, float* t_out, int32_t* id_out);
 int wpt_shadow_rays(size_t n, const float* pq, const int32_t* light, uint8_t* occluded);
 int wpt_presolve_rays(size_t n, const float* rays, uint8_t* resolved, float* t_out, int32_t* id_out);
+int wpt_presolve_shadow_rays(size_t n, const float* pq, const int32_t* light, uint8_t* resolved);
 
 int wpt_shutdown(void);
 
@@ -148,6 +150,8 @@
 int wpt_debug_scene_lights(void* h, uint32_t* out);
 int wpt_debug_scene_presolve(void* h, size_t n, const float* rays, uint8_t* resolved, float* t_out, int32_t* id_out);
 int wpt_debug_scene_guards(void* h, uint32_t* num_guards, float* boxes, uint32_t* leaf_guard);
+int wpt_debug_scene_presolve_shadow(void* h, size_t n, const float* pq, const int32_t* light, uint8_t* resolved);
+int wpt_debug_scene_guard_lights(void* h, uint32_t* light_guards, uint32_t* num, int32_t* ids);
 void wpt_debug_scene_free(void* h);
 void* wpt_debug_scene_new_gpu(int32_t scene_id, const float* mesh_vertices, size_t num_vertices);
 int wpt_debug_scene_build_info(void* h, double* out);
diff --git a/wasm-pathtracer_amd/_lib.py b/wasm-pathtracer_amd/_lib.py
--- a/wasm-pathtracer_amd/_lib.py
+++ b/wasm-pathtracer_amd/_lib.py
@@ -53,6 +53,9 @@
     "wpt_presolve_rays": (ctypes.c_int, [c_sz, c_p, c_p, c_p, c_p]),
     "wpt_debug_scene_presolve": (ctypes.c_int, [c_p, c_sz, c_p, c_p, c_p, c_p]),
     "wpt_debug_scene_guards": (ctypes.c_int, [c_p, c_p, c_p, c_p]),
+    "wpt_presolve_shadow_rays": (ctypes.c_int, [c_sz, c_p, c_p, c_p]),
+    "wpt_debug_scene_presolve_shadow": (ctypes.c_int, [c_p, c_sz, c_p, c_p, c_p]),
+    "wpt_debug_scene_guard_lights": (ctypes.c_int, [c_p, c_p, c_p, c_p]),
     "wpt_shutdown": (ctypes.c_int, []),
     "wpt_debug_scene_new": (c_p, [c_i32, c_p, c_sz]),
     "wpt_debug_scene_info": (ctypes.c_int, [c_p, c_p]),
diff --git a/wasm-pathtracer_amd/csrc/wpt_api.cpp b/wasm-pathtracer_amd/csrc/wpt_api.cpp
--- a/wasm-pathtracer_amd/csrc/wpt_api.cpp
+++ b/wasm-pathtracer_amd/csrc/wpt_api.cpp
@@ -517,7 +517,7 @@
   std::string err;
   if (!g_session->renderer.flush_counts(err)) return fail(WPT_ERR_DEVICE, err);
   const Stats& st = g_session->renderer.stats();
-  uint64_t v[42] = {st.paths,          st.rays,           st.shadow_rays,    st.node_visits,  st.prim_tests,
+  uint64_t v[43] = {st.paths,          st.rays,           st.shadow_rays,    st.node_visits,  st.prim_tests,
                     st.bounces,        st.ext_visits,     st.ext_tests,      st.ext_node_bytes, st.sh_visits,
                     st.sh_tests,       st.sh_node_bytes,  st.fallback_ext,   st.fallback_sh,  st.ext_lane_iters,
                     st.ext_live_iters, st.sh_lane_iters,  st.sh_live_iters,  st.photon_rays,  st.photons,
@@ -526,8 +526,8 @@
                     st.ex_body_lanes,  st.ex_bodies,      st.lf_body_lanes,  st.lf_bodies,    st.stock_traced,
                     st.stock_deficit,  st.stock_waits,    st.plan_us,        st.stock_us,
                     st.stock_rays,     st.stock_rays_used, st.presolved_rays,
-                    st.dropped_rays};
-  for (size_t i = 0; i < n && i < 42; i++) out[i] = v[i];
+                    st.dropped_rays,   st.shadow_presolved_rays};
+  for (size_t i = 0; i < n && i < 43; i++) out[i] = v[i];
   return WPT_OK;
 }
 
@@ -688,6 +688,14 @@
   if (n && (!rays || !resolved || !t_out || !id_out)) return fail(WPT_ERR_INVALID_ARG, "null argument");
   std::string err;
   if (!g_session->renderer.presolve_rays(n, rays, resolved, t_out, id_out, err)) return fail(WPT_ERR_DEVICE, err);
+  return WPT_OK;
+}
+
+int wpt_presolve_shadow_rays(size_t n, const float* pq, const int32_t* light, uint8_t* resolved) {
+  if (!g_session) return fail(WPT_ERR_NOT_INIT, "init not called");
+  if (n && (!pq || !light || !resolved)) return fail(WPT_ERR_INVALID_ARG, "null argument");
+  std::string err;
+  if (!g_session->renderer.presolve_shadow_rays(n, pq, light, resolved, err)) return fail(WPT_ERR_DEVICE, err);
   return WPT_OK;
 }
 
@@ -846,6 +854,46 @@
   return WPT_OK;
 }
 
+static void host_presolve_view(const HostScene* sc, HostPlanes& hp, PresolveBoxes& pre) {
+  hp = HostPlanes{};
+  pre = PresolveBoxes{};
+  if (sc->use_bvh && sc->shapes.size() > sc->num_inf && sc->num_inf <= 16) {
+    pre = sc->pre;
+    hp.num_inf = sc->num_inf;
+    for (uint32_t i = 0; i < sc->num_inf; i++) {
+      const float* g = sc->shapes[i].g;
+      const V3 loc = mk(g[0], g[1], g[2]), nrm = mk(g[3], g[4], g[5]);
+      hp.planes[i] = HostPlanes::P4{nrm.x, nrm.y, nrm.z, dot(nrm, loc)};
+    }
+  }
+}
+
+int wpt_debug_scene_presolve_shadow(void* h, size_t n, const float* pq, const int32_t* light, uint8_t* resolved) {
+  const HostScene* sc = (const HostScene*)h;
+  if (!sc || (n && (!pq || !light || !resolved))) return fail(WPT_ERR_INVALID_ARG, "null argument");
+  HostPlanes hp;
+  PresolveBoxes pre;
+  host_presolve_view(sc, hp, pre);
+  for (size_t i = 0; i < n; i++) {
+    const float* r = pq + 6 * i;
+    V3 o, d;
+    float dl;
+    shadow_operands(mk(r[0], r[1], r[2]), mk(r[3], r[4], r[5]), o, d, dl);
+    resolved[i] = presolve_shadow(hp, pre, o, d, dl, light[i]) ? 1 : 0;
+  }
+  return WPT_OK;
+}
+
+int wpt_debug_scene_guard_lights(void* h, uint32_t* light_guards, uint32_t* num, int32_t* ids) {
+  const HostScene* sc = (const HostScene*)h;
+  if (!sc || !light_guards || !num) return fail(WPT_ERR_INVALID_ARG, "null argument");
+  *light_guards = sc->pre.light_guards;
+  *num = sc->pre.num_guard_lights;
+  if (ids)
+    for (int k = 0; k < kMaxGuardLights; k++) ids[k] = (uint32_t)k < sc->pre.num_guard_lights ? sc->pre.guard_light_id[k] : -1;
+  return WPT_OK;
+}
+
 int wpt_debug_scene_guards(void* h, uint32_t* num_guards, float* boxes, uint32_t* leaf_guard) {
   const HostScene* sc = (const HostScene*)h;
   if (!sc || !num_guards) return fail(WPT_ERR_INVALID_ARG, "null argument");
diff --git a/wasm-pathtracer_amd/csrc/wpt_presolve.h b/wasm-pathtracer_amd/csrc/wpt_presolve.h
--- a/wasm-pathtracer_amd/csrc/wpt_presolve.h
+++ b/wasm-pathtracer_amd/csrc/wpt_presolve.h
@@ -4,11 +4,16 @@
 namespace wpt {
 
 constexpr int kMaxGuards = 4;
+constexpr int kMaxGuardLights = 4;
 
 struct PresolveBoxes {
   uint32_t num_guards;
   float root[6];
   float guard[kMaxGuards][6];
+  uint32_t light_guards;
+  uint32_t num_guard_lights;
+  int32_t guard_light_id[kMaxGuardLights];
+  float guard_light[kMaxGuardLights][16];
 };
 
 WPT_HD void presolve_slab(const float* b, V3 o, V3 inv, float& hh, float& tmax) {
@@ -77,6 +82,77 @@
   return true;
 }
 
+
+WPT_HD void tri_record(const float* g, float* out) {
+  const V3 v0 = mk(g[0], g[1], g[2]), v1 = mk(g[3], g[4], g[5]), v2 = mk(g[6], g[7], g[8]);
+  const V3 n = cross(sub(v1, v0), sub(v2, v0));
+  const V3 nn = normalize(n);
+  const float od = dot(n, v0);
+  out[0] = v0.x; out[1] = v0.y; out[2] = v0.z; out[3] = n.x;
+  out[4] = v1.x; out[5] = v1.y; out[6] = v1.z; out[7] = n.y;
+  out[8] = v2.x; out[9] = v2.y; out[10] = v2.z; out[11] = n.z;
+  out[12] = nn.x; out[13] = nn.y; out[14] = nn.z; out[15] = od;
+}
+
+WPT_HD bool tri_hit_rec(const float* r, V3 o, V3 d, float& t) {
+  const V3 n = mk(r[3], r[7], r[11]);
+  const float n_dot_d = dot(n, d);
+  if (n_dot_d == 0.0f) return false;
+  const float tt = (r[15] - dot(n, o)) / n_dot_d;
+  if (tt <= 0.0f) return false;
+  const V3 nn = mk(r[12], r[13], r[14]);
+  const V3 pp = add(o, scale(d, tt));
+  const V3 v0 = mk(r[0], r[1], r[2]), v1 = mk(r[4], r[5], r[6]), v2 = mk(r[8], r[9], r[10]);
+  if (!(dot(nn, cross(sub(v1, v0), sub(pp, v0))) + kTriSlack >= 0.0f)) return false;
+  if (!(dot(nn, cross(sub(v2, v1), sub(pp, v1))) + kTriSlack >= 0.0f)) return false;
+  if (!(dot(nn, cross(sub(v0, v2), sub(pp, v2))) + kTriSlack >= 0.0f)) return false;
+  t = tt;
+  return true;
+}
+
+WPT_HD void shadow_operands(V3 p, V3 q, V3& o, V3& d, float& dir_len) {
+  V3 tl = sub(q, p);
+  dir_len = sqrtf(dot(tl, tl));
+  tl = divs(tl, dir_len);
+  o = add(p, scale(tl, kEpsilon));
+  d = tl;
+}
+
+template <class SC>
+WPT_HD bool presolve_shadow(const SC& S, const PresolveBoxes& B, V3 o, V3 d, float dir_len, int32_t light) {
+  if (B.num_guards == 0u) return false;
+  if (d.x == 0.0f || d.y == 0.0f || d.z == 0.0f) return false;
+  const V3 inv = mk(1.0f / d.x, 1.0f / d.y, 1.0f / d.z);
+  const float inf = presolve_inf();
+  if (!(fabsf(inv.x) < inf) || !(fabsf(inv.y) < inf) || !(fabsf(inv.z) < inf)) return false;
+  for (uint32_t i = 0; i < S.num_inf; i++) {
+    const V3 n = mk(S.planes[i].x, S.planes[i].y, S.planes[i].z);
+    const float n_dot_dir = dot(n, d);
+    if (n_dot_dir == 0.0f) continue;
+    const float tt = (S.planes[i].w - dot(n, o)) / n_dot_dir;
+    if (tt <= 0.0f) continue;
+    if (0.0f < tt && !(tt >= dir_len)) return false;
+  }
+  bool clear = true;
+#if defined(__HIP_DEVICE_COMPILE__)
+#pragma unroll
+#endif
+  for (int g = 0; g < kMaxGuards; g++) {
+    if ((uint32_t)g < B.num_guards && ((B.light_guards >> g) & 1u) == 0u) {
+      float hh, tmax;
+      presolve_slab(B.guard[g], o, inv, hh, tmax);
+      clear = clear && (!(hh <= tmax) || dir_len < hh);
+    }
+  }
+  if (!clear) return false;
+  for (uint32_t k = 0; k < B.num_guard_lights; k++) {
+    if (B.guard_light_id[k] == light) continue;
+    float t;
+    if (tri_hit_rec(B.guard_light[k], o, d, t) && !(t >= dir_len)) return false;
+  }
+  return true;
+}
+
 struct HostPlanes {
   struct P4 { float x, y, z, w; };
   P4 planes[16];
diff --git a/wasm-pathtracer_amd/csrc/wpt_render.h b/wasm-pathtracer_amd/csrc/wpt_render.h
--- a/wasm-pathtracer_amd/csrc/wpt_render.h
+++ b/wasm-pathtracer_amd/csrc/wpt_render.h
@@ -67,6 +67,7 @@
   uint64_t stock_rays_used = 0;
   uint64_t presolved_rays = 0;
   uint64_t dropped_rays = 0;
+  uint64_t shadow_presolved_rays = 0;
 };
 
 constexpr int kTimedKernels = 7;
@@ -81,8 +82,9 @@
 constexpr uint64_t kMinLanePaths = 1024;
 constexpr size_t kFinishWord = 2 + 2 * (size_t)kMaxBounces;
 constexpr size_t kResWord = kFinishWord + 4;
-constexpr size_t kCountWords = kResWord + 2 * ((size_t)kMaxBounces + 1);
-static_assert(kResWord % 2 == 0, "the presolved counts are 64-bit slots");
+constexpr size_t kShResWord = kResWord + 2 * ((size_t)kMaxBounces + 1);
+constexpr size_t kCountWords = kShResWord + 2 * ((size_t)kMaxBounces + 1);
+static_assert(kResWord % 2 == 0 && kShResWord % 2 == 0, "the presolved counts are 64-bit slots");
 constexpr uint32_t kWorkWords = 16;
 constexpr uint32_t kWorkCopies = 64;
 struct PathSet {
@@ -191,6 +193,7 @@
   bool unpack_ranks(const float4* gathered, uint64_t slot, std::string& err);
   bool trace_rays(size_t n, const float* rays, float* t_out, int32_t* id_out, std::string& err);
   bool presolve_rays(size_t n, const float* rays, uint8_t* resolved, float* t_out, int32_t* id_out, std::string& err);
+  bool presolve_shadow_rays(size_t n, const float* pq, const int32_t* light, uint8_t* resolved, std::string& err);
   bool shadow_rays(size_t n, const float* pq, const int32_t* light, uint8_t* occ, std::string& err);
   bool probe_read(std::vector<uint32_t>& meta, std::vector<uint4>& rec, double& ticks_per_us, std::string& err);
   void set_counting(bool on) { counting_ = on; }
@@ -401,8 +404,10 @@
   uint64_t finish_below_ = 1u << 18;
   int finish_every_ = 4;
   uint32_t num_guards_ = 0;
+  uint32_t light_guards_ = 0;
   bool presolve_ = true;
   bool drop_miss_ = true;
+  bool presolve_shadow_ = true;
   uint32_t probe_cap_ = 0, probe_waves_ = 0, probe_used_ = 0;
   uint4* d_probe_ = nullptr;
   std::vector<uint32_t> probe_meta_;
diff --git a/wasm-pathtracer_amd/csrc/wpt_render.hip b/wasm-pathtracer_amd/csrc/wpt_render.hip
--- a/wasm-pathtracer_amd/csrc/wpt_render.hip
+++ b/wasm-pathtracer_amd/csrc/wpt_render.hip
@@ -1031,6 +1031,7 @@
   int max_depth;
   int debug;
   int drop_miss;
+  int presolve_shadow;
 };
 
 struct RayStream {
@@ -1177,6 +1178,14 @@
   if (!R.alive) end_counts((flags >> kShadowShift) + (R.shadow ? 1u : 0u));
 }
 
+__device__ __forceinline__ void add_contribution_xyz(float4* __restrict__ col, float4 c) {
+  float* p = &col[__float_as_uint(c.w)].x;
+  const float x = p[0] + c.x, y = p[1] + c.y, z = p[2] + c.z;
+  p[0] = x;
+  p[1] = y;
+  p[2] = z;
+}
+
 template <bool TRI_ONLY, bool PNEE, int OCT, bool CR = false, bool PS = false>
 __global__ void WPT_SHADE_BOUNDS k_shade(DevScene S, ShadeParams P, RayStream in, RayStream out,
                                                        ShadowStream sh, float4* __restrict__ col,
@@ -1186,7 +1195,8 @@
                                                        float* __restrict__ t_nx, int32_t* __restrict__ id_nx,
                                                        uint32_t end) {
   constexpr uint32_t kWaves = kShadeBlock / 64;
-  static_assert(kWaves < 64, "the scan's totals and the second atomic lane sit in one wave");
+  static_assert(kWaves + 1 < 64, "the scan's totals and the other atomic lanes sit in one wave");
+  static_assert(kShadeBlock < 1024, "three 10-bit fields in the scan's third column");
   __shared__ uint32_t s_off[PS ? 3 : 2][kWaves];
   __shared__ f4v s_light[5 * kShadeLights];
   const uint32_t nh = *count;
@@ -1249,12 +1259,18 @@
         }
       }
     }
-    const uint64_t am = __ballot(R.alive && !res), sm = __ballot(R.shadow), rm = PS ? __ballot(res) : 0ull;
-    const uint64_t dm = PS ? __ballot(drop) : 0ull;
+    bool sres = false;
+    if constexpr (PS && !(PNEE && OCT == 0)) {
+      if (R.shadow && P.presolve_shadow)
+        sres = presolve_shadow(S, *S.pre, ld3(R.so), ld3(R.sd), R.so.w, (int32_t)__float_as_uint(R.sd.w));
+    }
+    const uint64_t am = __ballot(R.alive && !res), sm = __ballot(R.shadow && !sres), rm = PS ? __ballot(res) : 0ull;
+    const uint64_t dm = PS ? __ballot(drop) : 0ull, zm = PS ? __ballot(sres) : 0ull;
     if (lane == 0) {
       s_off[0][wid] = (uint32_t)__popcll(am);
       s_off[1][wid] = (uint32_t)__popcll(sm);
-      if constexpr (PS) s_off[2][wid] = (uint32_t)__popcll(rm) | ((uint32_t)__popcll(dm) << 16);
+      if constexpr (PS)
+        s_off[2][wid] = (uint32_t)__popcll(rm) | ((uint32_t)__popcll(dm) << 10) | ((uint32_t)__popcll(zm) << 20);
     }
     __syncthreads();
     if constexpr (!PS) {
@@ -1288,17 +1304,18 @@
       unsigned long long base = 0ull;
       uint32_t off;
       asm volatile("v_mov_b32 %0, %1" : "=v"(off) : "i"((uint32_t)(kResWord / 2)));
-      if (lane == kWaves - 1 || lane == kWaves)
-        base = atomicAdd(append + (lane == kWaves - 1 ? 0u : off),
-                         lane == kWaves - 1 ? ((unsigned long long)ia | ((unsigned long long)ib << 32))
-                                            : ((unsigned long long)(tc & 0xffffu) | ((unsigned long long)(tc >> 16) << 32)));
+      if (lane == kWaves + 1) asm volatile("v_mov_b32 %0, %1" : "=v"(off) : "i"((uint32_t)((kShResWord - 2) / 2)));
+      unsigned long long inc = (unsigned long long)ia | ((unsigned long long)ib << 32);
+      if (lane == kWaves) inc = (unsigned long long)(tc & 0x3ffu) | ((unsigned long long)((tc >> 10) & 0x3ffu) << 32);
+      if (lane == kWaves + 1) inc = (unsigned long long)(tc >> 20);
+      if (lane >= kWaves - 1 && lane <= kWaves + 1) base = atomicAdd(append + (lane == kWaves - 1 ? 0u : off), inc);
       const uint32_t ba = (uint32_t)__shfl((int)(uint32_t)base, (int)(kWaves - 1), 64);
       const uint32_t bb = (uint32_t)__shfl((int)(uint32_t)(base >> 32), (int)(kWaves - 1), 64);
       const uint32_t bc = (uint32_t)__shfl((int)(uint32_t)base, (int)kWaves, 64);
       if (lane < kWaves) {
         s_off[0][lane] = ba + ia - a;
         s_off[1][lane] = bb + ib - b;
-        s_off[2][lane] = bc + ((ic - c) & 0xffffu);
+        s_off[2][lane] = bc + ((ic - c) & 0x3ffu);
       }
     }
     __syncthreads();
@@ -1317,7 +1334,9 @@
         }
       }
     }
-    if (R.shadow) {
+    if (sres) {
+      add_contribution_xyz(col, R.sc);
+    } else if (R.shadow) {
       const uint32_t p = s_off[1][wid] + (uint32_t)__popcll(sm & below);
       st_stream(sh.o + p, R.so);
       st_stream(sh.d + p, R.sd);
@@ -1780,6 +1799,7 @@
 }
 
 __global__ void k_probe_add(uint4* rec, const uint32_t* __restrict__ res) { rec[0].w += res[0] + res[1]; }
+__global__ void k_probe_add_sh(uint4* rec, const uint32_t* __restrict__ sres) { rec[0].w += sres[0]; }
 
 __global__ void __launch_bounds__(kBlock) k_presolve(DevScene S, uint32_t n, const float* __restrict__ rays,
                                                      uint8_t* __restrict__ resolved, float* __restrict__ t_out,
@@ -1793,6 +1813,15 @@
   resolved[i] = res ? 1 : 0;
   t_out[i] = t;
   id_out[i] = id;
+}
+
+__global__ void __launch_bounds__(kBlock) k_presolve_shadow(DevScene S, uint32_t n, const float4* __restrict__ so,
+                                                            const float4* __restrict__ sd,
+                                                            uint8_t* __restrict__ resolved) {
+  const uint32_t i = blockIdx.x * kBlock + threadIdx.x;
+  if (i >= n) return;
+  const float4 o = so[i], d = sd[i];
+  resolved[i] = presolve_shadow(S, *S.pre, ld3(o), ld3(d), o.w, (int32_t)__float_as_uint(d.w)) ? 1 : 0;
 }
 
 __global__ void __launch_bounds__(kBlock) k_accumulate(const uint32_t* __restrict__ part_pix, uint64_t k0, uint32_t n,
@@ -2045,14 +2074,7 @@
     memset(out, 0, 4 * sizeof(float4));
     const float* g = s.g;
     if (s.kind == kTri) {
-      V3 v0 = mk(g[0], g[1], g[2]), v1 = mk(g[3], g[4], g[5]), v2 = mk(g[6], g[7], g[8]);
-      V3 n = cross(sub(v1, v0), sub(v2, v0));
-      V3 nn = normalize(n);
-      float od = dot(n, v0);
-      out[0] = make_float4(v0.x, v0.y, v0.z, n.x);
-      out[1] = make_float4(v1.x, v1.y, v1.z, n.y);
-      out[2] = make_float4(v2.x, v2.y, v2.z, n.z);
-      out[3] = make_float4(nn.x, nn.y, nn.z, od);
+      tri_record(g, &out[0].x);
     } else if (s.kind == kPlane) {
       V3 loc = mk(g[0], g[1], g[2]), n = mk(g[3], g[4], g[5]);
       out[0] = make_float4(n.x, n.y, n.z, dot(n, loc));
@@ -2199,6 +2221,7 @@
     if (!up(&pre, sizeof pre, &p)) return false;
     ds.pre = (const PresolveBoxes*)p;
     num_guards_ = pre.num_guards;
+    light_guards_ = pre.light_guards;
   }
   ds_ = ds;
   depth_ = sc.depth;
@@ -2259,6 +2282,7 @@
     case 36: if (!range(0, (int64_t)1 << 40)) return false; async_fused_below_ = (uint64_t)v; return true;
     case 37: if (!range(0, 1)) return false; presolve_ = v != 0; return true;
     case 38: if (!range(0, 1)) return false; drop_miss_ = v != 0; return true;
+    case 39: if (!range(0, 1)) return false; presolve_shadow_ = v != 0; return true;
     case 26:
       if (!range(0, 1)) return false;
       if (!drain_async(err)) return false;
@@ -2312,6 +2336,7 @@
     case 36: v = (int64_t)async_fused_below_; return true;
     case 37: v = presolve_ ? 1 : 0; return true;
     case 38: v = drop_miss_ ? 1 : 0; return true;
+    case 39: v = presolve_shadow_ ? 1 : 0; return true;
     case 26: v = async_prio_; return true;
     case 27: v = async_grid_pct_; return true;
     case 28: v = !scene_ok_ ? -1 : !ds_.use_bvh ? 2 : trav_ext_; return true;
@@ -2545,9 +2570,11 @@
     const uint32_t drop = presolve ? hc[kResWord + 2 * i + 1] : 0u;
     const uint64_t res = (uint64_t)(presolve ? hc[kResWord + 2 * i] : 0u) + drop;
     r += (i == 0 ? hc[0] : hc[2 + 2 * (i - 1)]) + res;
-    sr += hc[3 + 2 * i];
+    const uint32_t sres = presolve ? hc[kShResWord + 2 * i] : 0u;
+    sr += (uint64_t)hc[3 + 2 * i] + sres;
     st.presolved_rays += res;
     st.dropped_rays += drop;
+    st.shadow_presolved_rays += sres;
   }
   r += hc[kFinishWord];
   sr += hc[kFinishWord + 1];
@@ -2627,7 +2654,7 @@
 }
 
 bool Renderer::batch_advance(Batch& B, bool block, std::string& err) {
-  const ShadeParams SP{max_depth_, debug_, drop_miss_ ? 1 : 0};
+  const ShadeParams SP{max_depth_, debug_, drop_miss_ ? 1 : 0, presolve_shadow_ && light_guards_ != 0 ? 1 : 0};
   auto launch_finish = [&](const LaunchCtx& C, const RayStream& rin, uint32_t g, bool pn) -> bool {
     const PathSet& L = *C.ps;
 #define WPT_FIN(T, PN, CR)                                                                                 \
@@ -3545,6 +3572,10 @@
     default: LAUNCH_TIMED(C, 3, shadow, n_shadow, WPT_SH(true, true, 1)); break;
   }
 #undef WPT_SH
+  if (ds.probe && C.probe_res) {
+    k_probe_add_sh<<<1, 1, 0, C.stream>>>(ds.probe, cnt + (kShResWord - 3));
+    HIP_OK(hipGetLastError());
+  }
   return true;
 }
 
@@ -3568,6 +3599,7 @@
 #undef WPT_TR
   if (ds.probe && C.probe_res) {
     k_probe_add<<<1, 1, 0, C.stream>>>(ds.probe, C.probe_res);
+    k_probe_add_sh<<<1, 1, 0, C.stream>>>(ds.probe, L.sh_count(b - 1) + (kShResWord - 3));
     HIP_OK(hipGetLastError());
   }
   return true;
@@ -4157,6 +4189,41 @@
   return ok;
 }
 
+bool Renderer::presolve_shadow_rays(size_t n, const float* pq, const int32_t* light, uint8_t* resolved,
+                                    std::string& err) {
+  if (!scene_ok_) { err = "no scene"; return false; }
+  if (n == 0) return true;
+  if (n > 0xFFFFFFFFull / 16) { err = "too many rays"; return false; }
+  std::vector<float4> o(n), d(n);
+  for (size_t i = 0; i < n; i++) {
+    const float* r = pq + 6 * i;
+    V3 org, dir;
+    float dl;
+    shadow_operands(mk(r[0], r[1], r[2]), mk(r[3], r[4], r[5]), org, dir, dl);
+    o[i] = make_float4(org.x, org.y, org.z, dl);
+    d[i] = make_float4(dir.x, dir.y, dir.z, u2f((uint32_t)light[i]));
+  }
+  float4* dso = nullptr;
+  float4* dsd = nullptr;
+  uint8_t* df = nullptr;
+  bool ok = hipMalloc(&dso, 16 * n) == hipSuccess && hipMalloc(&dsd, 16 * n) == hipSuccess &&
+            hipMalloc(&df, n) == hipSuccess;
+  if (ok)
+    ok = hipMemcpyAsync(dso, o.data(), 16 * n, hipMemcpyHostToDevice, stream_) == hipSuccess &&
+         hipMemcpyAsync(dsd, d.data(), 16 * n, hipMemcpyHostToDevice, stream_) == hipSuccess;
+  if (ok) {
+    k_presolve_shadow<<<blocks_for((uint32_t)n), kBlock, 0, stream_>>>(ds_, (uint32_t)n, dso, dsd, df);
+    ok = hipGetLastError() == hipSuccess &&
+         hipMemcpyAsync(resolved, df, n, hipMemcpyDeviceToHost, stream_) == hipSuccess &&
+         hipStreamSynchronize(stream_) == hipSuccess;
+  }
+  (void)hipFree(dso);
+  (void)hipFree(dsd);
+  (void)hipFree(df);
+  if (!ok) err = "HIP error in presolve_shadow_rays";
+  return ok;
+}
+
 bool Renderer::shadow_rays(size_t n, const float* pq, const int32_t* light, uint8_t* occ, std::string& err) {
   if (!scene_ok_) { err = "no scene"; return false; }
   if (n == 0) return true;
diff --git a/wasm-pathtracer_amd/csrc/wpt_scene.cpp b/wasm-pathtracer_amd/csrc/wpt_scene.cpp
--- a/wasm-pathtracer_amd/csrc/wpt_scene.cpp
+++ b/wasm-pathtracer_amd/csrc/wpt_scene.cpp
@@ -398,6 +398,24 @@
     for (int k = 0; k < 6; k++) sc.pre.guard[i][k] = groups[i].b[k];
     for (uint32_t n : groups[i].leaves) sc.leaf_guard[n] = (uint32_t)i;
   }
+  for (size_t i = 0; i < groups.size(); i++) {
+    std::vector<uint32_t> prims;
+    bool lights_only = true;
+    for (uint32_t n : groups[i].leaves)
+      for (uint32_t k = 0; k < sc.nodes[n].count && lights_only; k++) {
+        const size_t sid = (size_t)sc.num_inf + sc.nodes[n].left_first + k;
+        lights_only = sid < sc.shapes.size() && sc.shapes[sid].kind == kTri && sc.shapes[sid].emissive &&
+                      prims.size() < (size_t)kMaxGuardLights;
+        prims.push_back((uint32_t)sid);
+      }
+    if (!lights_only || prims.empty() || sc.pre.num_guard_lights + prims.size() > (size_t)kMaxGuardLights) continue;
+    sc.pre.light_guards |= 1u << i;
+    for (uint32_t sid : prims) {
+      const uint32_t k = sc.pre.num_guard_lights++;
+      sc.pre.guard_light_id[k] = (int32_t)sid;
+      tri_record(sc.shapes[sid].g, sc.pre.guard_light[k]);
+    }
+  }
 }
 
 bool scene_init(HostScene& sc, std::vector<Shape> shapes, const float bg[3], Bvh2Builder* gpu, std::string* err) {
diff --git a/wasm-pathtracer_amd/interface.py b/wasm-pathtracer_amd/interface.py
--- a/wasm-pathtracer_amd/interface.py
+++ b/wasm-pathtracer_amd/interface.py
@@ -188,7 +188,8 @@
             "sum_chunks", "sum_resummed", "sum_fetched", "stock_consumed", "fill_paths", "trace_bytes",
             "finish_paths", "finish_max_bounces", "max_ray_visits", "ex_body_lanes", "ex_bodies", "lf_body_lanes",
             "lf_bodies", "stock_traced", "stock_deficit", "stock_waits", "plan_us", "stock_us",
-            "stock_rays", "stock_rays_used", "presolved_rays", "dropped_rays")
+            "stock_rays", "stock_rays_used", "presolved_rays", "dropped_rays",
+            "shadow_presolved_rays")
     out = (ctypes.c_uint64 * len(keys))()
     _check(lib().wpt_stats(ctypes.addressof(out), len(keys)))
     return dict(zip(keys, list(out)))
@@ -226,7 +227,8 @@
            "finish_below": 13, "trace_grid_pct": 14, "finish_every": 20, "probe": 22, "stock": 23, "stock_lanes": 24,
            "fill": 25, "async_prio": 26, "async_grid_pct": 27, "scene_traversal": 28, "scene_tri_only": 29,
            "stock_ahead": 30, "async_oneshot": 31, "stock_every": 32, "stock_extra": 33,
-           "log": 34, "stock_prefill": 35, "async_fused_below": 36, "presolve": 37, "drop_miss": 38}
+           "log": 34, "stock_prefill": 35, "async_fused_below": 36, "presolve": 37, "drop_miss": 38,
+           "presolve_shadow": 39}
 TRAVERSALS = {"bvh2": 0, "bvh4": 1, "auto": 3}
 OPTION_VALUES = {"traversal": TRAVERSALS, "traversal_sh": TRAVERSALS,
                  "bvh_build": {"auto": 0, "host": 1, "gpu": 2}}
@@ -296,6 +298,14 @@
     ids = np.empty(n, dtype=np.int32)
     _check(lib().wpt_presolve_rays(n, r.ctypes.data, res.ctypes.data, t.ctypes.data, ids.ctypes.data))
     return res.astype(bool), t, ids
+
+
+def presolve_shadow_rays(pq, light_ids):
+    p = np.ascontiguousarray(pq, dtype=np.float32).reshape(-1, 6)
+    li = np.ascontiguousarray(light_ids, dtype=np.int32)
+    res = np.zeros(p.shape[0], dtype=np.uint8)
+    _check(lib().wpt_presolve_shadow_rays(p.shape[0], p.ctypes.data, li.ctypes.data, res.ctypes.data))
+    return res.astype(bool)
 
 
 def shutdown():
@@ -350,6 +360,20 @@
                                               ids.ctypes.data))
         return res.astype(bool), t, ids
 
+    def presolve_shadow(self, pq, light_ids):
+        p = np.ascontiguousarray(pq, dtype=np.float32).reshape(-1, 6)
+        li = np.ascontiguousarray(light_ids, dtype=np.int32)
+        res = np.zeros(p.shape[0], dtype=np.uint8)
+        _check(lib().wpt_debug_scene_presolve_shadow(self.h, p.shape[0], p.ctypes.data, li.ctypes.data,
+                                                     res.ctypes.data))
+        return res.astype(bool)
+
+    def guard_lights(self):
+        m, n = ctypes.c_uint32(0), ctypes.c_uint32(0)
+        ids = np.full(4, -1, dtype=np.int32)
+        _check(lib().wpt_debug_scene_guard_lights(self.h, ctypes.addressof(m), ctypes.addressof(n), ids.ctypes.data))
+        return m.value, ids[: n.value].copy()
+
     def guards(self):
         ng = ctypes.c_uint32(0)
         boxes = np.zeros(30, dtype=np.float32)
```

After: 9773 Mray/s (median of 6 runs). 1.01x the previous value.
